# microsoft/esvit

Measured on NVIDIA H100. Metric: multi-crop images/sec, Swin-T W7 pretrain step (2 global 224^2 + 8 local 96^2 crops, DDINOLoss V+R, K=65536), higher is better.
Workload: dtype bf16

## Files before the change

esvit_b200/_lib.py:

```python
from __future__ import annotations

import ctypes
import os
from ctypes import c_double, c_float, c_int, c_longlong, c_void_p

HERE = os.path.dirname(os.path.abspath(__file__))
LIB_PATH = os.path.join(HERE, "lib", "libesvit_b200.so")
HEADER_PATH = os.path.join(os.path.dirname(HERE), "include", "esvit_b200.h")

ERR_BAD_ARG = 1001

P, I, L, F, D = c_void_p, c_int, c_longlong, c_float, c_double

SIGNATURES = {
    "esvit_add_ln_fwd": [P, P, P, I, P, P, F, P, P, I, P, P, L, I, P],
    "esvit_add_ln_bwd": [P, I, P, P, P, P, P, P, I, P, P, P, P, P, L, I, P],
    "esvit_patch_merge_ln_fwd": [P, P, P, F, P, P, P, I, I, I, I, P],
    "esvit_patch_merge_ln_bwd": [P, P, P, P, P, P, P, P, I, I, I, I, P],
    "esvit_token_mean_fwd": [P, P, I, I, I, P],
    "esvit_token_mean_bwd": [P, P, P, I, I, I, P],
    "esvit_patch_embed_fwd": [P, P, P, P, P, F, P, P, P, I, I, I, I, P],
    "esvit_patch_embed_bwd": [P, P, P, P, P, P, P, P, P, P, P, I, I, I, I, P],
    "esvit_window_attn_expand_bias": [P, P, I, I, P],
    "esvit_window_attn_fwd": [P, P, P, P, I, P, P, I, I, I, I, I, I, I, F, P],
    "esvit_window_attn_bwd": [P, P, P, P, I, P, P, P, P, P, P, I, I, I, I, I, I, I, F, P],
    "esvit_window_attn_probs": [P, P, P, P, I, P, I, I, I, I, I, I, I, F, P],
    "esvit_gemm_bias_act": [P, P, P, P, P, L, I, I, I, P],
    "esvit_gemm_mul_colsum": [P, P, P, P, P, P, L, I, I, P],
    "esvit_gemm_bf16": [P, P, P, P, P, L, I, I, I, I, I, I, P],
    "esvit_gemm_mul_colsum2": [P, P, P, P, P, P, L, I, I, I, I, P],
    "esvit_gemm_wgrad_ws_floats": [I, I],
    "esvit_gemm_wgrad": [P, P, P, P, L, I, I, I, I, P],
    "esvit_mlp_fwd": [P, P, P, P, P, P, P, P, L, I, P],
    "esvit_gelu_fwd": [P, P, L, P],
    "esvit_gelu_bwd": [P, P, P, L, P],
    "esvit_gelu_bwd_dbias": [P, P, P, P, L, I, P],
    "esvit_mul_bwd_dbias": [P, P, P, P, L, I, P],
    "esvit_l2norm_fwd": [P, P, P, F, L, I, P],
    "esvit_l2norm_bwd": [P, P, P, P, L, I, P],
    "esvit_weight_norm_fwd": [P, P, P, P, L, I, P],
    "esvit_weight_norm_bwd": [P, P, P, P, I, P, P, L, I, P],
    "esvit_row_lse": [P, P, F, P, L, I, P],
    "esvit_dino_ce_fwd": [P, P, P, P, P, P, P, F, F, P, L, I, P],
    "esvit_dino_ce_bwd": [P, P, P, P, P, P, P, P, P, F, F, P, L, I, P],
    "esvit_weighted_sum": [P, P, I, P, P],
    "esvit_row_softmax_q_max_k": [],
    "esvit_row_softmax_q": [P, P, F, P, P, L, I, P],
    "esvit_dino_ce_q_fwd": [P, P, P, P, P, F, P, L, I, P],
    "esvit_dino_ce_q_bwd": [P, P, P, P, P, P, P, F, P, L, I, P],
    "esvit_mixup_q_kpad": [I],
    "esvit_mixup_q": [P, P, I, I, I, F, P, P, P, P],
    "esvit_colsum_workspace_rows": [],
    "esvit_colsum": [P, L, I, P, P, P],
    "esvit_center_ema": [P, P, F, F, P, I, P],
    "esvit_normalize_rows": [P, P, L, I, F, P],
    "esvit_region_match": [P, P, I, I, I, I, I, P, P, P],
    "esvit_mhsa_fwd": [P, P, P, I, I, I, I, F, P],
    "esvit_mhsa_bwd": [P, P, P, P, P, P, I, I, I, I, F, P],
    "esvit_conv_im2col": [P, P, I, I, I, I, I, I, I, I, I, P],
    "esvit_conv_col2im": [P, P, I, I, I, I, I, I, I, I, P],
    "esvit_mhsa_win_fwd": [P, P, P, I, I, I, I, I, I, F, P],
    "esvit_mhsa_win_bwd": [P, P, P, P, P, P, I, I, I, I, I, I, F, P],
    "esvit_dwbn_fwd_stats": [P, P, P, P, P, I, I, I, I, I, I, P],
    "esvit_dwbn_fwd_apply": [P, P, P, P, P, P, P, P, P, L, I, I, F, F, P],
    "esvit_dwbn_bwd_stats": [P, P, P, P, P, P, P, L, I, P],
    "esvit_dwbn_bwd_apply": [P, P, P, P, P, P, P, P, P, P, I, I, I, I, I, I, I, P],
    "esvit_vil_sc_ws_floats": [I, I, I, I],
    "esvit_vil_sc_fwd": [P, P, P, P, P, P, P, P, I, I, I, I, F, P],
    "esvit_vil_sc_bwd": [P, P, P, P, P, P, P, P, P, P, P, P, P, P, P, I, I, I, I, F, P],
    "esvit_vil_dense_parts": [I],
    "esvit_vil_dense_fwd": [P, P, P, P, I, I, I, I, F, P],
    "esvit_vil_dense_bwd": [P, P, P, P, P, P, P, P, P, I, I, I, I, F, P],
    "esvit_vil_im2col": [P, P, I, I, I, I, I, I, I, I, P],
    "esvit_vil_col2im": [P, P, I, I, I, I, I, I, I, I, P],
    "esvit_vil_cls_cat_fwd": [P, P, P, I, I, I, P],
    "esvit_vil_cls_cat_bwd": [P, P, P, I, I, I, I, P],
    "esvit_vil_bias_spmv": [P, P, P, P, P, P, I, I, P, I, P],
    "esvit_vit_patches": [P, P, I, I, I, P],
    "esvit_vit_tokens_fwd": [P, P, P, P, I, I, I, P],
    "esvit_vit_tokens_bwd": [P, P, P, P, P, I, I, I, I, P],
    "esvit_vit_split": [P, P, P, I, I, I, I, P],
    "esvit_ema_multi": [P, P, P, I, D, P],
    "esvit_clip_multi": [P, P, I, F, P, P, P],
    "esvit_grad_sumsq_multi": [P, P, I, P, P],
    "esvit_adamw_ema_multi": [P, P, P, P, P, P, P, P, I, P, P, P, P],
    "esvit_knn_prep": [P, P, P, P, L, L, I, P],
    "esvit_knn_select": [P, L, P, P, P, P, P, I, I, I, I, I, P, P, P, P, P, P],
    "esvit_knn_vote": [P, P, P, P, L, I, F, I, P, P],
    "esvit_augment_coeffs": [P, P, P, I, I, P],
    "esvit_augment_resize_h": [P, P, P, P, P, I, L, P],
    "esvit_augment_color": [P, P, P, P, P, I, I, I, P],
    "esvit_augment_eval_coeffs": [P, P, P, I, I, P],
    "esvit_augment_eval_resize_h": [P, P, P, P, P, I, I, L, P],
    "esvit_augment_eval_resize_v": [P, P, P, P, P, I, I, P],
}

_lib = None


class EsvitKernelError(RuntimeError):
    pass


def load() -> ctypes.CDLL:
    global _lib
    if _lib is not None:
        return _lib
    if not os.path.isfile(LIB_PATH):
        raise EsvitKernelError(
            f"{LIB_PATH} not found: the esvit_b200 CUDA library has not been built "
            "(run `python -m esvit_b200.build` or `__graft_entry__.build()`); there is no CPU fallback")
    lib = ctypes.CDLL(LIB_PATH)
    for name, argtypes in SIGNATURES.items():
        fn = getattr(lib, name)
        fn.argtypes = argtypes
        fn.restype = c_int
    _lib = lib
    return lib


def _cuda_error_string(code: int) -> str:
    try:
        import torch
        return torch.cuda.cudart().cudaGetErrorString(code) if hasattr(torch.cuda.cudart(), "cudaGetErrorString") \
            else f"cudaError {code}"
    except Exception:
        return f"cudaError {code}"


def call(name: str, *args) -> None:
    rc = getattr(load(), name)(*args)
    if rc != 0:
        if rc == ERR_BAD_ARG:
            raise ValueError(f"{name}: unsupported shape / argument (ESVIT_ERR_BAD_ARG)")
        raise EsvitKernelError(f"{name} failed: {_cuda_error_string(rc)} (status {rc})")


_LAUNCHES = {"esvit_colsum": 2, "esvit_gemm_mul_colsum": 2, "esvit_gemm_mul_colsum2": 2, "esvit_gemm_wgrad": 2,
             "esvit_mixup_q": 2}
_launch_count = 0
_timed_names = set()
_timed_events = []
_META = {
    "esvit_dino_ce_bwd": lambda a: {"rows": int(a[-3]), "K": int(a[-2])},
    "esvit_window_attn_bwd": lambda a: _attn_meta(a),
    "esvit_window_attn_fwd": lambda a: _attn_meta(a),
    "esvit_window_attn_probs": lambda a: _attn_meta(a),
    "esvit_gemm_bias_act": lambda a: {"M": int(a[5]), "N": int(a[6]), "K": int(a[7])},
    "esvit_gemm_mul_colsum": lambda a: {"M": int(a[6]), "N": int(a[7]), "K": int(a[8])},
    "esvit_gemm_bf16": lambda a: {"M": int(a[5]), "N": int(a[6]), "K": int(a[7]), "b_mn": int(a[9]), "act": int(a[10]),
                                  "pre": a[4] is not None and a[4].value is not None},
    "esvit_gemm_mul_colsum2": lambda a: {"M": int(a[6]), "N": int(a[7]), "K": int(a[8])},
    "esvit_gemm_wgrad": lambda a: {"T": int(a[4]), "N": int(a[5]), "K": int(a[6])},
    "esvit_mlp_fwd": lambda a: {"M": int(a[8]), "C": int(a[9]), "student": a[6] is not None and a[6].value is not None},
    "esvit_add_ln_fwd": lambda a: {"T": int(a[-3]), "C": int(a[-2]), "has_x": a[0] is not None and a[0].value is not None,
                                   "has_delta": a[1] is not None and a[1].value is not None},
    "esvit_add_ln_bwd": lambda a: {"T": int(a[-3]), "C": int(a[-2])},
    "esvit_dino_ce_fwd": lambda a: {"rows": int(a[-3]), "K": int(a[-2])},
    "esvit_dino_ce_q_fwd": lambda a: {"rows": int(a[-3]), "K": int(a[-2])},
    "esvit_dino_ce_q_bwd": lambda a: {"rows": int(a[-3]), "K": int(a[-2])},
    "esvit_row_softmax_q": lambda a: {"rows": int(a[-3]), "K": int(a[-2])},
    "esvit_mixup_q": lambda a: {"ncrops": int(a[2]), "B": int(a[3]), "K": int(a[4])},
    "esvit_conv_im2col": lambda a: {"B": int(a[3]), "C": int(a[4]), "H": int(a[5]), "W": int(a[6]), "k": int(a[7]),
                                    "s": int(a[8]), "p": int(a[9]), "Kp": int(a[10])},
    "esvit_conv_col2im": lambda a: {"B": int(a[2]), "C": int(a[3]), "H": int(a[4]), "W": int(a[5]), "k": int(a[6]),
                                    "s": int(a[7]), "p": int(a[8]), "Kp": int(a[9])},
    "esvit_dwbn_fwd_stats": lambda a: {"B": int(a[5]), "H": int(a[6]), "W": int(a[7]), "Hp": int(a[8]), "Wp": int(a[9]),
                                       "C": int(a[10])},
    "esvit_dwbn_fwd_apply": lambda a: {"N": int(a[9]), "C": int(a[10])},
    "esvit_dwbn_bwd_stats": lambda a: {"N": int(a[7]), "C": int(a[8])},
    "esvit_dwbn_bwd_apply": lambda a: {"B": int(a[10]), "H": int(a[11]), "W": int(a[12]), "Hp": int(a[13]),
                                       "Wp": int(a[14]), "C": int(a[15])},
    "esvit_mhsa_win_fwd": lambda a: {"B": int(a[3]), "H": int(a[4]), "W": int(a[5]), "w": int(a[6]), "C": int(a[7]),
                                     "nH": int(a[8])},
    "esvit_mhsa_win_bwd": lambda a: {"B": int(a[6]), "H": int(a[7]), "W": int(a[8]), "w": int(a[9]), "C": int(a[10]),
                                     "nH": int(a[11])},
    "esvit_vil_sc_fwd": lambda a: {"B": int(a[8]), "nx": int(a[9]), "ny": int(a[10]), "nH": int(a[11])},
    "esvit_vil_sc_bwd": lambda a: {"B": int(a[15]), "nx": int(a[16]), "ny": int(a[17]), "nH": int(a[18])},
    "esvit_vil_dense_fwd": lambda a: {"B": int(a[4]), "L": int(a[5]), "C": int(a[6]), "nH": int(a[7])},
    "esvit_vil_dense_bwd": lambda a: {"B": int(a[9]), "L": int(a[10]), "C": int(a[11]), "nH": int(a[12])},
    "esvit_mhsa_fwd": lambda a: {"B": int(a[3]), "L": int(a[4]), "C": int(a[5]), "nH": int(a[6])},
    "esvit_mhsa_bwd": lambda a: {"B": int(a[6]), "L": int(a[7]), "C": int(a[8]), "nH": int(a[9])},
    "esvit_vit_tokens_bwd": lambda a: {"B": int(a[-5]), "N": int(a[-4]), "D": int(a[-3])},
    "esvit_patch_embed_fwd": lambda a: {"B": int(a[-5]), "H": int(a[-4]), "W": int(a[-3]), "E": int(a[-2])},
    "esvit_patch_embed_bwd": lambda a: {"B": int(a[-5]), "H": int(a[-4]), "W": int(a[-3]), "E": int(a[-2])},
}


def _attn_meta(a):
    B, H, W, C, nH, ws = (int(a[i]) for i in (-9, -8, -7, -6, -5, -4))
    return {"tokens": B * H * W, "C": C, "nH": nH, "ws": ws, "windows": B * (-(-H // ws)) * (-(-W // ws))}


def reset_counters() -> None:
    global _launch_count
    _launch_count = 0
    _timed_events.clear()


def launch_count() -> int:
    return _launch_count


def time_entry_point(names) -> None:
    global _timed_names
    if names is None:
        _timed_names = set()
    elif isinstance(names, str):
        _timed_names = {names}
    else:
        _timed_names = set(names)


def timed_results():
    out = []
    for name, e0, e1, meta in _timed_events:
        d = {"name": name, "ms": e0.elapsed_time(e1)}
        d.update(meta)
        out.append(d)
    return out


_plain_call = call


def call(name: str, *args) -> None:
    global _launch_count
    if name == "esvit_ema_multi":
        _launch_count += (args[3] + 63) // 64
    elif name == "esvit_clip_multi":
        _launch_count += 2 * ((args[2] + 63) // 64)
    elif name == "esvit_grad_sumsq_multi":
        _launch_count += (args[2] + 63) // 64
    elif name == "esvit_adamw_ema_multi":
        _launch_count += (args[8] + 31) // 32 + 1
    else:
        _launch_count += _LAUNCHES.get(name, 1)
    if name in _timed_names:
        import torch
        e0, e1 = torch.cuda.Event(enable_timing=True), torch.cuda.Event(enable_timing=True)
        e0.record()
        _plain_call(name, *args)
        e1.record()
        _timed_events.append((name, e0, e1, _META[name](args) if name in _META else {}))
    else:
        _plain_call(name, *args)
```

esvit_b200/csrc/gemm2_wgmma.cu:

```cuda
#include <cuda.h>

#include "common.cuh"

namespace hg {

constexpr int BK = 64;
constexpr int FOLD_THREADS = 64;
constexpr int SMEM_LIMIT = 232448;
enum { EPI_BIAS = 0, EPI_GELU = 1, EPI_MUL = 2, EPI_F32 = 3 };

__device__ __forceinline__ uint32_t smem_u32(const void* p) { return (uint32_t)__cvta_generic_to_shared(p); }
__device__ __forceinline__ void mbar_init(uint64_t* bar, uint32_t count) {
  asm volatile("mbarrier.init.shared::cta.b64 [%0], %1;\n" ::"r"(smem_u32(bar)), "r"(count));
}
__device__ __forceinline__ void mbar_expect_tx(uint64_t* bar, uint32_t bytes) {
  asm volatile("mbarrier.arrive.expect_tx.shared::cta.b64 _, [%0], %1;\n" ::"r"(smem_u32(bar)), "r"(bytes) : "memory");
}
__device__ __forceinline__ void mbar_arrive(uint64_t* bar) {
  asm volatile("mbarrier.arrive.shared::cta.b64 _, [%0];\n" ::"r"(smem_u32(bar)) : "memory");
}
__device__ __forceinline__ uint64_t global_ns() {
  uint64_t t;
  asm volatile("mov.u64 %0, %%globaltimer;\n" : "=l"(t));
  return t;
}
__device__ __forceinline__ void mbar_wait(uint64_t* bar, uint32_t parity) {
  const uint32_t a = smem_u32(bar);
  uint32_t done = 0;
  uint64_t t0 = 0;
  for (uint32_t it = 0;; ++it) {
    asm volatile(
        "{\n\t.reg .pred p;\n\t"
        "mbarrier.try_wait.parity.shared::cta.b64 p, [%1], %2;\n\t"
        "selp.u32 %0, 1, 0, p;\n\t}\n"
        : "=r"(done)
        : "r"(a), "r"(parity)
        : "memory");
    if (done) return;
    if ((it & 1023u) == 1023u) {
      const uint64_t t = global_ns();
      if (t0 == 0) t0 = t;
      else if (t - t0 > 2000000000ull) __trap();
    }
  }
}
__device__ __forceinline__ void tma_load_2d(uint32_t smem_dst, const CUtensorMap* map, uint64_t* bar, int c0, int c1) {
  asm volatile(
      "cp.async.bulk.tensor.2d.shared::cluster.global.mbarrier::complete_tx::bytes [%0], [%1, {%3, %4}], [%2];\n" ::"r"(smem_dst),
      "l"(map), "r"(smem_u32(bar)), "r"(c0), "r"(c1)
      : "memory");
}
__device__ __forceinline__ void tma_store_2d(const CUtensorMap* map, uint32_t smem_src, int c0, int c1) {
  asm volatile("cp.async.bulk.tensor.2d.global.shared::cta.bulk_group [%0, {%2, %3}], [%1];\n" ::"l"(map), "r"(smem_src),
               "r"(c0), "r"(c1)
               : "memory");
}
__device__ __forceinline__ void bulk_commit() { asm volatile("cp.async.bulk.commit_group;\n" ::: "memory"); }
template <int N>
__device__ __forceinline__ void bulk_wait_read() { asm volatile("cp.async.bulk.wait_group.read %0;\n" ::"n"(N) : "memory"); }
__device__ __forceinline__ void bulk_wait_all() { asm volatile("cp.async.bulk.wait_group 0;\n" ::: "memory"); }
__device__ __forceinline__ void fence_proxy_async() { asm volatile("fence.proxy.async.shared::cta;\n" ::: "memory"); }
__device__ __forceinline__ void named_barrier(int id, int threads) {
  asm volatile("bar.sync %0, %1;\n" ::"r"(id), "r"(threads) : "memory");
}
__device__ __forceinline__ void stmatrix_x4(uint32_t addr, uint32_t r0, uint32_t r1, uint32_t r2, uint32_t r3) {
  asm volatile("stmatrix.sync.aligned.m8n8.x4.shared.b16 [%0], {%1, %2, %3, %4};\n" ::"r"(addr), "r"(r0), "r"(r1), "r"(r2),
               "r"(r3)
               : "memory");
}
__device__ __forceinline__ void ldmatrix_x4(uint32_t addr, uint32_t& r0, uint32_t& r1, uint32_t& r2, uint32_t& r3) {
  asm volatile("ldmatrix.sync.aligned.m8n8.x4.shared.b16 {%0, %1, %2, %3}, [%4];\n"
               : "=r"(r0), "=r"(r1), "=r"(r2), "=r"(r3)
               : "r"(addr)
               : "memory");
}
__device__ __forceinline__ float2 unpack_bf162(uint32_t u) { return __bfloat1622float2(*reinterpret_cast<const bf162*>(&u)); }

__device__ __forceinline__ uint64_t make_smem_desc(uint32_t smem_addr, bool mn_major) {
  uint64_t d = 0;
  d |= (uint64_t)((smem_addr & 0x3FFFF) >> 4);
  d |= (uint64_t)(mn_major ? (8192 >> 4) : 1) << 16;
  d |= (uint64_t)(1024 >> 4) << 32;
  d |= (uint64_t)1 << 62;
  return d;
}
__device__ __forceinline__ void wgmma_fence() { asm volatile("wgmma.fence.sync.aligned;\n" ::: "memory"); }
__device__ __forceinline__ void wgmma_commit() { asm volatile("wgmma.commit_group.sync.aligned;\n" ::: "memory"); }
template <int N>
__device__ __forceinline__ void wgmma_wait() { asm volatile("wgmma.wait_group.sync.aligned %0;\n" ::"n"(N) : "memory"); }

template <int TA, int TB>
__device__ __forceinline__ void wgmma_n128(float (&d)[64], uint64_t da, uint64_t db, uint32_t scale_d) {
  asm volatile(
      "{\n\t.reg .pred p;\n\t"
      "setp.ne.b32 p, %66, 0;\n\t"
      "wgmma.mma_async.sync.aligned.m64n128k16.f32.bf16.bf16 "
      "{%0, %1, %2, %3, %4, %5, %6, %7, %8, %9, %10, %11, %12, %13, %14, %15, %16, %17, %18, %19, %20, %21, %22, %23, %24, %25, %26, %27, %28, %29, %30, %31, %32, %33, %34, %35, %36, %37, %38, %39, %40, %41, %42, %43, %44, %45, %46, %47, %48, %49, %50, %51, %52, %53, %54, %55, %56, %57, %58, %59, %60, %61, %62, %63}, "
      "%64, %65, p, 1, 1, %67, %68;\n\t}\n"
      : "+f"(d[0]), "+f"(d[1]), "+f"(d[2]), "+f"(d[3]), "+f"(d[4]), "+f"(d[5]), "+f"(d[6]), "+f"(d[7]), "+f"(d[8]), "+f"(d[9]), "+f"(d[10]), "+f"(d[11]), "+f"(d[12]), "+f"(d[13]), "+f"(d[14]), "+f"(d[15]), "+f"(d[16]), "+f"(d[17]), "+f"(d[18]), "+f"(d[19]), "+f"(d[20]), "+f"(d[21]), "+f"(d[22]), "+f"(d[23]), "+f"(d[24]), "+f"(d[25]), "+f"(d[26]), "+f"(d[27]), "+f"(d[28]), "+f"(d[29]), "+f"(d[30]), "+f"(d[31]), "+f"(d[32]), "+f"(d[33]), "+f"(d[34]), "+f"(d[35]), "+f"(d[36]), "+f"(d[37]), "+f"(d[38]), "+f"(d[39]), "+f"(d[40]), "+f"(d[41]), "+f"(d[42]), "+f"(d[43]), "+f"(d[44]), "+f"(d[45]), "+f"(d[46]), "+f"(d[47]), "+f"(d[48]), "+f"(d[49]), "+f"(d[50]), "+f"(d[51]), "+f"(d[52]), "+f"(d[53]), "+f"(d[54]), "+f"(d[55]), "+f"(d[56]), "+f"(d[57]), "+f"(d[58]), "+f"(d[59]), "+f"(d[60]), "+f"(d[61]), "+f"(d[62]), "+f"(d[63])
      : "l"(da), "l"(db), "r"(scale_d), "n"(TA), "n"(TB));
}
template <int TA, int TB>
__device__ __forceinline__ void wgmma_n256(float (&d)[128], uint64_t da, uint64_t db, uint32_t scale_d) {
  asm volatile(
      "{\n\t.reg .pred p;\n\t"
      "setp.ne.b32 p, %130, 0;\n\t"
      "wgmma.mma_async.sync.aligned.m64n256k16.f32.bf16.bf16 "
      "{%0, %1, %2, %3, %4, %5, %6, %7, %8, %9, %10, %11, %12, %13, %14, %15, %16, %17, %18, %19, %20, %21, %22, %23, %24, %25, %26, %27, %28, %29, %30, %31, %32, %33, %34, %35, %36, %37, %38, %39, %40, %41, %42, %43, %44, %45, %46, %47, %48, %49, %50, %51, %52, %53, %54, %55, %56, %57, %58, %59, %60, %61, %62, %63, %64, %65, %66, %67, %68, %69, %70, %71, %72, %73, %74, %75, %76, %77, %78, %79, %80, %81, %82, %83, %84, %85, %86, %87, %88, %89, %90, %91, %92, %93, %94, %95, %96, %97, %98, %99, %100, %101, %102, %103, %104, %105, %106, %107, %108, %109, %110, %111, %112, %113, %114, %115, %116, %117, %118, %119, %120, %121, %122, %123, %124, %125, %126, %127}, "
      "%128, %129, p, 1, 1, %131, %132;\n\t}\n"
      : "+f"(d[0]), "+f"(d[1]), "+f"(d[2]), "+f"(d[3]), "+f"(d[4]), "+f"(d[5]), "+f"(d[6]), "+f"(d[7]), "+f"(d[8]), "+f"(d[9]), "+f"(d[10]), "+f"(d[11]), "+f"(d[12]), "+f"(d[13]), "+f"(d[14]), "+f"(d[15]), "+f"(d[16]), "+f"(d[17]), "+f"(d[18]), "+f"(d[19]), "+f"(d[20]), "+f"(d[21]), "+f"(d[22]), "+f"(d[23]), "+f"(d[24]), "+f"(d[25]), "+f"(d[26]), "+f"(d[27]), "+f"(d[28]), "+f"(d[29]), "+f"(d[30]), "+f"(d[31]), "+f"(d[32]), "+f"(d[33]), "+f"(d[34]), "+f"(d[35]), "+f"(d[36]), "+f"(d[37]), "+f"(d[38]), "+f"(d[39]), "+f"(d[40]), "+f"(d[41]), "+f"(d[42]), "+f"(d[43]), "+f"(d[44]), "+f"(d[45]), "+f"(d[46]), "+f"(d[47]), "+f"(d[48]), "+f"(d[49]), "+f"(d[50]), "+f"(d[51]), "+f"(d[52]), "+f"(d[53]), "+f"(d[54]), "+f"(d[55]), "+f"(d[56]), "+f"(d[57]), "+f"(d[58]), "+f"(d[59]), "+f"(d[60]), "+f"(d[61]), "+f"(d[62]), "+f"(d[63]), "+f"(d[64]), "+f"(d[65]), "+f"(d[66]), "+f"(d[67]), "+f"(d[68]), "+f"(d[69]), "+f"(d[70]), "+f"(d[71]), "+f"(d[72]), "+f"(d[73]), "+f"(d[74]), "+f"(d[75]), "+f"(d[76]), "+f"(d[77]), "+f"(d[78]), "+f"(d[79]), "+f"(d[80]), "+f"(d[81]), "+f"(d[82]), "+f"(d[83]), "+f"(d[84]), "+f"(d[85]), "+f"(d[86]), "+f"(d[87]), "+f"(d[88]), "+f"(d[89]), "+f"(d[90]), "+f"(d[91]), "+f"(d[92]), "+f"(d[93]), "+f"(d[94]), "+f"(d[95]), "+f"(d[96]), "+f"(d[97]), "+f"(d[98]), "+f"(d[99]), "+f"(d[100]), "+f"(d[101]), "+f"(d[102]), "+f"(d[103]), "+f"(d[104]), "+f"(d[105]), "+f"(d[106]), "+f"(d[107]), "+f"(d[108]), "+f"(d[109]), "+f"(d[110]), "+f"(d[111]), "+f"(d[112]), "+f"(d[113]), "+f"(d[114]), "+f"(d[115]), "+f"(d[116]), "+f"(d[117]), "+f"(d[118]), "+f"(d[119]), "+f"(d[120]), "+f"(d[121]), "+f"(d[122]), "+f"(d[123]), "+f"(d[124]), "+f"(d[125]), "+f"(d[126]), "+f"(d[127])
      : "l"(da), "l"(db), "r"(scale_d), "n"(TA), "n"(TB));
}

__device__ __forceinline__ void wgmma_ss_n64(float (&d)[32], uint64_t da, uint64_t db, uint32_t scale_d) {
  asm volatile(
      "{\n\t.reg .pred p;\n\t"
      "setp.ne.b32 p, %34, 0;\n\t"
      "wgmma.mma_async.sync.aligned.m64n64k16.f32.bf16.bf16 "
      "{%0, %1, %2, %3, %4, %5, %6, %7, %8, %9, %10, %11, %12, %13, %14, %15, %16, %17, %18, %19, %20, %21, %22, %23, %24, %25, %26, %27, %28, %29, %30, %31}, "
      "%32, %33, p, 1, 1, 0, 0;\n\t}\n"
      : "+f"(d[0]), "+f"(d[1]), "+f"(d[2]), "+f"(d[3]), "+f"(d[4]), "+f"(d[5]), "+f"(d[6]), "+f"(d[7]), "+f"(d[8]), "+f"(d[9]), "+f"(d[10]), "+f"(d[11]), "+f"(d[12]), "+f"(d[13]), "+f"(d[14]), "+f"(d[15]), "+f"(d[16]), "+f"(d[17]), "+f"(d[18]), "+f"(d[19]), "+f"(d[20]), "+f"(d[21]), "+f"(d[22]), "+f"(d[23]), "+f"(d[24]), "+f"(d[25]), "+f"(d[26]), "+f"(d[27]), "+f"(d[28]), "+f"(d[29]), "+f"(d[30]), "+f"(d[31])
      : "l"(da), "l"(db), "r"(scale_d));
}
__device__ __forceinline__ void wgmma_rs(float (&d)[48], const uint32_t (&a)[4], uint64_t db, uint32_t scale_d) {
  asm volatile(
      "{\n\t.reg .pred p;\n\t"
      "setp.ne.b32 p, %53, 0;\n\t"
      "wgmma.mma_async.sync.aligned.m64n96k16.f32.bf16.bf16 "
      "{%0, %1, %2, %3, %4, %5, %6, %7, %8, %9, %10, %11, %12, %13, %14, %15, %16, %17, %18, %19, %20, %21, %22, %23, %24, %25, %26, %27, %28, %29, %30, %31, %32, %33, %34, %35, %36, %37, %38, %39, %40, %41, %42, %43, %44, %45, %46, %47}, "
      "{%48, %49, %50, %51}, %52, p, 1, 1, 0;\n\t}\n"
      : "+f"(d[0]), "+f"(d[1]), "+f"(d[2]), "+f"(d[3]), "+f"(d[4]), "+f"(d[5]), "+f"(d[6]), "+f"(d[7]), "+f"(d[8]), "+f"(d[9]), "+f"(d[10]), "+f"(d[11]), "+f"(d[12]), "+f"(d[13]), "+f"(d[14]), "+f"(d[15]), "+f"(d[16]), "+f"(d[17]), "+f"(d[18]), "+f"(d[19]), "+f"(d[20]), "+f"(d[21]), "+f"(d[22]), "+f"(d[23]), "+f"(d[24]), "+f"(d[25]), "+f"(d[26]), "+f"(d[27]), "+f"(d[28]), "+f"(d[29]), "+f"(d[30]), "+f"(d[31]), "+f"(d[32]), "+f"(d[33]), "+f"(d[34]), "+f"(d[35]), "+f"(d[36]), "+f"(d[37]), "+f"(d[38]), "+f"(d[39]), "+f"(d[40]), "+f"(d[41]), "+f"(d[42]), "+f"(d[43]), "+f"(d[44]), "+f"(d[45]), "+f"(d[46]), "+f"(d[47])
      : "r"(a[0]), "r"(a[1]), "r"(a[2]), "r"(a[3]), "l"(db), "r"(scale_d));
}
__device__ __forceinline__ void wgmma_rs(float (&d)[64], const uint32_t (&a)[4], uint64_t db, uint32_t scale_d) {
  asm volatile(
      "{\n\t.reg .pred p;\n\t"
      "setp.ne.b32 p, %69, 0;\n\t"
      "wgmma.mma_async.sync.aligned.m64n128k16.f32.bf16.bf16 "
      "{%0, %1, %2, %3, %4, %5, %6, %7, %8, %9, %10, %11, %12, %13, %14, %15, %16, %17, %18, %19, %20, %21, %22, %23, %24, %25, %26, %27, %28, %29, %30, %31, %32, %33, %34, %35, %36, %37, %38, %39, %40, %41, %42, %43, %44, %45, %46, %47, %48, %49, %50, %51, %52, %53, %54, %55, %56, %57, %58, %59, %60, %61, %62, %63}, "
      "{%64, %65, %66, %67}, %68, p, 1, 1, 0;\n\t}\n"
      : "+f"(d[0]), "+f"(d[1]), "+f"(d[2]), "+f"(d[3]), "+f"(d[4]), "+f"(d[5]), "+f"(d[6]), "+f"(d[7]), "+f"(d[8]), "+f"(d[9]), "+f"(d[10]), "+f"(d[11]), "+f"(d[12]), "+f"(d[13]), "+f"(d[14]), "+f"(d[15]), "+f"(d[16]), "+f"(d[17]), "+f"(d[18]), "+f"(d[19]), "+f"(d[20]), "+f"(d[21]), "+f"(d[22]), "+f"(d[23]), "+f"(d[24]), "+f"(d[25]), "+f"(d[26]), "+f"(d[27]), "+f"(d[28]), "+f"(d[29]), "+f"(d[30]), "+f"(d[31]), "+f"(d[32]), "+f"(d[33]), "+f"(d[34]), "+f"(d[35]), "+f"(d[36]), "+f"(d[37]), "+f"(d[38]), "+f"(d[39]), "+f"(d[40]), "+f"(d[41]), "+f"(d[42]), "+f"(d[43]), "+f"(d[44]), "+f"(d[45]), "+f"(d[46]), "+f"(d[47]), "+f"(d[48]), "+f"(d[49]), "+f"(d[50]), "+f"(d[51]), "+f"(d[52]), "+f"(d[53]), "+f"(d[54]), "+f"(d[55]), "+f"(d[56]), "+f"(d[57]), "+f"(d[58]), "+f"(d[59]), "+f"(d[60]), "+f"(d[61]), "+f"(d[62]), "+f"(d[63])
      : "r"(a[0]), "r"(a[1]), "r"(a[2]), "r"(a[3]), "l"(db), "r"(scale_d));
}
__device__ __forceinline__ void wgmma_rs(float (&d)[96], const uint32_t (&a)[4], uint64_t db, uint32_t scale_d) {
  asm volatile(
      "{\n\t.reg .pred p;\n\t"
      "setp.ne.b32 p, %101, 0;\n\t"
      "wgmma.mma_async.sync.aligned.m64n192k16.f32.bf16.bf16 "
      "{%0, %1, %2, %3, %4, %5, %6, %7, %8, %9, %10, %11, %12, %13, %14, %15, %16, %17, %18, %19, %20, %21, %22, %23, %24, %25, %26, %27, %28, %29, %30, %31, %32, %33, %34, %35, %36, %37, %38, %39, %40, %41, %42, %43, %44, %45, %46, %47, %48, %49, %50, %51, %52, %53, %54, %55, %56, %57, %58, %59, %60, %61, %62, %63, %64, %65, %66, %67, %68, %69, %70, %71, %72, %73, %74, %75, %76, %77, %78, %79, %80, %81, %82, %83, %84, %85, %86, %87, %88, %89, %90, %91, %92, %93, %94, %95}, "
      "{%96, %97, %98, %99}, %100, p, 1, 1, 0;\n\t}\n"
      : "+f"(d[0]), "+f"(d[1]), "+f"(d[2]), "+f"(d[3]), "+f"(d[4]), "+f"(d[5]), "+f"(d[6]), "+f"(d[7]), "+f"(d[8]), "+f"(d[9]), "+f"(d[10]), "+f"(d[11]), "+f"(d[12]), "+f"(d[13]), "+f"(d[14]), "+f"(d[15]), "+f"(d[16]), "+f"(d[17]), "+f"(d[18]), "+f"(d[19]), "+f"(d[20]), "+f"(d[21]), "+f"(d[22]), "+f"(d[23]), "+f"(d[24]), "+f"(d[25]), "+f"(d[26]), "+f"(d[27]), "+f"(d[28]), "+f"(d[29]), "+f"(d[30]), "+f"(d[31]), "+f"(d[32]), "+f"(d[33]), "+f"(d[34]), "+f"(d[35]), "+f"(d[36]), "+f"(d[37]), "+f"(d[38]), "+f"(d[39]), "+f"(d[40]), "+f"(d[41]), "+f"(d[42]), "+f"(d[43]), "+f"(d[44]), "+f"(d[45]), "+f"(d[46]), "+f"(d[47]), "+f"(d[48]), "+f"(d[49]), "+f"(d[50]), "+f"(d[51]), "+f"(d[52]), "+f"(d[53]), "+f"(d[54]), "+f"(d[55]), "+f"(d[56]), "+f"(d[57]), "+f"(d[58]), "+f"(d[59]), "+f"(d[60]), "+f"(d[61]), "+f"(d[62]), "+f"(d[63]), "+f"(d[64]), "+f"(d[65]), "+f"(d[66]), "+f"(d[67]), "+f"(d[68]), "+f"(d[69]), "+f"(d[70]), "+f"(d[71]), "+f"(d[72]), "+f"(d[73]), "+f"(d[74]), "+f"(d[75]), "+f"(d[76]), "+f"(d[77]), "+f"(d[78]), "+f"(d[79]), "+f"(d[80]), "+f"(d[81]), "+f"(d[82]), "+f"(d[83]), "+f"(d[84]), "+f"(d[85]), "+f"(d[86]), "+f"(d[87]), "+f"(d[88]), "+f"(d[89]), "+f"(d[90]), "+f"(d[91]), "+f"(d[92]), "+f"(d[93]), "+f"(d[94]), "+f"(d[95])
      : "r"(a[0]), "r"(a[1]), "r"(a[2]), "r"(a[3]), "l"(db), "r"(scale_d));
}

template <int BN, int TA, int TB>
__device__ __forceinline__ void wgmma_tile(float (&d)[BN / 2], uint64_t da, uint64_t db, uint32_t scale_d) {
  if constexpr (BN == 256) wgmma_n256<TA, TB>(d, da, db, scale_d);
  else wgmma_n128<TA, TB>(d, da, db, scale_d);
}

constexpr float GELU_A = 0.7978845608028654f, GELU_B = 0.7978845608028654f * 0.044715f;
__device__ __forceinline__ float tanh_approx(float x) {
  float y;
  asm("tanh.approx.f32 %0, %1;\n" : "=f"(y) : "f"(x));
  return y;
}
__device__ __forceinline__ float gelu_fwd(float x) {
  const float x2 = x * x;
  const float th = tanh_approx(x * fmaf(GELU_B, x2, GELU_A));
  const float hx = 0.5f * x;
  return fmaf(hx, th, hx);
}
__device__ __forceinline__ float gelu_fwd_grad(float x, float& dy) {
  const float x2 = x * x;
  const float th = tanh_approx(x * fmaf(GELU_B, x2, GELU_A));
  const float hx = 0.5f * x;
  const float m = fmaf(th, th, -1.f);
  const float nc = fmaf(-3.f * GELU_B, x2, -GELU_A);
  dy = fmaf(hx * m, nc, fmaf(0.5f, th, 0.5f));
  return fmaf(hx, th, hx);
}
constexpr float QGELU_A = 1.702f;
__device__ __forceinline__ float qgelu_fwd(float x) { return x * __frcp_rn(1.f + __expf(-QGELU_A * x)); }
__device__ __forceinline__ float qgelu_fwd_grad(float x, float& dy) {
  const float s = __frcp_rn(1.f + __expf(-QGELU_A * x));
  dy = s * fmaf(QGELU_A * x, 1.f - s, 1.f);
  return x * s;
}

struct Params {
  const float* bias;
  bf16* out;
  bf16* aux;
  float* colsum;
  float* part;
  int M, N, K;
  int splits;
  int kb_per_split;
};

template <int WG, int BN, int EPI>
struct Cfg {
  static constexpr bool PP = WG == 1;
  static constexpr int NEP = PP ? 2 : 1;
  static constexpr int BM = 64 * WG;
  static constexpr int A_BYTES = BM * BK * 2;
  static constexpr int B_BYTES = BN * BK * 2;
  static constexpr int STAGE_BYTES = A_BYTES + B_BYTES;
  static constexpr int BAR_BYTES = PP ? 512 : 256;
  static constexpr int NCHUNK = BN / 64;
  static constexpr int CHUNK_BYTES = BM * 128;
  static constexpr int EP_WG_BYTES = EPI == EPI_BIAS ? 2 * CHUNK_BYTES
                                   : EPI == EPI_GELU ? 4 * CHUNK_BYTES
                                   : EPI == EPI_MUL  ? NCHUNK * CHUNK_BYTES : 0;
  static constexpr int EP_BYTES = NEP * EP_WG_BYTES;
  static constexpr int CS_BYTES = EPI == EPI_MUL ? 8 * BN * 4 : 0;
  static constexpr int STAGES_RAW = (SMEM_LIMIT - 1024  - BAR_BYTES - EP_BYTES - CS_BYTES) / STAGE_BYTES;
  static constexpr int STAGES = STAGES_RAW > 6 ? 6 : STAGES_RAW;
  static constexpr int SMEM = 1024 + STAGES * STAGE_BYTES + EP_BYTES + CS_BYTES + BAR_BYTES;
  static constexpr int NTHREADS = 384;
  static_assert(STAGES >= (BN == 256 && (WG == 2 || EPI == EPI_MUL) ? 3 : 4), "operand ring too shallow");
  static_assert(SMEM <= SMEM_LIMIT, "shared memory budget");
  static_assert((2 * STAGES + 2 * NEP + 2 * NEP * NCHUNK + 2) * 8 <= BAR_BYTES, "mbarrier area");
};

template <int WG, int BN, int EPI, int AMN, int BMN, bool QUICK = false>
__global__ void __launch_bounds__(384, 1) gemm_kernel(const __grid_constant__ CUtensorMap map_a,
                                                      const __grid_constant__ CUtensorMap map_b,
                                                      const __grid_constant__ CUtensorMap map_o,
                                                      const __grid_constant__ CUtensorMap map_x,
                                                      const Params p) {
  using C = Cfg<WG, BN, EPI>;
  constexpr int STAGES = C::STAGES, BM = C::BM, NCHUNK = C::NCHUNK;
  constexpr bool PP = C::PP;
  extern __shared__ __align__(1024) uint8_t smem_raw[];
  uint8_t* tiles = smem_raw + ((1024u - (smem_u32(smem_raw) & 1023u)) & 1023u);
  uint8_t* ep = tiles + STAGES * C::STAGE_BYTES;
  float* cs_part = reinterpret_cast<float*>(ep + C::EP_BYTES);
  uint64_t* full = reinterpret_cast<uint64_t*>(ep + C::EP_BYTES + C::CS_BYTES);
  uint64_t* empty = full + STAGES;
  uint64_t* cs_full = empty + STAGES;
  uint64_t* cs_empty = cs_full + C::NEP;
  uint64_t* mul_full = cs_empty + C::NEP;
  uint64_t* mul_empty = mul_full + C::NEP * NCHUNK;
  uint64_t* turn = mul_empty + C::NEP * NCHUNK;

  const int wg = threadIdx.x >> 7;
  const int m_tiles = (p.M + BM - 1) / BM, n_tiles = (p.N + BN - 1) / BN;
  const int tiles_mn = m_tiles * n_tiles, num_items = tiles_mn * p.splits;
  const int k_blocks = (p.K + BK - 1) / BK;

  if (threadIdx.x == 0) {
    asm volatile("prefetch.tensormap [%0];\n" ::"l"(&map_a) : "memory");
    asm volatile("prefetch.tensormap [%0];\n" ::"l"(&map_b) : "memory");
    for (int i = 0; i < STAGES; i++) { mbar_init(&full[i], 1); mbar_init(&empty[i], 128 * WG); }
    for (int e = 0; e < C::NEP; e++) { mbar_init(&cs_full[e], 4 * WG); mbar_init(&cs_empty[e], FOLD_THREADS); }
    if constexpr (EPI == EPI_MUL)
      for (int i = 0; i < C::NEP * NCHUNK; i++) { mbar_init(&mul_full[i], 1); mbar_init(&mul_empty[i], WG); }
    if constexpr (PP) { mbar_init(&turn[0], 128); mbar_init(&turn[1], 128); }
    asm volatile("fence.mbarrier_init.release.cluster;\n" ::: "memory");
  }
  __syncthreads();

  if (wg == 2) {
    asm volatile("setmaxnreg.dec.sync.aligned.u32 40;\n" ::: "memory");
    if (threadIdx.x == 256) {
      int stage = 0;
      uint32_t phase = 0;
      int local = 0;
      if constexpr (EPI == EPI_MUL) asm volatile("prefetch.tensormap [%0];\n" ::"l"(&map_x) : "memory");
      for (int item = blockIdx.x; item < num_items; item += gridDim.x, local++) {
        const int tile = item % tiles_mn, split = item / tiles_mn;
        const int m0 = (tile / n_tiles) * BM, n0 = (tile % n_tiles) * BN;
        const int kb0 = split * p.kb_per_split;
        int kb1 = kb0 + p.kb_per_split; kb1 = kb1 < k_blocks ? kb1 : k_blocks;
        const int e = PP ? (local & 1) : 0, use = PP ? local >> 1 : local;
        auto load_mul = [&](int j) {
          mbar_wait(&mul_empty[e * NCHUNK + j], (use & 1) ^ 1);
          const uint32_t dst = smem_u32(ep + e * C::EP_WG_BYTES + j * C::CHUNK_BYTES);
          mbar_expect_tx(&mul_full[e * NCHUNK + j], C::CHUNK_BYTES);
#pragma unroll
          for (int h = 0; h < WG; h++)
            tma_load_2d(dst + h * 8192, &map_x, &mul_full[e * NCHUNK + j], n0 + 64 * j, m0 + 64 * h);
        };
        for (int kb = kb0; kb < kb1; kb++) {
          mbar_wait(&empty[stage], phase ^ 1);
          const uint32_t sa = smem_u32(tiles + stage * C::STAGE_BYTES), sb = sa + C::A_BYTES;
          mbar_expect_tx(&full[stage], C::STAGE_BYTES);
          if (!AMN) {
            tma_load_2d(sa, &map_a, &full[stage], kb * BK, m0);
          } else {
#pragma unroll
            for (int j = 0; j < BM / 64; j++)
              tma_load_2d(sa + j * 8192, &map_a, &full[stage], m0 + j * 64, kb * BK);
          }
          if (!BMN) {
            tma_load_2d(sb, &map_b, &full[stage], kb * BK, n0);
          } else {
#pragma unroll
            for (int j = 0; j < BN / 64; j++)
              tma_load_2d(sb + j * 8192, &map_b, &full[stage], n0 + j * 64, kb * BK);
          }
          if (++stage == STAGES) { stage = 0; phase ^= 1; }
          if constexpr (EPI == EPI_MUL) if (kb - kb0 < NCHUNK) load_mul(kb - kb0);
        }
        if constexpr (EPI == EPI_MUL)
          for (int j = kb1 - kb0; j < NCHUNK; j++) load_mul(j);
      }
    } else if (EPI == EPI_MUL && threadIdx.x >= 256 + 32 && threadIdx.x < 256 + 32 + FOLD_THREADS) {
      const int t = threadIdx.x - 256 - 32;
      float* dst = p.colsum + (long long)blockIdx.x * p.N;
      int local = 0;
      for (int item = blockIdx.x; item < num_items; item += gridDim.x, local++) {
        const int n0 = ((item % tiles_mn) % n_tiles) * BN;
        const int e = PP ? (local & 1) : 0, use = PP ? local >> 1 : local;
        mbar_wait(&cs_full[e], use & 1);
        for (int c = t; c < BN && n0 + c < p.N; c += FOLD_THREADS) {
          float sum = 0.f;
#pragma unroll
          for (int w = 0; w < 4 * WG; w++) sum += cs_part[(4 * e + w) * BN + c];
          atomicAdd(dst + n0 + c, sum);
        }
        mbar_arrive(&cs_empty[e]);
      }
    }
  } else {
    asm volatile("setmaxnreg.inc.sync.aligned.u32 232;\n" ::: "memory");
    const int t = threadIdx.x & 127, warp = t >> 5, lane = t & 31;
    const int row0 = PP ? 0 : 64 * wg;
    const int frag_row = row0 + warp * 16 + (lane >> 2);
    const int frag_col = 2 * (lane & 3);
    const uint32_t rows_off = PP ? 0u : (uint32_t)wg * 8192u;
    const int e = PP ? wg : 0;
    uint8_t* const my_ep = ep + e * C::EP_WG_BYTES;
    constexpr uint32_t KSTEP_A = AMN ? (2048 >> 4) : (32 >> 4), KSTEP_B = BMN ? (2048 >> 4) : (32 >> 4);
    int stage = 0;
    uint32_t phase = 0;
    int local = 0;
    for (int item = blockIdx.x; item < num_items; item += gridDim.x, local++) {
      const int tile = item % tiles_mn, split = item / tiles_mn;
      const int m0 = (tile / n_tiles) * BM, n0 = (tile % n_tiles) * BN;
      const int kb0 = split * p.kb_per_split;
      int kb1 = kb0 + p.kb_per_split; kb1 = kb1 < k_blocks ? kb1 : k_blocks;
      if constexpr (PP) {
        if ((local & 1) != wg) {
          stage += kb1 - kb0;
          while (stage >= STAGES) { stage -= STAGES; phase ^= 1; }
          continue;
        }
        if (local > 0) mbar_wait(&turn[wg], ((local - 1) >> 1) & 1);
      }
      const int use = PP ? local >> 1 : local;
      float acc[BN / 2];
      int prev = -1;
      for (int kb = kb0; kb < kb1; kb++) {
        mbar_wait(&full[stage], phase);
        const uint32_t sa = smem_u32(tiles + stage * C::STAGE_BYTES) + rows_off;
        const uint64_t da = make_smem_desc(sa, AMN), db = make_smem_desc(smem_u32(tiles + stage * C::STAGE_BYTES) + C::A_BYTES, BMN);
        wgmma_fence();
#pragma unroll
        for (int k = 0; k < BK / 16; k++)
          wgmma_tile<BN, AMN, BMN>(acc, da + k * KSTEP_A, db + k * KSTEP_B, (kb > kb0 || k != 0) ? 1u : 0u);
        wgmma_commit();
        wgmma_wait<1>();
        if (prev >= 0) mbar_arrive(&empty[prev]);
        prev = stage;
        if (++stage == STAGES) { stage = 0; phase ^= 1; }
      }
      if constexpr (PP) mbar_arrive(&turn[wg ^ 1]);
      wgmma_wait<0>();
      if (prev >= 0) mbar_arrive(&empty[prev]);

      if constexpr (EPI == EPI_F32) {
#pragma unroll
        for (int i = 0; i < BN / 8; i++) {
          const int col = n0 + i * 8 + frag_col;
          if (col >= p.N) continue;
#pragma unroll
          for (int h = 0; h < 2; h++) {
            const int row = m0 + frag_row + 8 * h;
            if (row >= p.M) continue;
            const long long off = (long long)row * p.N + col;
            *reinterpret_cast<float2*>(p.part + (long long)split * p.M * p.N + off) =
                make_float2(acc[4 * i + 2 * h], acc[4 * i + 2 * h + 1]);
          }
        }
        continue;
      }

      if constexpr (EPI == EPI_MUL) mbar_wait(&cs_empty[e], (use & 1) ^ 1);
      const uint32_t lrow = (uint32_t)(warp * 16 + (lane & 15)) * 128u, lsw = lane & 7, lblk = lane >> 4;
      const bool leader = t == 0;
#pragma unroll
      for (int c = 0; c < NCHUNK; c++) {
        uint32_t buf;
        if constexpr (EPI == EPI_MUL) {
          buf = smem_u32(my_ep + c * C::CHUNK_BYTES) + rows_off;
          mbar_wait(&mul_full[e * NCHUNK + c], use & 1);
        } else {
          buf = smem_u32(my_ep + (c & 1) * (EPI == EPI_GELU ? 2 : 1) * C::CHUNK_BYTES) + rows_off;
        }
#pragma unroll
        for (int jj = 0; jj < 8; jj += 2) {
          const int i = c * 8 + jj;
          const uint32_t addr = buf + lrow + (((jj + lblk) ^ lsw) << 4);
          const float* a0 = acc + 4 * i;
          if constexpr (EPI == EPI_MUL) {
            uint32_t m[4];
            ldmatrix_x4(addr, m[0], m[1], m[2], m[3]);
            uint32_t o[4];
            float cs[2][2] = {{0.f, 0.f}, {0.f, 0.f}};
#pragma unroll
            for (int q = 0; q < 4; q++) {
              const float2 mf = unpack_bf162(m[q]);
              o[q] = pack_bf162(a0[2 * q] * mf.x, a0[2 * q + 1] * mf.y);
              const float2 of = unpack_bf162(o[q]);
              cs[q >> 1][0] += of.x; cs[q >> 1][1] += of.y;
            }
            stmatrix_x4(addr, o[0], o[1], o[2], o[3]);
#pragma unroll
            for (int s = 0; s < 2; s++) {
              float cs0 = cs[s][0], cs1 = cs[s][1];
#pragma unroll
              for (int o2 = 4; o2 < 32; o2 <<= 1) {
                cs0 += __shfl_xor_sync(0xffffffffu, cs0, o2);
                cs1 += __shfl_xor_sync(0xffffffffu, cs1, o2);
              }
              if (lane < 4)
                *reinterpret_cast<float2*>(cs_part + (wg * 4 + warp) * BN + (i + s) * 8 + frag_col) = make_float2(cs0, cs1);
            }
          } else {
            float b[4] = {0.f, 0.f, 0.f, 0.f};
            if (p.bias) {
#pragma unroll
              for (int s = 0; s < 2; s++) {
                const int col = n0 + (i + s) * 8 + frag_col;
                if (col < p.N) {
                  const float2 bb = __ldg(reinterpret_cast<const float2*>(p.bias + col));
                  b[2 * s] = bb.x; b[2 * s + 1] = bb.y;
                }
              }
            }
            uint32_t o[4], d[4];
#pragma unroll
            for (int q = 0; q < 4; q++) {
              const float v0 = a0[2 * q] + b[2 * (q >> 1)], v1 = a0[2 * q + 1] + b[2 * (q >> 1) + 1];
              if constexpr (EPI == EPI_GELU) {
                if (p.aux) {
                  float d0, d1;
                  float y0, y1;
                  if constexpr (QUICK) {
                    y0 = qgelu_fwd_grad(v0, d0); y1 = qgelu_fwd_grad(v1, d1);
                  } else {
                    y0 = gelu_fwd_grad(v0, d0); y1 = gelu_fwd_grad(v1, d1);
                  }
                  o[q] = pack_bf162(y0, y1);
                  d[q] = pack_bf162(d0, d1);
                } else if constexpr (QUICK) {
                  o[q] = pack_bf162(qgelu_fwd(v0), qgelu_fwd(v1));
                } else {
                  o[q] = pack_bf162(gelu_fwd(v0), gelu_fwd(v1));
                }
              } else {
                o[q] = pack_bf162(v0, v1);
              }
            }
            stmatrix_x4(addr, o[0], o[1], o[2], o[3]);
            if constexpr (EPI == EPI_GELU)
              if (p.aux) stmatrix_x4(addr + C::CHUNK_BYTES, d[0], d[1], d[2], d[3]);
          }
        }
        fence_proxy_async();
        if constexpr (EPI != EPI_MUL)
          if (leader) bulk_wait_read<0>();
        named_barrier(1 + wg, 128);
        if (leader) {
          const int gc = n0 + 64 * c, gr = m0 + row0;
          if (gc < p.N && gr < p.M) {
            tma_store_2d(&map_o, buf, gc, gr);
            if constexpr (EPI == EPI_GELU)
              if (p.aux) tma_store_2d(&map_x, buf + C::CHUNK_BYTES, gc, gr);
          }
          bulk_commit();
          if constexpr (EPI == EPI_MUL) {
            if (c > 0) { bulk_wait_read<1>(); mbar_arrive(&mul_empty[e * NCHUNK + c - 1]); }
            if (c == NCHUNK - 1) { bulk_wait_read<0>(); mbar_arrive(&mul_empty[e * NCHUNK + c]); }
          }
        }
      }
      if constexpr (EPI == EPI_MUL) {
        __syncwarp();
        if (lane == 0) mbar_arrive(&cs_full[e]);
      }
    }
    if constexpr (EPI != EPI_F32)
      if (t == 0) bulk_wait_all();
  }
}

template <int C>
struct MlpCfg {
  static constexpr int BM = 128, HB = 64;
  static constexpr int KB = (C + 63) / 64;
  static constexpr int NH = 4 * C / HB;
  static constexpr int X_BYTES = KB * BM * 128;
  static constexpr int W1_BYTES = KB * HB * 128;
  static constexpr int W2_BYTES = C * 128;
  static constexpr int STAGE_BYTES = W1_BYTES + W2_BYTES;
  static constexpr int CHUNK_BYTES = BM * 128;
  static constexpr int EP_BYTES = 2 * CHUNK_BYTES;
  static constexpr int BAR_BYTES = 128;
  static constexpr int STAGES_RAW = (SMEM_LIMIT - 1024 - BAR_BYTES - 2 * X_BYTES - EP_BYTES) / STAGE_BYTES;
  static constexpr int STAGES = STAGES_RAW > 4 ? 4 : STAGES_RAW;
  static constexpr int SMEM = 1024 + 2 * X_BYTES + STAGES * STAGE_BYTES + EP_BYTES + BAR_BYTES;
  static_assert(C % 32 == 0 && C <= 192, "acc2 [64 x C] must fit the consumer registers; C / 8 even");
  static_assert(STAGES >= 2, "weight ring too shallow");
  static_assert(SMEM <= SMEM_LIMIT, "shared memory budget");
  static_assert((2 * STAGES + 4) * 8 <= BAR_BYTES, "mbarrier area");
};

struct MlpParams {
  const float* b1;
  const float* b2;
  int M;
};

template <int C, bool STORE>
__global__ void __launch_bounds__(384, 1) mlp_fwd_kernel(const __grid_constant__ CUtensorMap map_x,
                                                         const __grid_constant__ CUtensorMap map_w1,
                                                         const __grid_constant__ CUtensorMap map_w2,
                                                         const __grid_constant__ CUtensorMap map_y,
                                                         const __grid_constant__ CUtensorMap map_h,
                                                         const __grid_constant__ CUtensorMap map_g, const MlpParams p) {
  using G = MlpCfg<C>;
  constexpr int BM = G::BM, KB = G::KB, NH = G::NH, STAGES = G::STAGES;
  extern __shared__ __align__(1024) uint8_t smem_raw[];
  uint8_t* xs = smem_raw + ((1024u - (smem_u32(smem_raw) & 1023u)) & 1023u);
  uint8_t* ws = xs + 2 * G::X_BYTES;
  uint8_t* ep = ws + STAGES * G::STAGE_BYTES;
  uint64_t* full = reinterpret_cast<uint64_t*>(ep + G::EP_BYTES);
  uint64_t* empty = full + STAGES;
  uint64_t* x_full = empty + STAGES;
  uint64_t* x_empty = x_full + 2;

  const int wg = threadIdx.x >> 7;
  const int num_items = (p.M + BM - 1) / BM;
  if (threadIdx.x == 0) {
    asm volatile("prefetch.tensormap [%0];\n" ::"l"(&map_x) : "memory");
    asm volatile("prefetch.tensormap [%0];\n" ::"l"(&map_w1) : "memory");
    asm volatile("prefetch.tensormap [%0];\n" ::"l"(&map_w2) : "memory");
    for (int i = 0; i < STAGES; i++) { mbar_init(&full[i], 1); mbar_init(&empty[i], 256); }
    for (int i = 0; i < 2; i++) { mbar_init(&x_full[i], 1); mbar_init(&x_empty[i], 256); }
    asm volatile("fence.mbarrier_init.release.cluster;\n" ::: "memory");
  }
  __syncthreads();

  if (wg == 2) {
    asm volatile("setmaxnreg.dec.sync.aligned.u32 40;\n" ::: "memory");
    if (threadIdx.x == 256) {
      int stage = 0;
      uint32_t phase = 0;
      int local = 0;
      for (int item = blockIdx.x; item < num_items; item += gridDim.x, local++) {
        const int m0 = item * BM, xb = local & 1;
        mbar_wait(&x_empty[xb], ((local >> 1) & 1) ^ 1);
        mbar_expect_tx(&x_full[xb], G::X_BYTES);
#pragma unroll
        for (int kb = 0; kb < KB; kb++)
          tma_load_2d(smem_u32(xs + xb * G::X_BYTES + kb * BM * 128), &map_x, &x_full[xb], kb * 64, m0);
        for (int j = 0; j < NH; j++) {
          mbar_wait(&empty[stage], phase ^ 1);
          const uint32_t sw = smem_u32(ws + stage * G::STAGE_BYTES);
          mbar_expect_tx(&full[stage], G::STAGE_BYTES);
#pragma unroll
          for (int kb = 0; kb < KB; kb++) tma_load_2d(sw + kb * 8192, &map_w1, &full[stage], kb * 64, j * 64);
          tma_load_2d(sw + G::W1_BYTES, &map_w2, &full[stage], j * 64, 0);
          if (++stage == STAGES) { stage = 0; phase ^= 1; }
        }
      }
    }
  } else {
    asm volatile("setmaxnreg.inc.sync.aligned.u32 232;\n" ::: "memory");
    const int t = threadIdx.x & 127, warp = t >> 5, lane = t & 31;
    const int frag_col = 2 * (lane & 3);
    const uint32_t lrow = (uint32_t)(warp * 16 + (lane & 15)) * 128u, lsw = lane & 7, lblk = lane >> 4;
    const bool leader = t == 0;
    const uint32_t hbuf = smem_u32(ep) + wg * 8192;
    int stage = 0;
    uint32_t phase = 0;
    int local = 0;
    for (int item = blockIdx.x; item < num_items; item += gridDim.x, local++) {
      const int m0 = item * BM, xb = local & 1;
      const uint64_t da = make_smem_desc(smem_u32(xs + xb * G::X_BYTES) + wg * 8192, false);
      float acc1[32], acc2[C / 2];
      mbar_wait(&x_full[xb], (local >> 1) & 1);
      for (int j = 0; j < NH; j++) {
        {
          const uint64_t db = make_smem_desc(smem_u32(ws + stage * G::STAGE_BYTES), false);
          mbar_wait(&full[stage], phase);
          wgmma_fence();
#pragma unroll
          for (int k = 0; k < C / 16; k++)
            wgmma_ss_n64(acc1, da + (k >> 2) * (BM * 128 >> 4) + (k & 3) * 2, db + (k >> 2) * (8192 >> 4) + (k & 3) * 2,
                         k ? 1u : 0u);
          wgmma_commit();
        }
        wgmma_wait<0>();
        if (j == NH - 1) mbar_arrive(&x_empty[xb]);
        if constexpr (STORE) {
          if (leader) bulk_wait_read<0>();
          named_barrier(1 + wg, 128);
        }
        uint32_t af[4][4];
#pragma unroll
        for (int s = 0; s < 4; s++) {
          const float* a0 = acc1 + 8 * s;
          float b[4] = {0.f, 0.f, 0.f, 0.f};
          if (p.b1) {
#pragma unroll
            for (int u = 0; u < 2; u++) {
              const float2 bb = __ldg(reinterpret_cast<const float2*>(p.b1 + j * 64 + (2 * s + u) * 8 + frag_col));
              b[2 * u] = bb.x; b[2 * u + 1] = bb.y;
            }
          }
          uint32_t d[4];
#pragma unroll
          for (int q = 0; q < 4; q++) {
            const float v0 = a0[2 * q] + b[2 * (q >> 1)], v1 = a0[2 * q + 1] + b[2 * (q >> 1) + 1];
            if constexpr (STORE) {
              float d0, d1;
              const float y0 = gelu_fwd_grad(v0, d0), y1 = gelu_fwd_grad(v1, d1);
              af[s][q] = pack_bf162(y0, y1);
              d[q] = pack_bf162(d0, d1);
            } else {
              af[s][q] = pack_bf162(gelu_fwd(v0), gelu_fwd(v1));
            }
          }
          if constexpr (STORE) {
            const uint32_t addr = hbuf + lrow + (((2 * s + lblk) ^ lsw) << 4);
            stmatrix_x4(addr, af[s][0], af[s][1], af[s][2], af[s][3]);
            stmatrix_x4(addr + G::CHUNK_BYTES, d[0], d[1], d[2], d[3]);
          }
        }
        if constexpr (STORE) fence_proxy_async();
        const uint64_t d2 = make_smem_desc(smem_u32(ws + stage * G::STAGE_BYTES) + G::W1_BYTES, false);
        wgmma_fence();
#pragma unroll
        for (int s = 0; s < 4; s++) wgmma_rs(acc2, af[s], d2 + s * 2, (j > 0 || s > 0) ? 1u : 0u);
        wgmma_commit();
        if constexpr (STORE) {
          named_barrier(1 + wg, 128);
          if (leader) {
            const int gr = m0 + 64 * wg;
            if (gr < p.M) {
              tma_store_2d(&map_h, hbuf, j * 64, gr);
              tma_store_2d(&map_g, hbuf + G::CHUNK_BYTES, j * 64, gr);
            }
            bulk_commit();
          }
        }
        wgmma_wait<0>();
        mbar_arrive(&empty[stage]);
        if (++stage == STAGES) { stage = 0; phase ^= 1; }
      }
#pragma unroll
      for (int c = 0; c < KB; c++) {
        const uint32_t buf = smem_u32(ep + (c & 1) * G::CHUNK_BYTES) + wg * 8192;
        if (leader) bulk_wait_read<0>();
        named_barrier(1 + wg, 128);
#pragma unroll
        for (int jj = 0; jj < 8; jj += 2) {
          const int i = c * 8 + jj;
          if (i >= C / 8) continue;
          const float* a0 = acc2 + 4 * i;
          float b[4] = {0.f, 0.f, 0.f, 0.f};
          if (p.b2) {
#pragma unroll
            for (int u = 0; u < 2; u++) {
              const float2 bb = __ldg(reinterpret_cast<const float2*>(p.b2 + (i + u) * 8 + frag_col));
              b[2 * u] = bb.x; b[2 * u + 1] = bb.y;
            }
          }
          uint32_t o[4];
#pragma unroll
          for (int q = 0; q < 4; q++) o[q] = pack_bf162(a0[2 * q] + b[2 * (q >> 1)], a0[2 * q + 1] + b[2 * (q >> 1) + 1]);
          stmatrix_x4(buf + lrow + (((jj + lblk) ^ lsw) << 4), o[0], o[1], o[2], o[3]);
        }
        fence_proxy_async();
        named_barrier(1 + wg, 128);
        if (leader) {
          const int gr = m0 + 64 * wg;
          if (gr < p.M) tma_store_2d(&map_y, buf, c * 64, gr);
          bulk_commit();
        }
      }
    }
    if (t == 0) bulk_wait_all();
  }
}

typedef CUresult (*EncodeFn)(CUtensorMap*, CUtensorMapDataType, cuuint32_t, void*, const cuuint64_t*, const cuuint64_t*,
                             const cuuint32_t*, const cuuint32_t*, CUtensorMapInterleave, CUtensorMapSwizzle,
                             CUtensorMapL2promotion, CUtensorMapFloatOOBfill);

static EncodeFn get_encode() {
  static EncodeFn fn = nullptr;
  if (!fn) {
    void* ptr = nullptr;
    cudaDriverEntryPointQueryResult qres;
    if (cudaGetDriverEntryPoint("cuTensorMapEncodeTiled", &ptr, cudaEnableDefault, &qres) == cudaSuccess &&
        qres == cudaDriverEntryPointSuccess)
      fn = (EncodeFn)ptr;
  }
  return fn;
}

static bool make_map(CUtensorMap* map, const void* ptr, long long rows, long long cols, int box_rows) {
  EncodeFn enc = get_encode();
  if (!enc) return false;
  cuuint64_t dims[2] = {(cuuint64_t)cols, (cuuint64_t)rows};
  cuuint64_t strides[1] = {(cuuint64_t)cols * 2};
  cuuint32_t box[2] = {64u, (cuuint32_t)box_rows};
  cuuint32_t estr[2] = {1, 1};
  auto encode = [&]() {
    return enc(map, CU_TENSOR_MAP_DATA_TYPE_BFLOAT16, 2, const_cast<void*>(ptr), dims, strides, box, estr,
               CU_TENSOR_MAP_INTERLEAVE_NONE, CU_TENSOR_MAP_SWIZZLE_128B, CU_TENSOR_MAP_L2_PROMOTION_L2_128B,
               CU_TENSOR_MAP_FLOAT_OOB_FILL_NONE);
  };
  CUresult r = encode();
  if (r == CUDA_ERROR_INVALID_CONTEXT) {
    int dev = 0;
    if (cudaGetDevice(&dev) == cudaSuccess && cudaSetDevice(dev) == cudaSuccess) r = encode();
  }
  return r == CUDA_SUCCESS;
}

template <int C, bool STORE>
static int mlp_launch(const void* x, const void* w1, const float* b1, const void* w2, const float* b2, void* y, void* h,
                      void* g, int M, void* stream) {
  using G = MlpCfg<C>;
  CUtensorMap mx, m1, m2, my, mh = {}, mg = {};
  if (!make_map(&mx, x, M, C, G::BM) || !make_map(&m1, w1, 4 * C, C, 64) || !make_map(&m2, w2, C, 4 * C, C) ||
      !make_map(&my, y, M, C, 64))
    return ESVIT_ERR_BAD_ARG;
  if (STORE && (!make_map(&mh, h, M, 4 * C, 64) || !make_map(&mg, g, M, 4 * C, 64))) return ESVIT_ERR_BAD_ARG;
  auto kernel = mlp_fwd_kernel<C, STORE>;
  static bool attr_set = false;
  if (!attr_set) {
    cudaError_t e = cudaFuncSetAttribute(kernel, cudaFuncAttributeMaxDynamicSharedMemorySize, G::SMEM);
    if (e != cudaSuccess) return (int)e;
    attr_set = true;
  }
  const int items = (M + G::BM - 1) / G::BM;
  int grid = esvit_num_sms();
  if (grid > items) grid = items;
  MlpParams p;
  p.b1 = b1; p.b2 = b2; p.M = M;
  kernel<<<grid, 384, G::SMEM, (cudaStream_t)stream>>>(mx, m1, m2, my, mh, mg, p);
  return (int)cudaGetLastError();
}

template <int C>
static int mlp_launch_c(const void* x, const void* w1, const float* b1, const void* w2, const float* b2, void* y, void* h,
                        void* g, int M, void* stream) {
  return h ? mlp_launch<C, true>(x, w1, b1, w2, b2, y, h, g, M, stream)
           : mlp_launch<C, false>(x, w1, b1, w2, b2, y, h, g, M, stream);
}

__global__ void __launch_bounds__(256) colsum_fold_kernel(const float* __restrict__ ws, int rows, int N, float* __restrict__ colsum) {
  const int n = blockIdx.x * 256 + threadIdx.x;
  if (n >= N) return;
  float s = 0.f;
  for (int r = 0; r < rows; r++) s += ws[(long long)r * N + n];
  colsum[n] += s;
}

__global__ void __launch_bounds__(256) split_fold_kernel(const float* __restrict__ part, int splits, long long n4,
                                                         float* __restrict__ out, int accumulate) {
  const long long i = (long long)blockIdx.x * 256 + threadIdx.x;
  if (i >= n4) return;
  float4 s = accumulate ? reinterpret_cast<const float4*>(out)[i] : make_float4(0.f, 0.f, 0.f, 0.f);
  for (int k = 0; k < splits; k++) {
    const float4 t = reinterpret_cast<const float4*>(part)[(long long)k * n4 + i];
    s.x += t.x; s.y += t.y; s.z += t.z; s.w += t.w;
  }
  reinterpret_cast<float4*>(out)[i] = s;
}

constexpr int MAX_GRID = 160;

struct Call {
  const void* a; const void* b;
  int a_mn, b_mn;
  Params p;
};

template <int WG, int BN, int EPI, int AMN, int BMN, bool QUICK = false>
static int launch_cfg(const Call& c, void* stream, int* rows_out) {
  using C = Cfg<WG, BN, EPI>;
  Params p = c.p;
  CUtensorMap ma, mb;
  if (!(AMN ? make_map(&ma, c.a, p.K, p.M, 64) : make_map(&ma, c.a, p.M, p.K, C::BM))) return ESVIT_ERR_BAD_ARG;
  if (!(BMN ? make_map(&mb, c.b, p.K, p.N, 64) : make_map(&mb, c.b, p.N, p.K, BN))) return ESVIT_ERR_BAD_ARG;
  CUtensorMap mo = {}, mx = {};
  if (EPI != EPI_F32) {
    auto aligned = [](const void* q) { return ((uintptr_t)q & 15u) == 0; };
    if (!p.out || !aligned(p.out) || (p.aux && !aligned(p.aux))) return ESVIT_ERR_BAD_ARG;
    if (!make_map(&mo, p.out, p.M, p.N, 64)) return ESVIT_ERR_BAD_ARG;
    if (p.aux && !make_map(&mx, p.aux, p.M, p.N, 64)) return ESVIT_ERR_BAD_ARG;
  }
  auto kernel = gemm_kernel<WG, BN, EPI, AMN, BMN, QUICK>;
  static bool attr_set = false;
  if (!attr_set) {
    cudaError_t e = cudaFuncSetAttribute(kernel, cudaFuncAttributeMaxDynamicSharedMemorySize, C::SMEM);
    if (e != cudaSuccess) return (int)e;
    attr_set = true;
  }
  const int m_tiles = (p.M + C::BM - 1) / C::BM, n_tiles = (p.N + BN - 1) / BN;
  const long long items = (long long)m_tiles * n_tiles * p.splits;
  int grid = esvit_num_sms();
  if (EPI == EPI_MUL && grid > MAX_GRID) grid = MAX_GRID;
  if ((long long)grid > items) grid = (int)items;
  if (EPI == EPI_MUL) {
    cudaError_t e = cudaMemsetAsync(p.colsum, 0, (size_t)grid * p.N * sizeof(float), (cudaStream_t)stream);
    if (e != cudaSuccess) return (int)e;
  }
  if (rows_out) *rows_out = grid;
  kernel<<<grid, C::NTHREADS, C::SMEM, (cudaStream_t)stream>>>(ma, mb, mo, mx, p);
  return (int)cudaGetLastError();
}

template <int WG, int BN, int EPI>
static int launch_majors(const Call& c, void* stream, int* rows_out) {
  if constexpr (EPI == EPI_F32) {
    if (c.a_mn && c.b_mn) return launch_cfg<WG, BN, EPI, 1, 1>(c, stream, rows_out);
  } else if constexpr (EPI == EPI_MUL) {
    if (!c.a_mn) return c.b_mn ? launch_cfg<WG, BN, EPI, 0, 1>(c, stream, rows_out) : launch_cfg<WG, BN, EPI, 0, 0>(c, stream, rows_out);
  } else {
    if (!c.a_mn) return c.b_mn ? launch_cfg<WG, BN, EPI, 0, 1>(c, stream, rows_out) : launch_cfg<WG, BN, EPI, 0, 0>(c, stream, rows_out);
    return c.b_mn ? launch_cfg<WG, BN, EPI, 1, 1>(c, stream, rows_out) : launch_cfg<WG, BN, EPI, 1, 0>(c, stream, rows_out);
  }
  return ESVIT_ERR_BAD_ARG;
}

template <int EPI>
static int launch_epi(const Call& c, int wg, int bn, void* stream, int* rows_out) {
  if (wg == 2 && bn == 256) return launch_majors<2, 256, EPI>(c, stream, rows_out);
  if (wg == 2 && bn == 128) return launch_majors<2, 128, EPI>(c, stream, rows_out);
  if (wg == 1 && bn == 256) return launch_majors<1, 256, EPI>(c, stream, rows_out);
  if (wg == 1 && bn == 128) return launch_majors<1, 128, EPI>(c, stream, rows_out);
  return ESVIT_ERR_BAD_ARG;
}

static int launch_quick(const Call& c, int wg, int bn, void* stream) {
  if (c.a_mn || c.b_mn) return ESVIT_ERR_BAD_ARG;
  if (wg == 2 && bn == 256) return launch_cfg<2, 256, EPI_GELU, 0, 0, true>(c, stream, nullptr);
  if (wg == 2 && bn == 128) return launch_cfg<2, 128, EPI_GELU, 0, 0, true>(c, stream, nullptr);
  if (wg == 1 && bn == 256) return launch_cfg<1, 256, EPI_GELU, 0, 0, true>(c, stream, nullptr);
  if (wg == 1 && bn == 128) return launch_cfg<1, 128, EPI_GELU, 0, 0, true>(c, stream, nullptr);
  return ESVIT_ERR_BAD_ARG;
}

static int launch(const Call& c, int epi, int wg, int bn, void* stream, int* rows_out = nullptr) {
  switch (epi) {
    case EPI_BIAS: return launch_epi<EPI_BIAS>(c, wg, bn, stream, rows_out);
    case EPI_GELU: return launch_epi<EPI_GELU>(c, wg, bn, stream, rows_out);
    case EPI_MUL: return launch_epi<EPI_MUL>(c, wg, bn, stream, rows_out);
    case EPI_F32: return launch_epi<EPI_F32>(c, wg, bn, stream, rows_out);
  }
  return ESVIT_ERR_BAD_ARG;
}

static bool pads_more(long long n, int wide, int narrow) {
  return (n + wide - 1) / wide * wide > (n + narrow - 1) / narrow * narrow;
}
static void pick_tile(long long M, int N, int K, int tile, bool fit_n, int* wg, int* bn) {
  tile %= 10000;
  if (tile > 0) { *wg = tile / 1000; *bn = tile % 1000; return; }
  const int sms = esvit_num_sms();
  const bool narrow = fit_n && (pads_more(N, 256, 128) || K <= 256);
  const int cand[4][2] = {{2, 256}, {2, 128}, {1, 256}, {1, 128}};
  for (const auto& cd : cand) {
    if (cd[1] == 256 && (N <= 128 || narrow)) continue;
    const long long items = ((M + 64 * cd[0] - 1) / (64 * cd[0])) * ((N + cd[1] - 1) / cd[1]);
    if (items >= sms) { *wg = cd[0]; *bn = cd[1]; return; }
  }
  *wg = 1; *bn = 128;
}
static void pick_tile_wgrad(int Nout, int Kin, int tile, int* wg, int* bn) {
  tile %= 10000;
  if (tile > 0) { *wg = tile / 1000; *bn = tile % 1000; return; }
  *bn = Kin > 128 && !pads_more(Kin, 256, 128) ? 256 : 128;
  *wg = Nout > 64 && !pads_more(Nout, 128, 64) ? 2 : 1;
}

}

ESVIT_API int esvit_gemm_bf16(const void* a, const void* b, const float* bias, void* out, void* pre, long long M, int N,
                              int K, int a_mn, int b_mn, int act, int tile, void* stream) {
  if (M <= 0 || N <= 0 || K <= 0 || (N % 8) || (K % 8) || M > 0x7fffffffLL || (a_mn && (M % 8)) || act < 0 || act > 2)
    return ESVIT_ERR_BAD_ARG;
  hg::Call c;
  c.a = a; c.b = b; c.a_mn = a_mn ? 1 : 0; c.b_mn = b_mn ? 1 : 0;
  c.p.bias = bias; c.p.out = (bf16*)out; c.p.aux = act ? (bf16*)pre : nullptr; c.p.colsum = nullptr; c.p.part = nullptr;
  c.p.M = (int)M; c.p.N = N; c.p.K = K; c.p.splits = 1; c.p.kb_per_split = (K + hg::BK - 1) / hg::BK;
  int wg, bn;
  hg::pick_tile(M, N, K, tile, true, &wg, &bn);
  if (act == 2) return hg::launch_quick(c, wg, bn, stream);
  return hg::launch(c, act ? hg::EPI_GELU : hg::EPI_BIAS, wg, bn, stream);
}

ESVIT_API int esvit_gemm_mul_colsum2(const void* a, const void* b, const void* mult, void* out, float* colsum, float* ws,
                                     long long M, int N, int K, int b_mn, int tile, void* stream) {
  if (M <= 0 || N <= 0 || K <= 0 || (N % 8) || (K % 8) || M > 0x7fffffffLL || !mult || !colsum || !ws) return ESVIT_ERR_BAD_ARG;
  hg::Call c;
  c.a = a; c.b = b; c.a_mn = 0; c.b_mn = b_mn ? 1 : 0;
  c.p.bias = nullptr; c.p.out = (bf16*)out; c.p.aux = (bf16*)mult; c.p.colsum = ws; c.p.part = nullptr;
  c.p.M = (int)M; c.p.N = N; c.p.K = K; c.p.splits = 1; c.p.kb_per_split = (K + hg::BK - 1) / hg::BK;
  int wg, bn, rows = 0;
  hg::pick_tile(M, N, K, tile, false, &wg, &bn);
  const int rc = hg::launch(c, hg::EPI_MUL, wg, bn, stream, &rows);
  if (rc != 0) return rc;
  hg::colsum_fold_kernel<<<(N + 255) / 256, 256, 0, (cudaStream_t)stream>>>(ws, rows, N, colsum);
  ESVIT_LAUNCH_CHECK();
}

static long long wgrad_ws_floats(int N, int K) {
  const int tiles = ((N + 127) / 128) * ((K + 255) / 256);
  long long splits = (2LL * 160 + tiles - 1) / tiles;
  if (splits > 96) splits = 96;
  if (splits < 1) splits = 1;
  return splits * (long long)N * K;
}
ESVIT_API int esvit_gemm_wgrad_ws_floats(int N, int K) {
  const long long n = wgrad_ws_floats(N, K);
  return n > 0x7fffffffLL ? -1 : (int)n;
}
ESVIT_API int esvit_gemm_wgrad(const void* dy, const void* x, float* dw, float* ws, long long T, int N, int K,
                               int accumulate, int tile, void* stream) {
  if (T <= 0 || N <= 0 || K <= 0 || (N % 8) || (K % 8) || T > 0x7fffffffLL || !ws) return ESVIT_ERR_BAD_ARG;
  int wg, bn;
  hg::pick_tile_wgrad(N, K, tile, &wg, &bn);
  const int m_tiles = (N + 64 * wg - 1) / (64 * wg), n_tiles = (K + bn - 1) / bn;
  const int tiles = m_tiles * n_tiles;
  const int k_blocks = (int)((T + hg::BK - 1) / hg::BK);
  const int ctas = esvit_num_sms();
  int splits = tiles >= ctas ? 1 : ctas / tiles;
  if (splits > k_blocks / 8) splits = k_blocks / 8;
  if (tile >= 10000) splits = tile / 10000;
  const long long cap = wgrad_ws_floats(N, K) / ((long long)N * K);
  if (splits > cap) splits = (int)cap;
  if (splits > k_blocks) splits = k_blocks;
  if (splits < 1) splits = 1;
  int kbs = (k_blocks + splits - 1) / splits;
  splits = (k_blocks + kbs - 1) / kbs;
  hg::Call c;
  c.a = dy; c.b = x; c.a_mn = 1; c.b_mn = 1;
  c.p.bias = nullptr; c.p.out = nullptr; c.p.aux = nullptr; c.p.colsum = nullptr; c.p.part = ws;
  c.p.M = N; c.p.N = K; c.p.K = (int)T; c.p.splits = splits; c.p.kb_per_split = kbs;
  const int rc = hg::launch(c, hg::EPI_F32, wg, bn, stream);
  if (rc != 0) return rc;
  const long long n4 = (long long)N * K / 4;
  hg::split_fold_kernel<<<(unsigned)((n4 + 255) / 256), 256, 0, (cudaStream_t)stream>>>(ws, splits, n4, dw, accumulate);
  ESVIT_LAUNCH_CHECK();
}

ESVIT_API int esvit_mlp_fwd(const void* x, const void* w1, const float* b1, const void* w2, const float* b2, void* y,
                            void* h, void* gelu_grad, long long M, int C, void* stream) {
  auto aligned = [](const void* q, uintptr_t a) { return ((uintptr_t)q & (a - 1)) == 0; };
  if (M <= 0 || M > 0x7fffffffLL || !x || !w1 || !w2 || !y || (h == nullptr) != (gelu_grad == nullptr)) return ESVIT_ERR_BAD_ARG;
  if (!aligned(x, 16) || !aligned(w1, 16) || !aligned(w2, 16) || !aligned(y, 16) || !aligned(h, 16) ||
      !aligned(gelu_grad, 16) || !aligned(b1, 8) || !aligned(b2, 8))
    return ESVIT_ERR_BAD_ARG;
  switch (C) {
    case 96: return hg::mlp_launch_c<96>(x, w1, b1, w2, b2, y, h, gelu_grad, (int)M, stream);
    case 128: return hg::mlp_launch_c<128>(x, w1, b1, w2, b2, y, h, gelu_grad, (int)M, stream);
    case 192: return hg::mlp_launch_c<192>(x, w1, b1, w2, b2, y, h, gelu_grad, (int)M, stream);
  }
  return ESVIT_ERR_BAD_ARG;
}

ESVIT_API int esvit_gemm_bias_act(const void* a, const void* w, const float* bias, void* out, void* pre, long long M,
                                  int N, int K, int act, void* stream) {
  return esvit_gemm_bf16(a, w, bias, out, pre, M, N, K, 0, 0, act, 0, stream);
}
ESVIT_API int esvit_gemm_mul_colsum(const void* a, const void* w, const void* mult, void* out, float* colsum, float* ws,
                                    long long M, int N, int K, void* stream) {
  return esvit_gemm_mul_colsum2(a, w, mult, out, colsum, ws, M, N, K, 0, 0, stream);
}
```

esvit_b200/linear.py:

```python
from __future__ import annotations

from typing import Optional

import torch
from torch.autograd import Function
from torch.autograd.function import once_differentiable

from . import ops

Tensor = torch.Tensor
BF16 = torch.bfloat16
F32 = torch.float32


def _wgrad(key, dy2: Tensor, x2: Tensor, shape):
    d = ops._Arena.accs
    if d is None:
        return ops.gemm_wgrad(dy2, x2).view(shape)
    buf = d.get(key)
    if buf is not None and tuple(buf.shape) == tuple(shape):
        ops.gemm_wgrad(dy2, x2, out=buf, accumulate=True)
        return None
    buf = d[key] = ops.gemm_wgrad(dy2, x2).view(shape)
    return buf.view(shape)


class LinearFn(Function):

    @staticmethod
    def forward(ctx, x, wp, w16, bias):
        y = ops.gemm(x, w16, bias)
        ctx.save_for_backward(x, w16)
        ctx.wkey = ("w", wp.data_ptr())
        ctx.wshape = tuple(wp.shape)
        return y

    @staticmethod
    @once_differentiable
    def backward(ctx, g):
        x, w16 = ctx.saved_tensors
        g = ops._chk(g, BF16, "g")
        N, K = w16.shape
        g2 = g.reshape(-1, N)
        dx = ops.gemm(g2, w16, None, b_mn=True).view(x.shape) if ctx.needs_input_grad[0] else None
        dw = _wgrad(ctx.wkey, g2, x.reshape(-1, K), ctx.wshape) if ctx.needs_input_grad[1] else None
        return dx, dw, None, None


class MlpFn(Function):

    @staticmethod
    def forward(ctx, x, w1p, w1, b1, w2p, w2, b2, act: int = 1):
        need = any(ctx.needs_input_grad)
        C = x.shape[-1]
        if act == 1 and C in ops.MLP_FUSED_C and w1.shape[0] == 4 * C:
            if need:
                y, h, pre = ops.mlp_fwd(x, w1, b1, w2, b2, want_h=True)
            else:
                y, h, pre = ops.mlp_fwd(x, w1, b1, w2, b2), None, None
        else:
            if need:
                h, pre = ops.gemm(x, w1, b1, act=act, want_pre=True)
            else:
                h, pre = ops.gemm(x, w1, b1, act=act), None
            y = ops.gemm(h, w2, b2)
        ctx.save_for_backward(x, w1, w2, pre, h)
        ctx.keys = (("w", w1p.data_ptr()), tuple(w1p.shape), ("w", w2p.data_ptr()), tuple(w2p.shape))
        ctx.bias_meta = (b1.shape, b1.device, b1.data_ptr())
        return y

    @staticmethod
    @once_differentiable
    def backward(ctx, g):
        x, w1, w2, pre, h = ctx.saved_tensors
        k1, s1, k2, s2 = ctx.keys
        g = ops._chk(g, BF16, "g")
        Cc, Nh = g.shape[-1], pre.shape[-1]
        g2 = g.reshape(-1, Cc)
        dw2 = _wgrad(k2, g2, h.reshape(-1, Nh), s2) if ctx.needs_input_grad[4] else None
        db1, first = ops._acc(("bias", ctx.bias_meta[2]), tuple(ctx.bias_meta[0]), ctx.bias_meta[1])
        dpre = ops.gemm_mul_colsum(g2, w2, pre.reshape(-1, Nh), db1, b_mn=True)
        dx = ops.gemm(dpre, w1, None, b_mn=True).view(x.shape) if ctx.needs_input_grad[0] else None
        dw1 = _wgrad(k1, dpre, x.reshape(-1, x.shape[-1]), s1) if ctx.needs_input_grad[1] else None
        return dx, dw1, None, (db1 if first else None), dw2, None, None, None


class HeadMlpFn(Function):

    @staticmethod
    def forward(ctx, x, w1p, w1, b1, w2p, w2, b2, w3p, w3, b3):
        need = any(ctx.needs_input_grad)
        if need:
            h1, p1 = ops.gemm(x, w1, b1, act=1, want_pre=True)
            h2, p2 = ops.gemm(h1, w2, b2, act=1, want_pre=True)
        else:
            h1, p1 = ops.gemm(x, w1, b1, act=1), None
            h2, p2 = ops.gemm(h1, w2, b2, act=1), None
        y = ops.gemm(h2, w3, b3)
        ctx.save_for_backward(x, w1, w2, w3, h1, p1, h2, p2)
        ctx.shapes = (tuple(w1p.shape), tuple(w2p.shape), tuple(w3p.shape))
        return y

    @staticmethod
    @once_differentiable
    def backward(ctx, g):
        x, w1, w2, w3, h1, p1, h2, p2 = ctx.saved_tensors
        s1, s2, s3 = ctx.shapes
        g = ops._chk(g, BF16, "g")
        g3 = g.reshape(-1, g.shape[-1])
        dev = g.device
        db3 = ops.colsum(g3)
        dw3 = ops.gemm_wgrad(g3, h2.reshape(-1, h2.shape[-1])).view(s3)
        db2 = torch.zeros(s2[0], dtype=F32, device=dev)
        d2 = ops.gemm_mul_colsum(g3, w3, p2.reshape(-1, p2.shape[-1]), db2, b_mn=True)
        dw2 = ops.gemm_wgrad(d2, h1.reshape(-1, h1.shape[-1])).view(s2)
        db1 = torch.zeros(s1[0], dtype=F32, device=dev)
        d1 = ops.gemm_mul_colsum(d2, w2, p1.reshape(-1, p1.shape[-1]), db1, b_mn=True)
        dw1 = ops.gemm_wgrad(d1, x.reshape(-1, x.shape[-1])).view(s1)
        dx = ops.gemm(d1, w1, None, b_mn=True).view(x.shape) if ctx.needs_input_grad[0] else None
        return dx, dw1, None, db1, dw2, None, db2, dw3, None, db3


class LastLayerFn(Function):

    @staticmethod
    def forward(ctx, x, w_eff):
        y = ops.gemm(x, w_eff, None)
        ctx.save_for_backward(x, w_eff)
        return y

    @staticmethod
    @once_differentiable
    def backward(ctx, g):
        x, w = ctx.saved_tensors
        g = ops._chk(g, BF16, "g")
        Kp, Dm = w.shape
        g2 = g.reshape(-1, Kp)
        dx = ops.gemm(g2, w, None, b_mn=True).view(x.shape) if ctx.needs_input_grad[0] else None
        dw = ops.gemm_wgrad(g2, x.reshape(-1, Dm)).view(Kp, Dm) if ctx.needs_input_grad[1] else None
        return dx, dw
```

esvit_b200/ops.py:

```python
from __future__ import annotations

import ctypes
from typing import List, Optional, Sequence, Tuple

import torch
from torch.autograd import Function
from torch.autograd.function import once_differentiable

from . import _lib, shadow

Tensor = torch.Tensor
BF16 = torch.bfloat16
F32 = torch.float32


def _p(t: Optional[Tensor]):
    return ctypes.c_void_p(t.data_ptr()) if t is not None else None


def _po(t: Tensor, off_elems: int):
    return ctypes.c_void_p(t.data_ptr() + off_elems * t.element_size())


def _stream():
    return ctypes.c_void_p(torch.cuda.current_stream().cuda_stream)


class _Arena:
    buf: Optional[Tensor] = None
    off = 0
    accs: Optional[dict] = None
    warned = False


def begin_step(device, nfloats: int = 1 << 22) -> None:
    _Arena.buf = torch.zeros(nfloats, dtype=F32, device=device)
    _Arena.off = 0
    _Arena.accs = {}


def end_step() -> None:
    _Arena.accs = None


def _acc(key, shape, device) -> Tuple[Tensor, bool]:
    d = _Arena.accs
    if d is None:
        return _zeros(shape, device), True
    t = d.get(key)
    if t is not None and tuple(t.shape) == tuple(shape):
        return t, False
    t = d[key] = _zeros(shape, device)
    return t.view(t.shape), True


def _zeros(shape, device) -> Tensor:
    n = 1
    for d in shape:
        n *= int(d)
    buf = _Arena.buf
    n16 = (n + 3) & ~3
    if buf is not None and buf.device == torch.device(device) and _Arena.off + n16 <= buf.numel():
        v = buf[_Arena.off:_Arena.off + n].view(*shape)
        _Arena.off += n16
        return v
    if buf is not None and not _Arena.warned:
        _Arena.warned = True
        import warnings
        warnings.warn("esvit_b200: gradient-accumulator arena exhausted (%d floats); falling back to per-tensor torch.zeros - "
                      "pass a larger nfloats to ops.begin_step" % buf.numel())
    return torch.zeros(*shape, dtype=F32, device=device)


def _chk(t: Optional[Tensor], dtype, name: str) -> Optional[Tensor]:
    if t is None:
        return None
    if not t.is_cuda:
        raise RuntimeError(f"esvit_b200 op input `{name}` must be a CUDA tensor (no CPU fallback exists)")
    if t.dtype != dtype:
        raise TypeError(f"`{name}` must be {dtype}, got {t.dtype}")
    return t if t.is_contiguous() else t.contiguous()




def _add_ln_fwd(x, delta, keep, tps, gamma, beta, eps, want_y, y_bf16):
    ref = x if x is not None else delta
    T, C = ref.numel() // ref.shape[-1], ref.shape[-1]
    xout = torch.empty(ref.shape, dtype=F32, device=ref.device) if delta is not None else None
    y = mean = rstd = None
    if want_y:
        y = torch.empty(ref.shape, dtype=BF16 if y_bf16 else F32, device=ref.device)
        mean = torch.empty(T, dtype=F32, device=ref.device)
        rstd = torch.empty(T, dtype=F32, device=ref.device)
    _lib.call("esvit_add_ln_fwd", _p(x), _p(delta), _p(keep), tps, _p(gamma), _p(beta), eps, _p(xout), _p(y),
              1 if y_bf16 else 0, _p(mean), _p(rstd), T, C, _stream())
    return (xout if delta is not None else x), y, mean, rstd


class AddLayerNormFn(Function):

    @staticmethod
    def forward(ctx, x, delta, dbias, keep, gamma, beta, eps: float, y_bf16: bool):
        x = _chk(x, F32, "x")
        delta = _chk(delta, BF16, "delta")
        dbias = _chk(dbias, F32, "delta_bias")
        keep = _chk(keep, F32, "keep")
        gamma, beta = _chk(gamma, F32, "gamma"), _chk(beta, F32, "beta")
        ref = x if x is not None else delta
        tps = ref.numel() // ref.shape[-1] // ref.shape[0]
        xout, y, mean, rstd = _add_ln_fwd(x, delta, keep, tps, gamma, beta, eps, True, y_bf16)
        ctx.save_for_backward(xout, mean, rstd, gamma, keep)
        ctx.tps, ctx.y_bf16, ctx.has_dbias, ctx.has_x = tps, y_bf16, dbias is not None, x is not None
        return xout, y

    @staticmethod
    @once_differentiable
    def backward(ctx, g_xout, g_y):
        xout, mean, rstd, gamma, keep = ctx.saved_tensors
        T, C = xout.numel() // xout.shape[-1], xout.shape[-1]
        g_xout = _chk(g_xout, F32, "g_xout") if g_xout is not None else None
        if g_y is not None:
            g_y = _chk(g_y, BF16 if ctx.y_bf16 else F32, "g_y")
        dx = torch.empty_like(xout) if ctx.has_x else None
        ddelta = torch.empty(xout.shape, dtype=BF16, device=xout.device)
        acc, first = _acc(("add_ln", gamma.data_ptr()), (3, C), xout.device)
        _lib.call("esvit_add_ln_bwd", _p(g_y), 1 if ctx.y_bf16 else 0, _p(g_xout), _p(xout), _p(mean), _p(rstd),
                  _p(gamma), _p(keep), ctx.tps, _p(dx), _p(ddelta), _p(acc[0]), _p(acc[1]),
                  _p(acc[2]) if ctx.has_dbias else None, T, C, _stream())
        if not first:
            return dx, ddelta, None, None, None, None, None, None
        return dx, ddelta, (acc[2] if ctx.has_dbias else None), None, acc[0], acc[1], None, None


class LayerNormFn(Function):

    @staticmethod
    def forward(ctx, x, gamma, beta, eps: float, y_bf16: bool):
        x = _chk(x, F32, "x")
        gamma, beta = _chk(gamma, F32, "gamma"), _chk(beta, F32, "beta")
        _, y, mean, rstd = _add_ln_fwd(x, None, None, 1, gamma, beta, eps, True, y_bf16)
        ctx.save_for_backward(x, mean, rstd, gamma)
        ctx.y_bf16 = y_bf16
        return y

    @staticmethod
    @once_differentiable
    def backward(ctx, g_y):
        x, mean, rstd, gamma = ctx.saved_tensors
        T, C = x.numel() // x.shape[-1], x.shape[-1]
        g_y = _chk(g_y, BF16 if ctx.y_bf16 else F32, "g_y")
        dx = torch.empty_like(x)
        acc, first = _acc(("ln", gamma.data_ptr()), (2, C), x.device)
        _lib.call("esvit_add_ln_bwd", _p(g_y), 1 if ctx.y_bf16 else 0, None, _p(x), _p(mean), _p(rstd), _p(gamma),
                  None, 1, _p(dx), None, _p(acc[0]), _p(acc[1]), None, T, C, _stream())
        return (dx, acc[0], acc[1], None, None) if first else (dx, None, None, None, None)


class LayerNormResidFn(Function):

    @staticmethod
    def forward(ctx, x, gamma, beta, eps: float, y_bf16: bool):
        x = _chk(x, F32, "x")
        gamma, beta = _chk(gamma, F32, "gamma"), _chk(beta, F32, "beta")
        _, y, mean, rstd = _add_ln_fwd(x, None, None, 1, gamma, beta, eps, True, y_bf16)
        ctx.save_for_backward(x, mean, rstd, gamma)
        ctx.y_bf16 = y_bf16
        return x.view(x.shape), y

    @staticmethod
    @once_differentiable
    def backward(ctx, g_x, g_y):
        x, mean, rstd, gamma = ctx.saved_tensors
        T, C = x.numel() // x.shape[-1], x.shape[-1]
        g_x = _chk(g_x, F32, "g_x") if g_x is not None else None
        if g_y is None:
            return g_x, None, None, None, None
        g_y = _chk(g_y, BF16 if ctx.y_bf16 else F32, "g_y")
        dx = torch.empty_like(x)
        acc, first = _acc(("ln", gamma.data_ptr()), (2, C), x.device)
        _lib.call("esvit_add_ln_bwd", _p(g_y), 1 if ctx.y_bf16 else 0, _p(g_x), _p(x), _p(mean), _p(rstd), _p(gamma),
                  None, 1, _p(dx), None, _p(acc[0]), _p(acc[1]), None, T, C, _stream())
        return (dx, acc[0], acc[1], None, None) if first else (dx, None, None, None, None)


class ResidualAddFn(Function):

    @staticmethod
    def forward(ctx, x, delta, dbias, keep):
        x, delta, keep = _chk(x, F32, "x"), _chk(delta, BF16, "delta"), _chk(keep, F32, "keep")
        dbias = _chk(dbias, F32, "delta_bias")
        tps = x.numel() // x.shape[-1] // x.shape[0]
        xout, _, _, _ = _add_ln_fwd(x, delta, keep, tps, None, None, 0.0, False, False)
        ctx.save_for_backward(keep)
        ctx.tps, ctx.has_dbias = tps, dbias is not None
        ctx.dbias_ptr = dbias.data_ptr() if dbias is not None else 0
        return xout

    @staticmethod
    @once_differentiable
    def backward(ctx, g):
        (keep,) = ctx.saved_tensors
        g = _chk(g, F32, "g")
        T, C = g.numel() // g.shape[-1], g.shape[-1]
        ddelta = torch.empty(g.shape, dtype=BF16, device=g.device)
        db, first = _acc(("res", ctx.dbias_ptr), (C,), g.device) if ctx.has_dbias else (None, True)
        _lib.call("esvit_add_ln_bwd", None, 0, _p(g), None, None, None, None, _p(keep), ctx.tps, None, _p(ddelta),
                  None, None, _p(db), T, C, _stream())
        return g, ddelta, (db if first else None), None


def add_layer_norm(x: Tensor, delta: Optional[Tensor], keep: Optional[Tensor], gamma: Tensor, beta: Tensor,
                   eps: float, y_bf16: bool = True, delta_bias: Optional[Tensor] = None) -> Tuple[Tensor, Tensor]:
    if delta is None:
        if x.requires_grad and torch.is_grad_enabled():
            return LayerNormResidFn.apply(x, gamma, beta, eps, y_bf16)
        return x, LayerNormFn.apply(x, gamma, beta, eps, y_bf16)
    return AddLayerNormFn.apply(x, delta, delta_bias, keep, gamma, beta, eps, y_bf16)


def residual_add(x: Tensor, delta: Optional[Tensor], keep: Optional[Tensor],
                 delta_bias: Optional[Tensor] = None) -> Tensor:
    return x if delta is None else ResidualAddFn.apply(x, delta, delta_bias, keep)


class PatchEmbedGroupsFn(Function):

    @staticmethod
    def forward(ctx, w, bias, gamma, beta, eps: float, *imgs):
        w, bias = _chk(w, F32, "w"), _chk(bias, F32, "bias")
        gamma, beta = _chk(gamma, F32, "gamma"), _chk(beta, F32, "beta")
        imgs = [_chk(im, F32, "img") for im in imgs]
        E = w.shape[0]
        if tuple(w.shape[1:]) != (3, 4, 4) or any(im.shape[1] != 3 for im in imgs):
            raise ValueError("PatchEmbed kernel supports in_chans=3, patch_size=4")
        rows = [im.shape[0] * (im.shape[2] // 4) * (im.shape[3] // 4) for im in imgs]
        T = sum(rows)
        dev = imgs[0].device
        out = torch.empty(T, E, dtype=F32, device=dev)
        mean = torch.empty(T, dtype=F32, device=dev)
        rstd = torch.empty(T, dtype=F32, device=dev)
        r0 = 0
        for im, n in zip(imgs, rows):
            B, _, H, W = im.shape
            _lib.call("esvit_patch_embed_fwd", _p(im), _p(w), _p(bias), _p(gamma), _p(beta), eps, _p(out[r0:]),
                      _p(mean[r0:]), _p(rstd[r0:]), B, H, W, E, _stream())
            r0 += n
        ctx.save_for_backward(w, bias, gamma, mean, rstd, *imgs)
        ctx.rows = rows
        return out

    @staticmethod
    @once_differentiable
    def backward(ctx, g):
        w, bias, gamma, mean, rstd = ctx.saved_tensors[:5]
        imgs = ctx.saved_tensors[5:]
        E = w.shape[0]
        g = _chk(g, F32, "g")
        dw, first = _acc(("pe_w", w.data_ptr()), tuple(w.shape), w.device)
        acc, _ = _acc(("pe_b", w.data_ptr()), (3, E), w.device)
        r0 = 0
        for im, n in zip(imgs, ctx.rows):
            B, _, H, W = im.shape
            _lib.call("esvit_patch_embed_bwd", _p(im), _p(w), _p(bias), _p(gamma), _p(mean[r0:]), _p(rstd[r0:]),
                      _p(g[r0:]), _p(dw), _p(acc[0]), _p(acc[1]), _p(acc[2]), B, H, W, E, _stream())
            r0 += n
        none = (None,) * len(imgs)
        return ((dw, acc[0], acc[1], acc[2], None) if first else (None, None, None, None, None)) + none


def cat_adjacent(ts):
    ts = list(ts)
    if len(ts) == 1:
        return ts[0]
    t0 = ts[0]
    ok = all(t.shape == t0.shape and t.dtype == t0.dtype and t.device == t0.device and t.is_contiguous()
             and not t.requires_grad for t in ts)
    if ok:
        st, n = t0.untyped_storage(), t0.numel()
        ok = all(t.untyped_storage().data_ptr() == st.data_ptr() and t.storage_offset() == t0.storage_offset() + i * n
                 for i, t in enumerate(ts))
    if not ok:
        return torch.cat(ts)
    shape = (t0.shape[0] * len(ts),) + tuple(t0.shape[1:])
    return torch.as_strided(t0, shape, t0.stride(), t0.storage_offset())


ATTN_WS_FLOATS = 8192


class WindowAttentionGroupsFn(Function):

    @staticmethod
    def forward(ctx, qkv, qkv_bias, bias_table, groups, num_heads: int, ws: int, shift: int, scale: float, bias_exp):
        qkv = _chk(qkv, BF16, "qkv")
        qkv_bias = _chk(qkv_bias, F32, "qkv_bias")
        bias_table = _chk(bias_table, F32, "relative_position_bias_table")
        T, C3 = qkv.shape
        C = C3 // 3
        assert sum(B * H * W for B, H, W, _ in groups) == T
        qb = shadow.lookup(qkv_bias)
        if qb is None:
            qb = qkv_bias.detach().to(BF16)
        out = torch.empty(T, C, dtype=BF16, device=qkv.device)
        lse_off, n = [], 0
        for B, H, W, _ in groups:
            lse_off.append(n)
            n += B * (-(-H // ws)) * (-(-W // ws)) * num_heads * ws * ws
        lse = torch.empty(n, dtype=F32, device=qkv.device)
        ready = 1 if (bias_exp is not None and ws == 7) else 0
        bws = bias_exp if ready else torch.empty(num_heads * ATTN_WS_FLOATS, dtype=F32, device=qkv.device)
        for (B, H, W, r0), lo in zip(groups, lse_off):
            _lib.call("esvit_window_attn_fwd", _po(qkv, r0 * C3), _p(qb), _p(bias_table), _p(bws), ready, _po(out, r0 * C),
                      _po(lse, lo), B, H, W, C, num_heads, ws, shift, scale, _stream())
        ctx.save_for_backward(qkv, qb, bias_table, out, lse, bws if ready else None)
        ctx.meta = (tuple(groups), tuple(lse_off), C, num_heads, ws, shift, scale)
        return out

    @staticmethod
    @once_differentiable
    def backward(ctx, g):
        qkv, qb, bias_table, out, lse, bias_exp = ctx.saved_tensors
        groups, lse_off, C, nH, ws, shift, scale = ctx.meta
        g = _chk(g, BF16, "g")
        ready = 1 if bias_exp is not None else 0
        dqkv = torch.empty_like(qkv)
        dtable, first = _acc(("attn_t", bias_table.data_ptr()), tuple(bias_table.shape), qkv.device)
        dqb, _ = _acc(("attn_b", bias_table.data_ptr()), (3 * C,), qkv.device)
        bws = bias_exp if ready else torch.empty(nH * ATTN_WS_FLOATS, dtype=F32, device=qkv.device)
        for (B, H, W, r0), lo in zip(groups, lse_off):
            _lib.call("esvit_window_attn_bwd", _po(qkv, r0 * 3 * C), _p(qb), _p(bias_table), _p(bws), ready, _po(out, r0 * C),
                      _po(g, r0 * C), _po(lse, lo), _po(dqkv, r0 * 3 * C), _p(dtable), _p(dqb), B, H, W, C, nH, ws, shift,
                      scale, _stream())
        return dqkv, (dqb if first else None), (dtable if first else None), None, None, None, None, None, None


class PatchMergeLNGroupsFn(Function):

    @staticmethod
    def forward(ctx, x, gamma, beta, eps: float, groups):
        x, gamma, beta = _chk(x, F32, "x"), _chk(gamma, F32, "gamma"), _chk(beta, F32, "beta")
        T, C = x.shape
        assert sum(B * H * W for B, H, W, _ in groups) == T
        out_off, n = [], 0
        for B, H, W, _ in groups:
            out_off.append(n)
            n += B * ((H + 1) // 2) * ((W + 1) // 2)
        y = torch.empty(n, 4 * C, dtype=BF16, device=x.device)
        mean = torch.empty(n, dtype=F32, device=x.device)
        rstd = torch.empty(n, dtype=F32, device=x.device)
        for (B, H, W, r0), o0 in zip(groups, out_off):
            _lib.call("esvit_patch_merge_ln_fwd", _po(x, r0 * C), _p(gamma), _p(beta), eps, _po(y, o0 * 4 * C), _po(mean, o0),
                      _po(rstd, o0), B, H, W, C, _stream())
        ctx.save_for_backward(x, mean, rstd, gamma)
        ctx.meta = (tuple(groups), tuple(out_off))
        return y

    @staticmethod
    @once_differentiable
    def backward(ctx, g):
        x, mean, rstd, gamma = ctx.saved_tensors
        groups, out_off = ctx.meta
        T, C = x.shape
        g = _chk(g, BF16, "g")
        dx = torch.empty_like(x)
        acc, first = _acc(("merge", gamma.data_ptr()), (2, gamma.numel()), x.device)
        for (B, H, W, r0), o0 in zip(groups, out_off):
            _lib.call("esvit_patch_merge_ln_bwd", _po(g, o0 * 4 * C), _po(x, r0 * C), _po(mean, o0), _po(rstd, o0), _p(gamma),
                      _po(dx, r0 * C), _p(acc[0]), _p(acc[1]), B, H, W, C, _stream())
        return (dx, acc[0], acc[1], None, None) if first else (dx, None, None, None, None)


class TokenMeanGroupsFn(Function):

    @staticmethod
    def forward(ctx, region, groups):
        region = _chk(region, F32, "region")
        T, C = region.shape
        nb = sum(B for B, _, _, _ in groups)
        pooled = torch.empty(nb, C, dtype=F32, device=region.device)
        b0 = 0
        for B, H, W, r0 in groups:
            _lib.call("esvit_token_mean_fwd", _po(region, r0 * C), _po(pooled, b0 * C), B, H * W, C, _stream())
            b0 += B
        ctx.meta = (tuple(groups), T, C)
        return pooled

    @staticmethod
    @once_differentiable
    def backward(ctx, g):
        groups, T, C = ctx.meta
        g = _chk(g, F32, "g")
        d = torch.empty(T, C, dtype=F32, device=g.device)
        b0 = 0
        for B, H, W, r0 in groups:
            _lib.call("esvit_token_mean_bwd", _po(g, b0 * C), None, _po(d, r0 * C), B, H * W, C, _stream())
            b0 += B
        return d, None


class MhsaGroupsFn(Function):

    @staticmethod
    def forward(ctx, qkv, qkv_bias, groups, num_heads: int, scale: float):
        qkv = _chk(qkv, BF16, "qkv")
        T, C3 = qkv.shape
        C = C3 // 3
        if sum(B * L for B, L, _ in groups) != T:
            raise ValueError(f"groups {groups} do not cover the {T} rows of qkv")
        out = torch.empty(T, C, dtype=BF16, device=qkv.device)
        lse = torch.empty(T * num_heads, dtype=F32, device=qkv.device)
        for B, L, r0 in groups:
            _lib.call("esvit_mhsa_fwd", _po(qkv, r0 * C3), _po(out, r0 * C), _po(lse, r0 * num_heads), B, L, C, num_heads,
                      scale, _stream())
        ctx.save_for_backward(qkv, out, lse)
        ctx.meta = (tuple(groups), num_heads, scale, qkv_bias is not None)
        return out

    @staticmethod
    @once_differentiable
    def backward(ctx, g):
        qkv, out, lse = ctx.saved_tensors
        groups, nH, scale, has_bias = ctx.meta
        g = _chk(g, BF16, "g")
        T, C3 = qkv.shape
        C = C3 // 3
        dqkv = torch.empty_like(qkv)
        dvec = torch.empty_like(lse)
        for B, L, r0 in groups:
            _lib.call("esvit_mhsa_bwd", _po(qkv, r0 * C3), _po(out, r0 * C), _po(g, r0 * C), _po(lse, r0 * nH),
                      _po(dvec, r0 * nH), _po(dqkv, r0 * C3), B, L, C, nH, scale, _stream())
        return dqkv, (colsum(dqkv) if has_bias else None), None, None, None


def mhsa(qkv: Tensor, num_heads: int, scale: float) -> Tuple[Tensor, Tensor]:
    qkv = _chk(qkv, BF16, "qkv")
    B, L, C3 = qkv.shape
    out = torch.empty(B * L, C3 // 3, dtype=BF16, device=qkv.device)
    lse = torch.empty(B, num_heads, L, dtype=F32, device=qkv.device)
    _lib.call("esvit_mhsa_fwd", _p(qkv), _p(out), _p(lse), B, L, C3 // 3, num_heads, scale, _stream())
    return out, lse


def vit_patches(imgs: Sequence[Tensor], p: int) -> Tensor:
    imgs = [_chk(im, F32, "img") for im in imgs]
    rows = [im.shape[0] * (im.shape[2] // p) * (im.shape[3] // p) for im in imgs]
    out = torch.empty(sum(rows), 3 * p * p, dtype=BF16, device=imgs[0].device)
    r0 = 0
    for im, n in zip(imgs, rows):
        B, Cin, H, W = im.shape
        if Cin != 3 or H != W or H % p != 0:
            raise ValueError(f"expected square crops [B, 3, S, S] with S a multiple of {p}, got {tuple(im.shape)}")
        _lib.call("esvit_vit_patches", _p(im), _po(out, r0 * 3 * p * p), B, H, p, _stream())
        r0 += n
    return out


class VitTokensGroupsFn(Function):

    @staticmethod
    def forward(ctx, pe, bias, cls_token, groups, *pos):
        pe, cls = _chk(pe, BF16, "pe"), _chk(cls_token, F32, "cls_token")
        pos = [_chk(q, F32, "pos_embed") for q in pos]
        D = pe.shape[-1]
        T = sum(B * (N + 1) for B, N in groups)
        x = torch.empty(T, D, dtype=F32, device=pe.device)
        p0 = x0 = 0
        for (B, N), q in zip(groups, pos):
            if q.numel() != (N + 1) * D:
                raise ValueError(f"pos_embed of {q.numel()} values for {N} patches of width {D}")
            _lib.call("esvit_vit_tokens_fwd", _po(pe, p0 * D), _p(cls), _p(q), _po(x, x0 * D), B, N, D, _stream())
            p0 += B * N
            x0 += B * (N + 1)
        ctx.meta = (tuple(groups), D, pe.shape[0], tuple(tuple(q.shape) for q in pos))
        return x

    @staticmethod
    @once_differentiable
    def backward(ctx, g):
        groups, D, npe, pos_shapes = ctx.meta
        g = _chk(g, F32, "g")
        dpe = torch.empty(npe, D, dtype=BF16, device=g.device)
        dbias = torch.empty(D, dtype=F32, device=g.device)
        dcls = torch.empty(1, 1, D, dtype=F32, device=g.device)
        dpos, p0, x0 = [], 0, 0
        for gi, ((B, N), shp) in enumerate(zip(groups, pos_shapes)):
            d = torch.empty(shp, dtype=F32, device=g.device)
            _lib.call("esvit_vit_tokens_bwd", _po(g, x0 * D), _po(dpe, p0 * D), _p(d), _p(dbias), _p(dcls),
                      1 if gi else 0, B, N, D, _stream())
            dpos.append(d)
            p0 += B * N
            x0 += B * (N + 1)
        return (dpe, dbias, dcls, None) + tuple(dpos)


class VitSplitGroupsFn(Function):

    @staticmethod
    def forward(ctx, x, groups):
        x = _chk(x, F32, "x")
        D = x.shape[-1]
        nb = sum(B for B, _ in groups)
        cls = torch.empty(nb, D, dtype=F32, device=x.device)
        region = torch.empty(sum(B * N for B, N in groups), D, dtype=F32, device=x.device)
        _vit_split(x, cls, region, groups, 0)
        ctx.meta = (tuple(groups), tuple(x.shape))
        return cls, region

    @staticmethod
    @once_differentiable
    def backward(ctx, g_cls, g_region):
        groups, shape = ctx.meta
        g_cls = _chk(g_cls, F32, "g_cls")
        g_region = _chk(g_region, F32, "g_region")
        dx = torch.empty(shape, dtype=F32, device=(g_cls if g_cls is not None else g_region).device)
        _vit_split(dx, g_cls, g_region, groups, 1)
        return dx, None


def _vit_split(x, cls, region, groups, direction):
    D = x.shape[-1]
    x0 = b0 = q0 = 0
    for B, N in groups:
        _lib.call("esvit_vit_split", _po(x, x0 * D), _po(cls, b0 * D) if cls is not None else None,
                  _po(region, q0 * D) if region is not None else None, B, N, D, direction, _stream())
        x0 += B * (N + 1)
        b0 += B
        q0 += B * N


@torch.no_grad()
def window_attention_probs(qkv: Tensor, qkv_bias: Tensor, bias_table: Tensor, H: int, W: int, num_heads: int, ws: int,
                           shift: int, scale: float, bias_exp: Optional[Tensor] = None) -> Tensor:
    qkv = _chk(qkv, BF16, "qkv")
    qkv_bias = _chk(qkv_bias, F32, "qkv_bias")
    bias_table = _chk(bias_table.detach(), F32, "relative_position_bias_table")
    B, L, C3 = qkv.shape
    if L != H * W:
        raise ValueError(f"qkv has {L} tokens per sample, expected H * W = {H * W}")
    C = C3 // 3
    qb = shadow.lookup(qkv_bias)
    if qb is None:
        qb = qkv_bias.detach().to(BF16)
    nwin = B * (-(-H // ws)) * (-(-W // ws))
    probs = torch.empty(nwin, num_heads, ws * ws, ws * ws, dtype=F32, device=qkv.device)
    ready = 1 if (bias_exp is not None and ws == 7) else 0
    bws = bias_exp if ready else torch.empty(num_heads * ATTN_WS_FLOATS, dtype=F32, device=qkv.device)
    _lib.call("esvit_window_attn_probs", _p(qkv), _p(qb), _p(bias_table), _p(bws), ready, _p(probs), B, H, W, C,
              num_heads, ws, shift, scale, _stream())
    return probs


def expand_rel_pos_bias(bias_table: Tensor, num_heads: int, ws: int) -> Optional[Tensor]:
    if ws != 7:
        return None
    bias_table = _chk(bias_table.detach(), F32, "relative_position_bias_table")
    bws = torch.empty(num_heads * 4096, dtype=F32, device=bias_table.device)
    _lib.call("esvit_window_attn_expand_bias", _p(bias_table), _p(bws), num_heads, ws, _stream())
    return bws


class GeluFn(Function):
    @staticmethod
    def forward(ctx, x):
        x = _chk(x, BF16, "x")
        y = torch.empty_like(x)
        _lib.call("esvit_gelu_fwd", _p(x), _p(y), x.numel(), _stream())
        ctx.save_for_backward(x)
        return y

    @staticmethod
    @once_differentiable
    def backward(ctx, g):
        (x,) = ctx.saved_tensors
        g = _chk(g, BF16, "g")
        dx = torch.empty_like(x)
        _lib.call("esvit_gelu_bwd", _p(x), _p(g), _p(dx), x.numel(), _stream())
        return dx


class BiasGeluFn(Function):

    @staticmethod
    def forward(ctx, x, bias):
        x = _chk(x, BF16, "x")
        y = torch.empty_like(x)
        _lib.call("esvit_gelu_fwd", _p(x), _p(y), x.numel(), _stream())
        ctx.save_for_backward(x)
        ctx.bias_meta = (bias.shape, bias.device, bias.data_ptr())
        return y

    @staticmethod
    @once_differentiable
    def backward(ctx, g):
        (x,) = ctx.saved_tensors
        g = _chk(g, BF16, "g")
        N = x.shape[-1]
        dx = torch.empty_like(x)
        db, first = _acc(("bias", ctx.bias_meta[2]), tuple(ctx.bias_meta[0]), ctx.bias_meta[1])
        _lib.call("esvit_gelu_bwd_dbias", _p(x), _p(g), _p(dx), _p(db), x.numel() // N, N, _stream())
        return dx, (db if first else None)


GEMM_COLSUM_WS_ROWS = 160


def gemm_bias_act(a: Tensor, w: Tensor, bias: Optional[Tensor], act: int = 0, want_pre: bool = False):
    a, w = _chk(a, BF16, "a"), _chk(w, BF16, "w")
    bias = _chk(bias, F32, "bias")
    K = a.shape[-1]
    M = a.numel() // K
    N = w.shape[0]
    out = torch.empty(*a.shape[:-1], N, dtype=BF16, device=a.device)
    pre = torch.empty_like(out) if (act and want_pre) else None
    _lib.call("esvit_gemm_bias_act", _p(a), _p(w), _p(bias), _p(out), _p(pre), M, N, K, act, _stream())
    return (out, pre) if (act and want_pre) else out


def gemm(a: Tensor, b: Tensor, bias: Optional[Tensor] = None, act: int = 0, want_pre: bool = False, a_mn: bool = False,
         b_mn: bool = False, tile: int = 0):
    a, b = _chk(a, BF16, "a"), _chk(b, BF16, "b")
    bias = _chk(bias, F32, "bias")
    if a_mn:
        K, M = a.shape
        lead = (M,)
    else:
        K = a.shape[-1]
        M = a.numel() // K
        lead = tuple(a.shape[:-1])
    N = b.shape[1] if b_mn else b.shape[0]
    assert (b.shape[0] if b_mn else b.shape[1]) == K, (a.shape, b.shape)
    out = torch.empty(*lead, N, dtype=BF16, device=a.device)
    pre = torch.empty_like(out) if (act and want_pre) else None
    _lib.call("esvit_gemm_bf16", _p(a), _p(b), _p(bias), _p(out), _p(pre), M, N, K, 1 if a_mn else 0, 1 if b_mn else 0, act,
              tile, _stream())
    return (out, pre) if (act and want_pre) else out


def gemm_mul_colsum(a: Tensor, b: Tensor, mult: Tensor, colsum: Tensor, b_mn: bool = False, tile: int = 0) -> Tensor:
    a, b, mult = _chk(a, BF16, "a"), _chk(b, BF16, "b"), _chk(mult, BF16, "mult")
    K = a.shape[-1]
    M = a.numel() // K
    N = b.shape[1] if b_mn else b.shape[0]
    out = torch.empty_like(mult)
    ws = torch.empty(GEMM_COLSUM_WS_ROWS * N, dtype=F32, device=a.device)
    _lib.call("esvit_gemm_mul_colsum2", _p(a), _p(b), _p(mult), _p(out), _p(colsum), _p(ws), M, N, K, 1 if b_mn else 0, tile,
              _stream())
    return out


MLP_FUSED_C = (96, 128, 192)


def mlp_fwd(x: Tensor, w1: Tensor, b1: Optional[Tensor], w2: Tensor, b2: Optional[Tensor], want_h: bool = False):
    x, w1, w2 = _chk(x, BF16, "x"), _chk(w1, BF16, "w1"), _chk(w2, BF16, "w2")
    b1, b2 = _chk(b1, F32, "b1"), _chk(b2, F32, "b2")
    C = x.shape[-1]
    M = x.numel() // C
    assert tuple(w1.shape) == (4 * C, C) and tuple(w2.shape) == (C, 4 * C), (x.shape, w1.shape, w2.shape)
    y = torch.empty_like(x)
    h = torch.empty(*x.shape[:-1], 4 * C, dtype=BF16, device=x.device) if want_h else None
    pre = torch.empty_like(h) if want_h else None
    _lib.call("esvit_mlp_fwd", _p(x), _p(w1), _p(b1), _p(w2), _p(b2), _p(y), _p(h), _p(pre), M, C, _stream())
    return (y, h, pre) if want_h else y


_wgrad_ws = {}


def gemm_wgrad(dy: Tensor, x: Tensor, out: Optional[Tensor] = None, accumulate: bool = False, tile: int = 0) -> Tensor:
    dy, x = _chk(dy, BF16, "dy"), _chk(x, BF16, "x")
    N, K = dy.shape[-1], x.shape[-1]
    T = dy.numel() // N
    assert x.numel() // K == T
    if out is None:
        out = torch.empty(N, K, dtype=F32, device=dy.device)
        accumulate = False
    key = (dy.device, N, K)
    ws = _wgrad_ws.get(key)
    if ws is None:
        n = _lib.load().esvit_gemm_wgrad_ws_floats(N, K)
        if n <= 0:
            raise ValueError("esvit_gemm_wgrad: weight too large for the split-K workspace")
        ws = _wgrad_ws[key] = torch.empty(n, dtype=F32, device=dy.device)
    _lib.call("esvit_gemm_wgrad", _p(dy), _p(x), _p(out), _p(ws), T, N, K, 1 if accumulate else 0, tile, _stream())
    return out


class LinearGeluFn(Function):

    @staticmethod
    def forward(ctx, x, w, bias):
        out, pre = gemm_bias_act(x, w, bias, act=1, want_pre=True)
        ctx.save_for_backward(x, w, pre)
        ctx.bias_meta = (bias.shape, bias.device, bias.data_ptr())
        return out

    @staticmethod
    @once_differentiable
    def backward(ctx, g):
        x, w, pre = ctx.saved_tensors
        g = _chk(g, BF16, "g")
        N = pre.shape[-1]
        dh = torch.empty_like(pre)
        db, first = _acc(("bias", ctx.bias_meta[2]), tuple(ctx.bias_meta[0]), ctx.bias_meta[1])
        _lib.call("esvit_mul_bwd_dbias", _p(pre), _p(g), _p(dh), _p(db), pre.numel() // N, N, _stream())
        dh2 = dh.reshape(-1, N)
        dx = (dh2 @ w).view(x.shape) if ctx.needs_input_grad[0] else None
        dw = dh2.t() @ x.reshape(-1, x.shape[-1]) if ctx.needs_input_grad[1] else None
        return dx, dw, (db if first else None)




class MlpFn(Function):

    @staticmethod
    def forward(ctx, x, w1, b1, w2, b2, w2t):
        h, pre = gemm_bias_act(x, w1, b1, act=1, want_pre=True)
        with torch.autocast("cuda", enabled=False):
            y = torch.nn.functional.linear(h, w2, b2)
        ctx.save_for_backward(x, w1, pre, h, w2t)
        ctx.bias_meta = (b1.shape, b1.device, b1.data_ptr())
        return y

    @staticmethod
    @once_differentiable
    def backward(ctx, g):
        x, w1, pre, h, w2t = ctx.saved_tensors
        g = _chk(g, BF16, "g")
        C, N = g.shape[-1], pre.shape[-1]
        g2 = g.reshape(-1, C)
        M = g2.shape[0]
        dw2 = g2.t() @ h.reshape(-1, N) if ctx.needs_input_grad[3] else None
        dpre = torch.empty_like(pre)
        db1, first = _acc(("bias", ctx.bias_meta[2]), tuple(ctx.bias_meta[0]), ctx.bias_meta[1])
        ws = torch.empty(GEMM_COLSUM_WS_ROWS * N, dtype=F32, device=g.device)
        _lib.call("esvit_gemm_mul_colsum", _p(g2), _p(w2t), _p(pre), _p(dpre), _p(db1), _p(ws), M, N, C, _stream())
        d2 = dpre.reshape(-1, N)
        dx = (d2 @ w1).view(x.shape) if ctx.needs_input_grad[0] else None
        dw1 = d2.t() @ x.reshape(-1, x.shape[-1]) if ctx.needs_input_grad[1] else None
        return dx, dw1, (db1 if first else None), dw2, None, None


class LinearBiasFn(Function):

    @staticmethod
    def forward(ctx, x, w, b):
        ctx.save_for_backward(x, w)
        with torch.autocast("cuda", enabled=False):
            return torch.nn.functional.linear(x, w, b)

    @staticmethod
    @once_differentiable
    def backward(ctx, g):
        x, w = ctx.saved_tensors
        g2 = g.reshape(-1, g.shape[-1])
        dx = (g2 @ w).view(x.shape) if ctx.needs_input_grad[0] else None
        dw = g2.t() @ x.reshape(-1, x.shape[-1]) if ctx.needs_input_grad[1] else None
        return dx, dw, None


class L2NormFn(Function):
    @staticmethod
    def forward(ctx, x, eps: float):
        x = _chk(x, BF16, "x")
        R, Dm = x.numel() // x.shape[-1], x.shape[-1]
        y = torch.empty_like(x)
        inv = torch.empty(R, dtype=F32, device=x.device)
        _lib.call("esvit_l2norm_fwd", _p(x), _p(y), _p(inv), eps, R, Dm, _stream())
        ctx.save_for_backward(x, inv)
        return y

    @staticmethod
    @once_differentiable
    def backward(ctx, g):
        x, inv = ctx.saved_tensors
        g = _chk(g, BF16, "g")
        R, Dm = x.numel() // x.shape[-1], x.shape[-1]
        dx = torch.empty_like(x)
        _lib.call("esvit_l2norm_bwd", _p(x), _p(g), _p(inv), _p(dx), R, Dm, _stream())
        return dx, None


class WeightNormFn(Function):

    @staticmethod
    def forward(ctx, v, g):
        v, g = _chk(v, F32, "weight_v"), _chk(g, F32, "weight_g")
        K, Dm = v.shape
        w = torch.empty(K, Dm, dtype=BF16, device=v.device)
        norm = torch.empty(K, dtype=F32, device=v.device)
        _lib.call("esvit_weight_norm_fwd", _p(v), _p(g), _p(w), _p(norm), K, Dm, _stream())
        ctx.save_for_backward(v, g, norm)
        return w

    @staticmethod
    @once_differentiable
    def backward(ctx, gw):
        v, g, norm = ctx.saved_tensors
        f32 = gw.dtype == F32
        gw = _chk(gw, F32 if f32 else BF16, "gw")
        K, Dm = v.shape
        dv = torch.empty_like(v)
        dg = torch.empty_like(g) if ctx.needs_input_grad[1] else None
        _lib.call("esvit_weight_norm_bwd", _p(v), _p(g), _p(norm), _p(gw), 1 if f32 else 0, _p(dv), _p(dg), K, Dm, _stream())
        return dv, dg




def row_lse(x: Tensor, center: Optional[Tensor], inv_temp: float) -> Tensor:
    x = _chk(x, BF16, "logits")
    R, K = x.shape
    lse = torch.empty(R, dtype=F32, device=x.device)
    _lib.call("esvit_row_lse", _p(x), _p(center), inv_temp, _p(lse), R, K, _stream())
    return lse


def ce_q_enabled(K: int) -> bool:
    import os
    return os.environ.get("ESVIT_CE_Q", "1") != "0" and K <= _lib.load().esvit_row_softmax_q_max_k()


def row_softmax_q(x: Tensor, center: Tensor, inv_temp: float) -> Tuple[Tensor, Tensor]:
    x, center = _chk(x, BF16, "teacher logits"), _chk(center, F32, "center")
    R, K = x.shape
    lse = torch.empty(R, dtype=F32, device=x.device)
    q = torch.empty(R, K, dtype=torch.float16, device=x.device)
    _lib.call("esvit_row_softmax_q", _p(x), _p(center), inv_temp, _p(lse), _p(q), R, K, _stream())
    return lse, q


def _ce_q_fwd(s: Tensor, q: Tensor, trow: Tensor, order: Optional[Tensor], w: Tensor,
              inv_tau_s: float) -> Tuple[Tensor, Tensor]:
    R, K = s.shape
    lse_s = torch.empty(R, dtype=F32, device=s.device)
    row_loss = torch.empty(R, dtype=F32, device=s.device)
    _lib.call("esvit_dino_ce_q_fwd", _p(s), _p(q), _p(lse_s), _p(trow), _p(order), inv_tau_s, _p(row_loss), R, K,
              _stream())
    loss = torch.empty((), dtype=F32, device=s.device)
    _lib.call("esvit_weighted_sum", _p(row_loss), _p(w), R, _p(loss), _stream())
    return loss, lse_s


def _ce_q_bwd(s, q, lse_s, trow, w, order, gs, inv_tau_s: float) -> Tensor:
    R, K = s.shape
    ds = torch.empty_like(s)
    _lib.call("esvit_dino_ce_q_bwd", _p(s), _p(q), _p(lse_s), _p(trow), _p(order), _p(w), _p(gs), inv_tau_s, _p(ds),
              R, K, _stream())
    return ds


class DinoCEFn(Function):

    @staticmethod
    def forward(ctx, s, t, center, lse_t, trow, w, inv_temp_t: float, inv_tau_s: float, order=None):
        s, t = _chk(s, BF16, "student logits"), _chk(t, BF16, "teacher logits")
        center, w = _chk(center, F32, "center"), _chk(w, F32, "w")
        trow = _chk(trow, torch.int32, "trow")
        order = _chk(order, torch.int32, "order")
        ctx.use_q = lse_t is None
        ctx.temps = (inv_temp_t, inv_tau_s)
        if ctx.use_q:
            _, q = row_softmax_q(t, center, inv_temp_t)
            loss, lse_s = _ce_q_fwd(s, q, trow, order, w, inv_tau_s)
            ctx.save_for_backward(s, q, lse_s, trow, w, order)
            return loss
        R, K = s.shape
        lse_s = torch.empty(R, dtype=F32, device=s.device)
        row_loss = torch.empty(R, dtype=F32, device=s.device)
        lse_t = _chk(lse_t, F32, "lse_t")
        _lib.call("esvit_dino_ce_fwd", _p(s), _p(t), _p(center), _p(lse_s), _p(lse_t), _p(trow), _p(order), inv_temp_t,
                  inv_tau_s, _p(row_loss), R, K, _stream())
        ctx.save_for_backward(s, t, center, lse_s, lse_t, trow, w, order)
        loss = torch.empty((), dtype=F32, device=s.device)
        _lib.call("esvit_weighted_sum", _p(row_loss), _p(w), R, _p(loss), _stream())
        return loss

    @staticmethod
    @once_differentiable
    def backward(ctx, g):
        inv_temp_t, inv_tau_s = ctx.temps
        gs = _chk(g.reshape(1).to(F32), F32, "g")
        if ctx.use_q:
            ds = _ce_q_bwd(*ctx.saved_tensors, gs, inv_tau_s)
        else:
            s, t, center, lse_s, lse_t, trow, w, order = ctx.saved_tensors
            R, K = s.shape
            ds = torch.empty_like(s)
            _lib.call("esvit_dino_ce_bwd", _p(s), _p(t), _p(center), _p(lse_s), _p(lse_t), _p(trow), _p(order), _p(w),
                      _p(gs), inv_temp_t, inv_tau_s, _p(ds), R, K, _stream())
        return ds, None, None, None, None, None, None, None, None


def mixup_q(q: Tensor, targets: Tensor, w_scale: float) -> Tuple[Tensor, Tensor]:
    q, targets = _chk(q, torch.float16, "teacher probabilities"), _chk(targets, F32, "mixup targets")
    ncrops, B, B2 = targets.shape
    Rt, K = q.shape
    if B2 != B or Rt != 2 * B:
        raise ValueError(f"mixup targets {tuple(targets.shape)} do not fit {Rt} teacher rows")
    R = ncrops * B
    ws = torch.empty(2 * R * _lib.load().esvit_mixup_q_kpad(B), dtype=torch.float16, device=q.device)
    w = torch.empty(R, dtype=F32, device=q.device)
    q_hat = torch.empty(R, K, dtype=torch.float16, device=q.device)
    _lib.call("esvit_mixup_q", _p(targets), _p(q), ncrops, B, K, w_scale, _p(ws), _p(w), _p(q_hat), _stream())
    return q_hat, w


class DinoCEQFn(Function):

    @staticmethod
    def forward(ctx, s, q, trow, w, inv_tau_s: float):
        s, q = _chk(s, BF16, "student logits"), _chk(q, torch.float16, "teacher probabilities")
        trow, w = _chk(trow, torch.int32, "trow"), _chk(w, F32, "w")
        loss, lse_s = _ce_q_fwd(s, q, trow, None, w, inv_tau_s)
        ctx.save_for_backward(s, q, lse_s, trow, w)
        ctx.inv_tau_s = inv_tau_s
        return loss

    @staticmethod
    @once_differentiable
    def backward(ctx, g):
        s, q, lse_s, trow, w = ctx.saved_tensors
        gs = _chk(g.reshape(1).to(F32), F32, "g")
        return _ce_q_bwd(s, q, lse_s, trow, w, None, gs, ctx.inv_tau_s), None, None, None, None


_colsum_ws = {}


def colsum(t: Tensor, out: Optional[Tensor] = None) -> Tensor:
    t = _chk(t, BF16, "teacher logits")
    R, K = t.shape
    key = (t.device, K)
    ws = _colsum_ws.get(key)
    if ws is None:
        rows = _lib.load().esvit_colsum_workspace_rows()
        ws = _colsum_ws[key] = torch.empty(rows * K, dtype=F32, device=t.device)
    if out is None:
        out = torch.empty(K, dtype=F32, device=t.device)
    _lib.call("esvit_colsum", _p(t), R, K, _p(ws), _p(out), _stream())
    return out


def center_ema(center: Tensor, colsum_total: Tensor, rows_total: int, momentum: float,
               out: Optional[Tensor] = None) -> Tensor:
    assert center.is_cuda and center.dtype == F32 and center.is_contiguous()
    if out is None:
        out = torch.empty_like(center)
    _lib.call("esvit_center_ema", _p(center), _p(colsum_total), float(rows_total), momentum, _p(out), center.numel(),
              _stream())
    return out


def normalize_rows(x: Tensor, eps: float = 1e-12) -> Tensor:
    x = _chk(x, F32, "features")
    y = torch.empty_like(x)
    _lib.call("esvit_normalize_rows", _p(x), _p(y), x.shape[0], x.shape[1], eps, _stream())
    return y


def region_match(s_fea: Tensor, t_fea: Tensor, B: int, ncrops: int, Tg: int, Tl: int) -> Tuple[Tensor, Tensor]:
    sn, tn = normalize_rows(s_fea), normalize_rows(t_fea)
    P = sn.shape[1]
    Rs = sn.shape[0]
    assert Rs == B * (2 * Tg + (ncrops - 2) * Tl) and tn.shape[0] == 2 * B * Tg
    idx = torch.full((2, ncrops, B, Tg), -1, dtype=torch.int64, device=sn.device)
    trow = torch.empty(Rs, 2, dtype=torch.int32, device=sn.device)
    _lib.call("esvit_region_match", _p(sn), _p(tn), B, ncrops, Tg, Tl, P, _p(idx), _p(trow), _stream())
    return idx, trow




def win_padded(H: int, W: int, w: int) -> Tuple[int, int]:
    return -(-H // w) * w, -(-W // w) * w


def conv_out_size(S: int, k: int, stride: int, pad: int) -> int:
    return (S + 2 * pad - k) // stride + 1


class ConvEmbedFn(Function):

    @staticmethod
    def forward(ctx, x, weight, w16, bias, imgs, groups, k: int, stride: int, pad: int):
        w16 = _chk(w16, BF16, "w16")
        Cout, Kp = w16.shape
        Cin = weight.shape[1]
        if imgs is not None:
            src = [(_chk(im, F32, "img"), 1, im.shape[0], im.shape[2], im.shape[3]) for im in imgs]
        else:
            x = _chk(x, F32, "x")
            src = [(x, 0, B, H, W, r0) for B, H, W, r0 in groups]
        n = [s[2] * conv_out_size(s[3], k, stride, pad) * conv_out_size(s[4], k, stride, pad) for s in src]
        rows = torch.empty(sum(n), Kp, dtype=BF16, device=w16.device)
        r0 = 0
        for s, ni in zip(src, n):
            t, nchw, B, H, W = s[:5]
            base = _p(t) if nchw else _po(t, s[5] * Cin)
            _lib.call("esvit_conv_im2col", base, _po(rows, r0 * Kp), nchw, B, Cin, H, W, k, stride, pad, Kp, _stream())
            r0 += ni
        y = gemm(rows, w16, bias)
        ctx.save_for_backward(rows, w16)
        ctx.meta = (tuple(weight.shape), None if imgs is not None else (tuple(x.shape), tuple(groups)), k, stride, pad)
        return y

    @staticmethod
    @once_differentiable
    def backward(ctx, g):
        rows, w16 = ctx.saved_tensors
        wshape, xmeta, k, stride, pad = ctx.meta
        g = _chk(g, BF16, "g")
        Cout, Cin = wshape[0], wshape[1]
        K = Cin * k * k
        dw = None
        if ctx.needs_input_grad[1]:
            dw = gemm_wgrad(g, rows)
            dw = (dw[:, :K].contiguous() if dw.shape[1] != K else dw).view(wshape)
        dx = None
        if xmeta is not None and ctx.needs_input_grad[0]:
            xshape, groups = xmeta
            drows = gemm(g, w16, None, b_mn=True)
            Kp = drows.shape[1]
            dx = torch.empty(xshape, dtype=F32, device=g.device)
            o0 = 0
            for B, H, W, r0 in groups:
                _lib.call("esvit_conv_col2im", _po(drows, o0 * Kp), _po(dx, r0 * Cin), B, Cin, H, W, k, stride, pad, Kp,
                          _stream())
                o0 += B * conv_out_size(H, k, stride, pad) * conv_out_size(W, k, stride, pad)
        return dx, dw, None, None, None, None, None, None, None


def _bn_part(groups, C: int, device) -> Tensor:
    n = max(-(-(B * Hp * Wp) // 256) for B, H, W, w, _, _ in groups for Hp, Wp in (win_padded(H, W, w),))
    return torch.empty(n * 9 * C, dtype=F32, device=device)


class DwBnFn(Function):

    @staticmethod
    def forward(ctx, y, weight, gamma, beta, bn, groups, train: bool, pg):
        y = _chk(y, BF16, "y")
        w = _chk(weight, F32, "weight").view(-1, 9)
        gamma, beta = _chk(gamma, F32, "gamma"), _chk(beta, F32, "beta")
        C = y.shape[1]
        Tp = sum(B * Hp * Wp for B, H, W, w_, _, _ in groups for Hp, Wp in (win_padded(H, W, w_),))
        z = torch.empty(Tp, C, dtype=BF16, device=y.device)
        out = torch.empty_like(z)
        part = _bn_part(groups, C, y.device)
        sums = torch.empty(len(groups), 2 * C + 1, dtype=torch.float64, device=y.device)
        stat = torch.empty(len(groups), 4 * C, dtype=F32, device=y.device)
        rm, rv, nbt = bn.running_mean, bn.running_var, bn.num_batches_tracked
        for i, (B, H, W, w_, r0, p0) in enumerate(groups):
            Hp, Wp = win_padded(H, W, w_)
            _lib.call("esvit_dwbn_fwd_stats", _po(y, r0 * C), _p(w), _po(z, p0 * C), _p(part), _p(sums[i]), B, H, W,
                      Hp, Wp, C, _stream())
            if train and pg is not None:
                torch.distributed.all_reduce(sums[i], group=pg)
            _lib.call("esvit_dwbn_fwd_apply", _po(z, p0 * C), _p(gamma), _p(beta), _p(sums[i]) if train else None,
                      _p(rm), _p(rv), _p(nbt) if (train and nbt is not None) else None, _p(stat[i]), _po(out, p0 * C),
                      B * Hp * Wp, C, 1 if train else 0, float(bn.momentum), float(bn.eps), _stream())
        ctx.save_for_backward(y, z, w, stat)
        ctx.meta = (tuple(groups), train, pg, tuple(weight.shape), gamma.data_ptr(), weight.data_ptr())
        return out

    @staticmethod
    @once_differentiable
    def backward(ctx, g):
        y, z, w, stat = ctx.saved_tensors
        groups, train, pg, wshape, gptr, wptr = ctx.meta
        g = _chk(g, BF16, "g")
        C = y.shape[1]
        dy = torch.empty_like(y)
        part = _bn_part(groups, C, y.device)
        bsums = torch.empty(2 * C + 1, dtype=torch.float64, device=y.device)
        coef = torch.empty(3 * C, dtype=F32, device=y.device)
        dwt, first_w = _acc(("dw", wptr), wshape, y.device)
        aff, first_a = _acc(("bn", gptr), (2, C), y.device)
        for i, (B, H, W, w_, r0, p0) in enumerate(groups):
            Hp, Wp = win_padded(H, W, w_)
            N = B * Hp * Wp
            _lib.call("esvit_dwbn_bwd_stats", _po(g, p0 * C), _po(z, p0 * C), _p(stat[i]), _p(part), _p(bsums),
                      _p(aff[0]), _p(aff[1]), N, C, _stream())
            if train and pg is not None:
                torch.distributed.all_reduce(bsums, group=pg)
            _lib.call("esvit_dwbn_bwd_apply", _po(g, p0 * C), _po(z, p0 * C), _po(y, r0 * C), _p(w), _p(stat[i]),
                      _p(bsums), _p(coef), _po(dy, r0 * C), _p(part), _p(dwt), B, H, W, Hp, Wp, C, 1 if train else 0,
                      _stream())
        return (dy, dwt if first_w else None, aff[0] if first_a else None, aff[1] if first_a else None,
                None, None, None, None)


class MhsaWinGroupsFn(Function):

    @staticmethod
    def forward(ctx, qkv, qkv_bias, groups, num_heads: int, scale: float):
        qkv = _chk(qkv, BF16, "qkv")
        Tp, C3 = qkv.shape
        C = C3 // 3
        T = sum(B * H * W for B, H, W, _, _, _ in groups)
        out = torch.empty(T, C, dtype=BF16, device=qkv.device)
        lse = torch.empty(Tp * num_heads, dtype=F32, device=qkv.device)
        for B, H, W, w, r0, p0 in groups:
            _lib.call("esvit_mhsa_win_fwd", _po(qkv, p0 * C3), _po(out, r0 * C), _po(lse, p0 * num_heads), B, H, W, w, C,
                      num_heads, scale, _stream())
        ctx.save_for_backward(qkv, out, lse)
        ctx.meta = (tuple(groups), num_heads, scale, qkv_bias is not None)
        return out

    @staticmethod
    @once_differentiable
    def backward(ctx, g):
        qkv, out, lse = ctx.saved_tensors
        groups, nH, scale, has_bias = ctx.meta
        g = _chk(g, BF16, "g")
        C3 = qkv.shape[1]
        C = C3 // 3
        dqkv = torch.empty_like(qkv)
        dvec = torch.empty_like(lse)
        for B, H, W, w, r0, p0 in groups:
            _lib.call("esvit_mhsa_win_bwd", _po(qkv, p0 * C3), _po(out, r0 * C), _po(g, r0 * C), _po(lse, p0 * nH),
                      _po(dvec, p0 * nH), _po(dqkv, p0 * C3), B, H, W, w, C, nH, scale, _stream())
        return dqkv, (colsum(dqkv) if has_bias else None), None, None, None


VIL_W = 7
VIL_NB = 1 + 9 * VIL_W * VIL_W
_vil_ws = {}


class SlidingChunkAttnFn(Function):

    @staticmethod
    def forward(ctx, q, kv, bias, bias_g, mode, B: int, nx: int, ny: int, num_heads: int, scale: float):
        q = _chk(q, BF16, "q")
        kv = _chk(kv, BF16, "kv")
        bias = _chk(bias, F32, "bias").contiguous()
        bias_g = _chk(bias_g, F32, "bias_g").contiguous()
        mode = _chk(mode, torch.int32, "mode")
        N, C = 1 + nx * ny, 32 * num_heads
        if q.shape != (B * N, C) or kv.shape != (B * N, 2 * C) or not q.is_contiguous() or not kv.is_contiguous():
            raise ValueError(f"q [B*N, C] = [{B * N}, {C}] and kv [B*N, 2C] contiguous required, got "
                             f"{tuple(q.shape)}, {tuple(kv.shape)}")
        if bias.shape != (num_heads, VIL_W * VIL_W, VIL_NB) or bias_g.shape != (num_heads, N) or mode.numel() != 1:
            raise ValueError("bias [nH, 49, 442], bias_g [nH, N] and a one-element mode required")
        mx, my = -(-nx // VIL_W), -(-ny // VIL_W)
        out = torch.empty(B * N, C, dtype=BF16, device=q.device)
        lse = torch.empty(B * num_heads * mx * my * VIL_W * VIL_W, dtype=F32, device=q.device)
        lse_g = torch.empty(B * num_heads, dtype=F32, device=q.device)
        _lib.call("esvit_vil_sc_fwd", _p(q), _p(kv), _p(bias), _p(bias_g), _p(mode), _p(out), _p(lse), _p(lse_g), B, nx,
                  ny, num_heads, scale, _stream())
        ctx.save_for_backward(q, kv, bias, bias_g, mode, out, lse, lse_g)
        ctx.meta = (B, nx, ny, num_heads, scale)
        return out

    @staticmethod
    @once_differentiable
    def backward(ctx, g):
        q, kv, bias, bias_g, mode, out, lse, lse_g = ctx.saved_tensors
        B, nx, ny, nH, scale = ctx.meta
        g = _chk(g, BF16, "g").contiguous()
        ws = _vil_sc_ws(q.device, B, nx, ny, nH)
        dq, dkv = torch.empty_like(q), torch.empty_like(kv)
        dvec = torch.empty_like(lse)
        dbias, dbias_g = torch.empty_like(bias), torch.empty_like(bias_g)
        _lib.call("esvit_vil_sc_bwd", _p(q), _p(kv), _p(bias), _p(bias_g), _p(mode), _p(out), _p(g), _p(lse), _p(lse_g),
                  _p(dvec), _p(ws), _p(dq), _p(dkv), _p(dbias), _p(dbias_g), B, nx, ny, nH, scale, _stream())
        return dq, dkv, dbias, dbias_g, None, None, None, None, None, None


def _vil_sc_ws(device, B: int, nx: int, ny: int, nH: int) -> Tensor:
    key = (device, B, nx, ny, nH)
    ws = _vil_ws.get(key)
    if ws is None:
        n = _lib.load().esvit_vil_sc_ws_floats(B, nx, ny, nH)
        if n <= 0:
            raise ValueError("esvit_vil_sc_bwd: problem too large for the workspace")
        ws = _vil_ws[key] = torch.empty(n, dtype=F32, device=device)
    return ws


class SlidingChunkAttnGroupsFn(Function):

    @staticmethod
    def forward(ctx, q, kv, q_bias, kv_bias, bias, modes, groups, num_heads: int, scale: float):
        q, kv = _chk(q, BF16, "q"), _chk(kv, BF16, "kv")
        bias = _chk(bias, F32, "bias")
        modes = _chk(modes, torch.int32, "modes")
        T, C = q.shape
        if C != 32 * num_heads or kv.shape != (T, 2 * C):
            raise ValueError(f"q [T, 32 nH] and kv [T, 2C] required, got {tuple(q.shape)}, {tuple(kv.shape)}")
        if sum(B * (1 + nx * ny) for B, nx, ny, _, _, _ in groups) != T or modes.numel() != len(groups):
            raise ValueError(f"groups {groups} do not cover the {T} rows, or not one mode per group")
        out = torch.empty(T, C, dtype=BF16, device=q.device)
        lse_off, lse_g_off, n, ng = [], [], 0, 0
        for B, nx, ny, _, _, _ in groups:
            lse_off.append(n)
            lse_g_off.append(ng)
            n += B * num_heads * (-(-nx // VIL_W)) * (-(-ny // VIL_W)) * VIL_W * VIL_W
            ng += B * num_heads
        lse = torch.empty(n, dtype=F32, device=q.device)
        lse_g = torch.empty(ng, dtype=F32, device=q.device)
        for gi, ((B, nx, ny, r0, bo, bgo), lo, lgo) in enumerate(zip(groups, lse_off, lse_g_off)):
            _lib.call("esvit_vil_sc_fwd", _po(q, r0 * C), _po(kv, r0 * 2 * C), _po(bias, bo), _po(bias, bgo),
                      _po(modes, gi), _po(out, r0 * C), _po(lse, lo), _po(lse_g, lgo), B, nx, ny, num_heads, scale,
                      _stream())
        ctx.save_for_backward(q, kv, bias, modes, out, lse, lse_g)
        ctx.meta = (tuple(groups), tuple(lse_off), tuple(lse_g_off), num_heads, scale, q_bias is not None,
                    kv_bias is not None)
        return out

    @staticmethod
    @once_differentiable
    def backward(ctx, g):
        q, kv, bias, modes, out, lse, lse_g = ctx.saved_tensors
        groups, lse_off, lse_g_off, nH, scale, has_qb, has_kvb = ctx.meta
        g = _chk(g, BF16, "g")
        C = q.shape[1]
        dq, dkv = torch.empty_like(q), torch.empty_like(kv)
        dvec = torch.empty_like(lse)
        dbias = torch.zeros_like(bias)
        for gi, ((B, nx, ny, r0, bo, bgo), lo, lgo) in enumerate(zip(groups, lse_off, lse_g_off)):
            ws = _vil_sc_ws(q.device, B, nx, ny, nH)
            _lib.call("esvit_vil_sc_bwd", _po(q, r0 * C), _po(kv, r0 * 2 * C), _po(bias, bo), _po(bias, bgo),
                      _po(modes, gi), _po(out, r0 * C), _po(g, r0 * C), _po(lse, lo), _po(lse_g, lgo), _po(dvec, lo),
                      _p(ws), _po(dq, r0 * C), _po(dkv, r0 * 2 * C), _po(dbias, bo), _po(dbias, bgo), B, nx, ny, nH,
                      scale, _stream())
        return (dq, dkv, colsum(dq) if has_qb else None, colsum(dkv) if has_kvb else None, dbias,
                None, None, None, None)


class DenseBiasAttnGroupsFn(Function):

    @staticmethod
    def forward(ctx, qkv, qkv_bias, bias, groups, num_heads: int, scale: float):
        qkv, bias = _chk(qkv, BF16, "qkv"), _chk(bias, F32, "bias")
        T, C3 = qkv.shape
        C = C3 // 3
        if sum(B * L for B, L, _, _ in groups) != T:
            raise ValueError(f"groups {groups} do not cover the {T} rows of qkv")
        out = torch.empty(T, C, dtype=BF16, device=qkv.device)
        lse = torch.empty(T * num_heads, dtype=F32, device=qkv.device)
        for B, L, r0, bo in groups:
            _lib.call("esvit_vil_dense_fwd", _po(qkv, r0 * C3), _po(bias, bo), _po(out, r0 * C), _po(lse, r0 * num_heads),
                      B, L, C, num_heads, scale, _stream())
        ctx.save_for_backward(qkv, bias, out, lse)
        ctx.meta = (tuple(groups), num_heads, scale, qkv_bias is not None)
        return out

    @staticmethod
    @once_differentiable
    def backward(ctx, g):
        qkv, bias, out, lse = ctx.saved_tensors
        groups, nH, scale, has_bias = ctx.meta
        g = _chk(g, BF16, "g")
        C = qkv.shape[1] // 3
        dqkv = torch.empty_like(qkv)
        dvec = torch.empty_like(lse)
        dbias = torch.zeros_like(bias)
        lib = _lib.load()
        for B, L, r0, bo in groups:
            part = torch.empty(lib.esvit_vil_dense_parts(B) * nH * L * L, dtype=F32, device=qkv.device)
            _lib.call("esvit_vil_dense_bwd", _po(qkv, r0 * 3 * C), _po(bias, bo), _po(out, r0 * C), _po(g, r0 * C),
                      _po(lse, r0 * nH), _po(dvec, r0 * nH), _p(part), _po(dqkv, r0 * 3 * C), _po(dbias, bo), B, L, C, nH,
                      scale, _stream())
        return dqkv, (colsum(dqkv) if has_bias else None), dbias, None, None, None


def vil_dense_attention(qkv: Tensor, bias: Tensor, num_heads: int, scale: float) -> Tuple[Tensor, Tensor]:
    qkv, bias = _chk(qkv, BF16, "qkv"), _chk(bias, F32, "bias")
    B, L, C3 = qkv.shape
    out = torch.empty(B * L, C3 // 3, dtype=BF16, device=qkv.device)
    lse = torch.empty(B, num_heads, L, dtype=F32, device=qkv.device)
    _lib.call("esvit_vil_dense_fwd", _p(qkv), _p(bias), _p(out), _p(lse), B, L, C3 // 3, num_heads, scale, _stream())
    return out, lse


class VilStreamEmbedFn(Function):

    @staticmethod
    def forward(ctx, x, weight, w16, bias, groups, p: int):
        x, w16 = _chk(x, F32, "x"), _chk(w16, BF16, "w16")
        Cout, Kp = w16.shape
        Cin = x.shape[1]
        if tuple(weight.shape) != (Cout, Cin, p, p):
            raise ValueError(f"weight {tuple(weight.shape)} is not [{Cout}, {Cin}, {p}, {p}]")
        n = [B * (H // p) * (W // p) for B, N, off, H, W, r0 in groups]
        alloc = torch.empty if Kp == Cin * p * p else torch.zeros
        rows = alloc(sum(n), Kp, dtype=BF16, device=x.device)
        o0 = 0
        for (B, N, off, H, W, r0), ni in zip(groups, n):
            _lib.call("esvit_vil_im2col", _po(x, r0 * Cin), _po(rows, o0 * Kp), B, N, off, Cin, H, W, p, Kp, _stream())
            o0 += ni
        y = gemm(rows, w16, bias)
        ctx.save_for_backward(rows, w16)
        ctx.meta = (tuple(weight.shape), tuple(x.shape), tuple(groups), tuple(n), p)
        return y

    @staticmethod
    @once_differentiable
    def backward(ctx, g):
        rows, w16 = ctx.saved_tensors
        wshape, xshape, groups, n, p = ctx.meta
        g = _chk(g, BF16, "g")
        K = wshape[1] * p * p
        dw = None
        if ctx.needs_input_grad[1]:
            dw = gemm_wgrad(g, rows)
            dw = (dw[:, :K].contiguous() if dw.shape[1] != K else dw).view(wshape)
        dx = None
        if ctx.needs_input_grad[0]:
            drows = gemm(g, w16, None, b_mn=True)
            Kp, Cin = drows.shape[1], xshape[1]
            dx = torch.empty(xshape, dtype=F32, device=g.device)
            o0 = 0
            for (B, N, off, H, W, r0), ni in zip(groups, n):
                _lib.call("esvit_vil_col2im", _po(drows, o0 * Kp), _po(dx, r0 * Cin), B, N, off, Cin, H, W, p, Kp,
                          _stream())
                o0 += ni
        return dx, dw, None, None, None, None


class ClsCatGroupsFn(Function):

    @staticmethod
    def forward(ctx, y, cls_token, groups):
        y, cls = _chk(y, F32, "y"), _chk(cls_token, F32, "cls_token")
        C = y.shape[1]
        out = torch.empty(sum(B * (1 + n) for B, n in groups), C, dtype=F32, device=y.device)
        y0 = x0 = 0
        for B, n in groups:
            _lib.call("esvit_vil_cls_cat_fwd", _po(y, y0 * C), _p(cls), _po(out, x0 * C), B, n, C, _stream())
            y0 += B * n
            x0 += B * (1 + n)
        ctx.meta = (tuple(groups), tuple(y.shape), tuple(cls_token.shape))
        return out

    @staticmethod
    @once_differentiable
    def backward(ctx, g):
        groups, yshape, cshape = ctx.meta
        g = _chk(g, F32, "g")
        C = yshape[1]
        dy = torch.empty(yshape, dtype=F32, device=g.device)
        dcls = torch.empty(cshape, dtype=F32, device=g.device)
        y0 = x0 = 0
        for gi, (B, n) in enumerate(groups):
            _lib.call("esvit_vil_cls_cat_bwd", _po(g, x0 * C), _po(dy, y0 * C), _p(dcls), B, n, C, 1 if gi else 0,
                      _stream())
            y0 += B * n
            x0 += B * (1 + n)
        return dy, dcls, None


class RelBiasFn(Function):

    @staticmethod
    def forward(ctx, table, g2l, g2g, plan):
        table = _chk(table, F32, "table")
        g2l, g2g = _chk(g2l, F32, "g2l"), _chk(g2g, F32, "g2g")
        (rp, col, val), _, nrows = plan
        n0, n1 = table.numel(), (g2l.numel() if g2l is not None else 0)
        y = torch.empty(nrows, dtype=F32, device=table.device)
        _lib.call("esvit_vil_bias_spmv", _p(rp), _p(col), _p(val), _p(table), _p(g2l), _p(g2g), n0, n1, _p(y), nrows,
                  _stream())
        ctx.plan = plan
        ctx.shapes = (tuple(table.shape), None if g2l is None else tuple(g2l.shape),
                      None if g2g is None else tuple(g2g.shape))
        return y

    @staticmethod
    @once_differentiable
    def backward(ctx, g):
        g = _chk(g, F32, "g")
        _, (rp, col, val), _ = ctx.plan
        shapes = ctx.shapes
        sizes = [0 if s is None else int(torch.Size(s).numel()) for s in shapes]
        d = torch.empty(sum(sizes), dtype=F32, device=g.device)
        _lib.call("esvit_vil_bias_spmv", _p(rp), _p(col), _p(val), _p(g), None, None, g.numel(), 0, _p(d), d.numel(),
                  _stream())
        out, o = [], 0
        for s, n in zip(shapes, sizes):
            out.append(None if s is None else d[o:o + n].view(s))
            o += n
        return out[0], out[1], out[2], None




def _ptr_array(tensors: Sequence[Tensor]):
    arr = (ctypes.c_void_p * len(tensors))()
    for i, t in enumerate(tensors):
        arr[i] = t.data_ptr()
    return arr


def _numel_array(tensors: Sequence[Tensor]):
    arr = (ctypes.c_longlong * len(tensors))()
    for i, t in enumerate(tensors):
        arr[i] = t.numel()
    return arr


def ema_update_(teacher: Sequence[Tensor], student: Sequence[Tensor], momentum: float) -> None:
    assert len(teacher) == len(student)
    for k, q in zip(teacher, student):
        if not (k.is_cuda and q.is_cuda and k.dtype == F32 and q.dtype == F32 and k.is_contiguous()
                and q.is_contiguous() and k.numel() == q.numel()):
            raise RuntimeError("ema_update_: fp32 contiguous CUDA tensors of equal size required")
    _lib.call("esvit_ema_multi", _ptr_array(teacher), _ptr_array(student), _numel_array(teacher), len(teacher),
              float(momentum), _stream())


def clip_grads_(grads: Sequence[Tensor], clip: float) -> Tensor:
    n = len(grads)
    dev = grads[0].device
    for g in grads:
        if not (g.is_cuda and g.dtype == F32 and g.is_contiguous()):
            raise RuntimeError("clip_grads_: fp32 contiguous CUDA gradients required")
    ws = torch.empty(n, dtype=torch.float64, device=dev)
    norms = torch.empty(n, dtype=F32, device=dev)
    _lib.call("esvit_clip_multi", _ptr_array(grads), _numel_array(grads), n, float(clip), _p(ws), _p(norms), _stream())
    return norms
```

include/esvit_b200.h:

```cpp
#ifndef ESVIT_B200_H
#define ESVIT_B200_H

#ifdef __cplusplus
extern "C" {
#endif

#define ESVIT_ERR_BAD_ARG 1001

int esvit_add_ln_fwd(const float* x, const void* delta, const float* keep, int tokens_per_sample,
                     const float* gamma, const float* beta, float eps, float* xout, void* y, int y_is_bf16,
                     float* mean, float* rstd, long long T, int C, void* stream);
int esvit_add_ln_bwd(const void* dy, int dy_is_bf16, const float* dxo, const float* xs, const float* mean,
                     const float* rstd, const float* gamma, const float* keep, int tokens_per_sample, float* dx,
                     void* ddelta, float* dgamma, float* dbeta, float* ddelta_bias, long long T, int C, void* stream);

int esvit_patch_merge_ln_fwd(const float* x, const float* gamma, const float* beta, float eps, void* y, float* mean,
                             float* rstd, int B, int H, int W, int C, void* stream);
int esvit_patch_merge_ln_bwd(const void* dy, const float* x, const float* mean, const float* rstd,
                             const float* gamma, float* dx, float* dgamma, float* dbeta, int B, int H, int W, int C,
                             void* stream);

int esvit_token_mean_fwd(const float* region, float* pooled, int B, int N, int C, void* stream);
int esvit_token_mean_bwd(const float* dpooled, const float* dregion_in, float* dregion, int B, int N, int C,
                         void* stream);

int esvit_patch_embed_fwd(const float* img, const float* w, const float* bias, const float* gamma, const float* beta,
                          float eps, float* out, float* mean, float* rstd, int B, int H, int W, int E, void* stream);
int esvit_patch_embed_bwd(const float* img, const float* w, const float* bias, const float* gamma, const float* mean,
                          const float* rstd, const float* dout, float* dw, float* dbias, float* dgamma, float* dbeta,
                          int B, int H, int W, int E, void* stream);

int esvit_window_attn_expand_bias(const float* bias_table, float* bias_ws, int nH, int ws, void* stream);
int esvit_window_attn_fwd(const void* qkv, const void* qkv_bias, const float* bias_table, float* bias_ws, int bias_ready,
                          void* out, float* lse, int B, int H, int W, int C, int nH, int ws, int shift, float scale,
                          void* stream);
int esvit_window_attn_bwd(const void* qkv, const void* qkv_bias, const float* bias_table, float* bias_ws, int bias_ready,
                          const void* out, const void* dout, const float* lse, void* dqkv, float* dbias_table,
                          float* dqkv_bias, int B, int H, int W, int C, int nH, int ws, int shift, float scale,
                          void* stream);
int esvit_window_attn_probs(const void* qkv, const void* qkv_bias, const float* bias_table, float* bias_ws, int bias_ready,
                            float* probs, int B, int H, int W, int C, int nH, int ws, int shift, float scale, void* stream);

int esvit_gemm_bias_act(const void* a, const void* w, const float* bias, void* out, void* pre, long long M, int N, int K,
                        int act, void* stream);
int esvit_gemm_mul_colsum(const void* a, const void* w, const void* mult, void* out, float* colsum, float* ws,
                          long long M, int N, int K, void* stream);

int esvit_gemm_bf16(const void* a, const void* b, const float* bias, void* out, void* pre, long long M, int N, int K,
                    int a_mn, int b_mn, int act, int tile, void* stream);
int esvit_gemm_mul_colsum2(const void* a, const void* b, const void* mult, void* out, float* colsum, float* ws,
                           long long M, int N, int K, int b_mn, int tile, void* stream);
int esvit_gemm_wgrad_ws_floats(int N, int K);
int esvit_gemm_wgrad(const void* dy, const void* x, float* dw, float* ws, long long T, int N, int K, int accumulate,
                     int tile, void* stream);
int esvit_mlp_fwd(const void* x, const void* w1, const float* b1, const void* w2, const float* b2, void* y, void* h,
                  void* gelu_grad, long long M, int C, void* stream);

int esvit_gelu_fwd(const void* x, void* y, long long n, void* stream);
int esvit_gelu_bwd(const void* x, const void* dy, void* dx, long long n, void* stream);
int esvit_gelu_bwd_dbias(const void* x, const void* dy, void* dx, float* dbias, long long R, int N, void* stream);
int esvit_mul_bwd_dbias(const void* gp, const void* dy, void* dx, float* dbias, long long R, int N, void* stream);

int esvit_l2norm_fwd(const void* x, void* y, float* inv, float eps, long long R, int D, void* stream);
int esvit_l2norm_bwd(const void* x, const void* dy, const float* inv, void* dx, long long R, int D, void* stream);
int esvit_weight_norm_fwd(const float* v, const float* g, void* w, float* norm, long long K, int D, void* stream);
int esvit_weight_norm_bwd(const float* v, const float* g, const float* norm, const void* dw, int dw_is_f32, float* dv,
                          float* dg, long long K, int D, void* stream);

int esvit_row_lse(const void* x, const float* center, float inv_temp, float* lse, long long R, int K, void* stream);
int esvit_dino_ce_fwd(const void* s, const void* t, const float* center, float* lse_s, const float* lse_t,
                      const int* trow, const int* order, float inv_temp_t, float inv_tau_s, float* row_loss, long long R,
                      int K, void* stream);
int esvit_dino_ce_bwd(const void* s, const void* t, const float* center, const float* lse_s, const float* lse_t,
                      const int* trow, const int* order, const float* w, const float* gscale, float inv_temp_t,
                      float inv_tau_s, void* ds, long long R, int K, void* stream);
int esvit_weighted_sum(const float* v, const float* w, int R, float* out, void* stream);
int esvit_row_softmax_q_max_k(void);
int esvit_row_softmax_q(const void* x, const float* center, float inv_temp, float* lse, void* q, long long R, int K,
                        void* stream);
int esvit_dino_ce_q_fwd(const void* s, const void* q, float* lse_s, const int* trow, const int* order, float inv_tau_s,
                        float* row_loss, long long R, int K, void* stream);
int esvit_dino_ce_q_bwd(const void* s, const void* q, const float* lse_s, const int* trow, const int* order,
                        const float* w, const float* gscale, float inv_tau_s, void* ds, long long R, int K, void* stream);
int esvit_mixup_q_kpad(int B);
int esvit_mixup_q(const float* targets, const void* q, int ncrops, int B, int K, float w_scale, void* ws, float* w,
                  void* q_out, void* stream);

int esvit_colsum_workspace_rows(void);
int esvit_colsum(const void* t, long long R, int K, float* workspace, float* out, void* stream);
int esvit_center_ema(const float* center, const float* colsum, float rows_total, float momentum, float* center_out,
                     int K, void* stream);

int esvit_normalize_rows(const float* x, float* y, long long R, int P, float eps, void* stream);
int esvit_region_match(const float* sn, const float* tn, int B, int ncrops, int Tg, int Tl, int P,
                       long long* idx_out, int* trow, void* stream);

int esvit_mhsa_fwd(const void* qkv, void* out, float* lse, int B, int L, int C, int nH, float scale, void* stream);
int esvit_mhsa_bwd(const void* qkv, const void* out, const void* dout, const float* lse, float* dvec, void* dqkv,
                   int B, int L, int C, int nH, float scale, void* stream);

int esvit_vit_patches(const float* img, void* patches, int B, int S, int p, void* stream);
int esvit_vit_tokens_fwd(const void* pe, const float* cls, const float* pos, float* x, int B, int N, int D, void* stream);
int esvit_vit_tokens_bwd(const float* g, void* dpe, float* dpos, float* dbias, float* dcls, int accumulate, int B, int N,
                         int D, void* stream);
int esvit_vit_split(float* x, float* cls, float* region, int B, int N, int D, int dir, void* stream);

int esvit_conv_im2col(const float* x, void* rows, int nchw, int B, int C, int H, int W, int k, int stride, int pad, int Kp,
                      void* stream);
int esvit_conv_col2im(const void* rows, float* dx, int B, int C, int H, int W, int k, int stride, int pad, int Kp,
                      void* stream);
int esvit_mhsa_win_fwd(const void* qkv, void* out, float* lse, int B, int H, int W, int w, int C, int nH, float scale,
                       void* stream);
int esvit_mhsa_win_bwd(const void* qkv, const void* out, const void* dout, const float* lse, float* dvec, void* dqkv,
                       int B, int H, int W, int w, int C, int nH, float scale, void* stream);
int esvit_dwbn_fwd_stats(const void* y, const float* w, void* z, float* part, double* sums, int B, int H, int W, int Hp,
                         int Wp, int C, void* stream);
int esvit_dwbn_fwd_apply(const void* z, const float* gamma, const float* beta, const double* sums, float* run_mean,
                         float* run_var, long long* nbt, float* stat, void* out, long long N, int C, int train,
                         float momentum, float eps, void* stream);
int esvit_dwbn_bwd_stats(const void* dy, const void* z, const float* stat, float* part, double* sums, float* dgamma,
                         float* dbeta, long long N, int C, void* stream);
int esvit_dwbn_bwd_apply(const void* dy, const void* z, const void* y, const float* w, const float* stat,
                         const double* sums, float* coef, void* dx, float* part, float* dw, int B, int H, int W, int Hp,
                         int Wp, int C, int train, void* stream);

int esvit_vil_sc_ws_floats(int B, int nx, int ny, int nH);
int esvit_vil_sc_fwd(const void* q, const void* kv, const float* bias, const float* bias_g, const int* mode, void* out,
                     float* lse, float* lse_g, int B, int nx, int ny, int nH, float scale, void* stream);
int esvit_vil_sc_bwd(const void* q, const void* kv, const float* bias, const float* bias_g, const int* mode,
                     const void* out, const void* dout, const float* lse, const float* lse_g, float* dvec, float* ws,
                     void* dq, void* dkv, float* dbias, float* dbias_g, int B, int nx, int ny, int nH, float scale,
                     void* stream);

int esvit_vil_dense_parts(int B);
int esvit_vil_dense_fwd(const void* qkv, const float* bias, void* out, float* lse, int B, int L, int C, int nH,
                        float scale, void* stream);
int esvit_vil_dense_bwd(const void* qkv, const float* bias, const void* out, const void* dout, const float* lse,
                        float* dvec, float* part, void* dqkv, float* dbias, int B, int L, int C, int nH, float scale,
                        void* stream);
int esvit_vil_im2col(const float* x, void* rows, int B, int N, int off, int Cin, int H, int W, int p, int Kp,
                     void* stream);
int esvit_vil_col2im(const void* drows, float* dx, int B, int N, int off, int Cin, int H, int W, int p, int Kp,
                     void* stream);
int esvit_vil_cls_cat_fwd(const float* y, const float* cls, float* out, int B, int n, int C, void* stream);
int esvit_vil_cls_cat_bwd(const float* g, float* dy, float* dcls, int B, int n, int C, int accumulate, void* stream);
int esvit_vil_bias_spmv(const int* rowptr, const int* col, const float* val, const float* s0, const float* s1,
                        const float* s2, int n0, int n1, float* y, int nrows, void* stream);

int esvit_ema_multi(void* const* teacher, const void* const* student, const long long* numel, int n, double momentum,
                    void* stream);
int esvit_clip_multi(void* const* grads, const long long* numel, int n, float clip, double* sumsq_ws, float* norms,
                     void* stream);
int esvit_grad_sumsq_multi(void* const* grads, const long long* numel, int n, double* sumsq, void* stream);
int esvit_adamw_ema_multi(void* const* params, const void* const* grads, void* const* exp_avg, void* const* exp_avg_sq,
                          void* const* teacher, void* const* param_bf16, void* const* teacher_bf16,
                          const long long* numel, int n, const float* hyper, float* state, const double* sumsq,
                          void* stream);

int esvit_knn_prep(const float* x, void* xb, float* norm, float* max_norm, long long R, long long R_pad, int D,
                   void* stream);
int esvit_knn_select(const void* S, long long ld, const float* a, const float* b, const float* a_norm,
                     const float* max_norm, const int* rows, int nrows, int N, int D, int k, int cap, int* cand_idx,
                     float* cand_val, int* count, float* sims, long long* idx, void* stream);
int esvit_knn_vote(const float* sims, const long long* idx, const long long* train_labels, const long long* test_labels,
                   long long M, int k, float T, int num_classes, long long* hits, void* stream);

int esvit_augment_coeffs(const double* params, const long long* meta, int* coef, int ncrops, int max_S, void* stream);
int esvit_augment_resize_h(const unsigned char* src, const double* params, const long long* meta, const int* coef,
                           unsigned char* tmp, int ncrops, long long max_pixels, void* stream);
int esvit_augment_color(const double* params, const long long* meta, const int* coef, const unsigned char* tmp,
                        const float* norm, int crop0, int ncrops, int S, void* stream);

int esvit_augment_eval_coeffs(const double* rec, const long long* meta, int* coef, int nimg, int S, void* stream);
int esvit_augment_eval_resize_h(const unsigned char* src, const double* rec, const long long* meta, const int* coef,
                                unsigned char* tmp, int nimg, int S, long long max_pixels, void* stream);
int esvit_augment_eval_resize_v(const long long* meta, const int* coef, const unsigned char* tmp, const float* norm,
                                float* out, int nimg, int S, void* stream);

#ifdef __cplusplus
}
#endif
#endif
```

Measured before the change: 1364.

## Fuse MLP backward with recompute of GELU pre-activation, drop saved gelu grad

The forward MLP no longer stores the GELU-gradient tensor and saves only the hidden activation. Backward calls a new warp-specialized wgmma kernel that recomputes x·W1+b1 on the fly, forms dpre from dy·W2ᵀ times the GELU derivative, and computes dx = dpre·W1 and the db1 column sums in the same pass. This removes a 4C-wide activation write and read plus separate GEMM launches. In exchange the first-layer GEMM runs again in backward, and a new kernel brings register and shared-memory pressure.

```diff
diff --git a/esvit_b200/_lib.py b/esvit_b200/_lib.py
--- a/esvit_b200/_lib.py
+++ b/esvit_b200/_lib.py
@@ -32,6 +32,9 @@
     "esvit_gemm_wgrad_ws_floats": [I, I],
     "esvit_gemm_wgrad": [P, P, P, P, L, I, I, I, I, P],
     "esvit_mlp_fwd": [P, P, P, P, P, P, P, P, L, I, P],
+    "esvit_mlp_bwd_ws_floats": [L, I],
+    "esvit_mlp_fwd_h": [P, P, P, P, P, P, P, L, I, P],
+    "esvit_mlp_bwd": [P, P, P, P, P, P, P, P, P, L, I, I, P],
     "esvit_gelu_fwd": [P, P, L, P],
     "esvit_gelu_bwd": [P, P, P, L, P],
     "esvit_gelu_bwd_dbias": [P, P, P, P, L, I, P],
@@ -137,7 +140,7 @@
 
 
 _LAUNCHES = {"esvit_colsum": 2, "esvit_gemm_mul_colsum": 2, "esvit_gemm_mul_colsum2": 2, "esvit_gemm_wgrad": 2,
-             "esvit_mixup_q": 2}
+             "esvit_mixup_q": 2, "esvit_mlp_bwd": 3}
 _launch_count = 0
 _timed_names = set()
 _timed_events = []
@@ -153,6 +156,8 @@
     "esvit_gemm_mul_colsum2": lambda a: {"M": int(a[6]), "N": int(a[7]), "K": int(a[8])},
     "esvit_gemm_wgrad": lambda a: {"T": int(a[4]), "N": int(a[5]), "K": int(a[6])},
     "esvit_mlp_fwd": lambda a: {"M": int(a[8]), "C": int(a[9]), "student": a[6] is not None and a[6].value is not None},
+    "esvit_mlp_fwd_h": lambda a: {"M": int(a[7]), "C": int(a[8]), "student": True},
+    "esvit_mlp_bwd": lambda a: {"M": int(a[9]), "C": int(a[10])},
     "esvit_add_ln_fwd": lambda a: {"T": int(a[-3]), "C": int(a[-2]), "has_x": a[0] is not None and a[0].value is not None,
                                    "has_delta": a[1] is not None and a[1].value is not None},
     "esvit_add_ln_bwd": lambda a: {"T": int(a[-3]), "C": int(a[-2])},
diff --git a/esvit_b200/csrc/gemm2_wgmma.cu b/esvit_b200/csrc/gemm2_wgmma.cu
--- a/esvit_b200/csrc/gemm2_wgmma.cu
+++ b/esvit_b200/csrc/gemm2_wgmma.cu
@@ -112,45 +112,49 @@
       : "l"(da), "l"(db), "r"(scale_d), "n"(TA), "n"(TB));
 }
 
+template <int TB = 0>
 __device__ __forceinline__ void wgmma_ss_n64(float (&d)[32], uint64_t da, uint64_t db, uint32_t scale_d) {
   asm volatile(
       "{\n\t.reg .pred p;\n\t"
       "setp.ne.b32 p, %34, 0;\n\t"
       "wgmma.mma_async.sync.aligned.m64n64k16.f32.bf16.bf16 "
       "{%0, %1, %2, %3, %4, %5, %6, %7, %8, %9, %10, %11, %12, %13, %14, %15, %16, %17, %18, %19, %20, %21, %22, %23, %24, %25, %26, %27, %28, %29, %30, %31}, "
-      "%32, %33, p, 1, 1, 0, 0;\n\t}\n"
+      "%32, %33, p, 1, 1, 0, %35;\n\t}\n"
       : "+f"(d[0]), "+f"(d[1]), "+f"(d[2]), "+f"(d[3]), "+f"(d[4]), "+f"(d[5]), "+f"(d[6]), "+f"(d[7]), "+f"(d[8]), "+f"(d[9]), "+f"(d[10]), "+f"(d[11]), "+f"(d[12]), "+f"(d[13]), "+f"(d[14]), "+f"(d[15]), "+f"(d[16]), "+f"(d[17]), "+f"(d[18]), "+f"(d[19]), "+f"(d[20]), "+f"(d[21]), "+f"(d[22]), "+f"(d[23]), "+f"(d[24]), "+f"(d[25]), "+f"(d[26]), "+f"(d[27]), "+f"(d[28]), "+f"(d[29]), "+f"(d[30]), "+f"(d[31])
-      : "l"(da), "l"(db), "r"(scale_d));
-}
+      : "l"(da), "l"(db), "r"(scale_d), "n"(TB));
+}
+template <int TB = 0>
 __device__ __forceinline__ void wgmma_rs(float (&d)[48], const uint32_t (&a)[4], uint64_t db, uint32_t scale_d) {
   asm volatile(
       "{\n\t.reg .pred p;\n\t"
       "setp.ne.b32 p, %53, 0;\n\t"
       "wgmma.mma_async.sync.aligned.m64n96k16.f32.bf16.bf16 "
       "{%0, %1, %2, %3, %4, %5, %6, %7, %8, %9, %10, %11, %12, %13, %14, %15, %16, %17, %18, %19, %20, %21, %22, %23, %24, %25, %26, %27, %28, %29, %30, %31, %32, %33, %34, %35, %36, %37, %38, %39, %40, %41, %42, %43, %44, %45, %46, %47}, "
-      "{%48, %49, %50, %51}, %52, p, 1, 1, 0;\n\t}\n"
+      "{%48, %49, %50, %51}, %52, p, 1, 1, %54;\n\t}\n"
       : "+f"(d[0]), "+f"(d[1]), "+f"(d[2]), "+f"(d[3]), "+f"(d[4]), "+f"(d[5]), "+f"(d[6]), "+f"(d[7]), "+f"(d[8]), "+f"(d[9]), "+f"(d[10]), "+f"(d[11]), "+f"(d[12]), "+f"(d[13]), "+f"(d[14]), "+f"(d[15]), "+f"(d[16]), "+f"(d[17]), "+f"(d[18]), "+f"(d[19]), "+f"(d[20]), "+f"(d[21]), "+f"(d[22]), "+f"(d[23]), "+f"(d[24]), "+f"(d[25]), "+f"(d[26]), "+f"(d[27]), "+f"(d[28]), "+f"(d[29]), "+f"(d[30]), "+f"(d[31]), "+f"(d[32]), "+f"(d[33]), "+f"(d[34]), "+f"(d[35]), "+f"(d[36]), "+f"(d[37]), "+f"(d[38]), "+f"(d[39]), "+f"(d[40]), "+f"(d[41]), "+f"(d[42]), "+f"(d[43]), "+f"(d[44]), "+f"(d[45]), "+f"(d[46]), "+f"(d[47])
-      : "r"(a[0]), "r"(a[1]), "r"(a[2]), "r"(a[3]), "l"(db), "r"(scale_d));
-}
+      : "r"(a[0]), "r"(a[1]), "r"(a[2]), "r"(a[3]), "l"(db), "r"(scale_d), "n"(TB));
+}
+template <int TB = 0>
 __device__ __forceinline__ void wgmma_rs(float (&d)[64], const uint32_t (&a)[4], uint64_t db, uint32_t scale_d) {
   asm volatile(
       "{\n\t.reg .pred p;\n\t"
       "setp.ne.b32 p, %69, 0;\n\t"
       "wgmma.mma_async.sync.aligned.m64n128k16.f32.bf16.bf16 "
       "{%0, %1, %2, %3, %4, %5, %6, %7, %8, %9, %10, %11, %12, %13, %14, %15, %16, %17, %18, %19, %20, %21, %22, %23, %24, %25, %26, %27, %28, %29, %30, %31, %32, %33, %34, %35, %36, %37, %38, %39, %40, %41, %42, %43, %44, %45, %46, %47, %48, %49, %50, %51, %52, %53, %54, %55, %56, %57, %58, %59, %60, %61, %62, %63}, "
-      "{%64, %65, %66, %67}, %68, p, 1, 1, 0;\n\t}\n"
+      "{%64, %65, %66, %67}, %68, p, 1, 1, %70;\n\t}\n"
       : "+f"(d[0]), "+f"(d[1]), "+f"(d[2]), "+f"(d[3]), "+f"(d[4]), "+f"(d[5]), "+f"(d[6]), "+f"(d[7]), "+f"(d[8]), "+f"(d[9]), "+f"(d[10]), "+f"(d[11]), "+f"(d[12]), "+f"(d[13]), "+f"(d[14]), "+f"(d[15]), "+f"(d[16]), "+f"(d[17]), "+f"(d[18]), "+f"(d[19]), "+f"(d[20]), "+f"(d[21]), "+f"(d[22]), "+f"(d[23]), "+f"(d[24]), "+f"(d[25]), "+f"(d[26]), "+f"(d[27]), "+f"(d[28]), "+f"(d[29]), "+f"(d[30]), "+f"(d[31]), "+f"(d[32]), "+f"(d[33]), "+f"(d[34]), "+f"(d[35]), "+f"(d[36]), "+f"(d[37]), "+f"(d[38]), "+f"(d[39]), "+f"(d[40]), "+f"(d[41]), "+f"(d[42]), "+f"(d[43]), "+f"(d[44]), "+f"(d[45]), "+f"(d[46]), "+f"(d[47]), "+f"(d[48]), "+f"(d[49]), "+f"(d[50]), "+f"(d[51]), "+f"(d[52]), "+f"(d[53]), "+f"(d[54]), "+f"(d[55]), "+f"(d[56]), "+f"(d[57]), "+f"(d[58]), "+f"(d[59]), "+f"(d[60]), "+f"(d[61]), "+f"(d[62]), "+f"(d[63])
-      : "r"(a[0]), "r"(a[1]), "r"(a[2]), "r"(a[3]), "l"(db), "r"(scale_d));
-}
+      : "r"(a[0]), "r"(a[1]), "r"(a[2]), "r"(a[3]), "l"(db), "r"(scale_d), "n"(TB));
+}
+template <int TB = 0>
 __device__ __forceinline__ void wgmma_rs(float (&d)[96], const uint32_t (&a)[4], uint64_t db, uint32_t scale_d) {
   asm volatile(
       "{\n\t.reg .pred p;\n\t"
       "setp.ne.b32 p, %101, 0;\n\t"
       "wgmma.mma_async.sync.aligned.m64n192k16.f32.bf16.bf16 "
       "{%0, %1, %2, %3, %4, %5, %6, %7, %8, %9, %10, %11, %12, %13, %14, %15, %16, %17, %18, %19, %20, %21, %22, %23, %24, %25, %26, %27, %28, %29, %30, %31, %32, %33, %34, %35, %36, %37, %38, %39, %40, %41, %42, %43, %44, %45, %46, %47, %48, %49, %50, %51, %52, %53, %54, %55, %56, %57, %58, %59, %60, %61, %62, %63, %64, %65, %66, %67, %68, %69, %70, %71, %72, %73, %74, %75, %76, %77, %78, %79, %80, %81, %82, %83, %84, %85, %86, %87, %88, %89, %90, %91, %92, %93, %94, %95}, "
-      "{%96, %97, %98, %99}, %100, p, 1, 1, 0;\n\t}\n"
+      "{%96, %97, %98, %99}, %100, p, 1, 1, %102;\n\t}\n"
       : "+f"(d[0]), "+f"(d[1]), "+f"(d[2]), "+f"(d[3]), "+f"(d[4]), "+f"(d[5]), "+f"(d[6]), "+f"(d[7]), "+f"(d[8]), "+f"(d[9]), "+f"(d[10]), "+f"(d[11]), "+f"(d[12]), "+f"(d[13]), "+f"(d[14]), "+f"(d[15]), "+f"(d[16]), "+f"(d[17]), "+f"(d[18]), "+f"(d[19]), "+f"(d[20]), "+f"(d[21]), "+f"(d[22]), "+f"(d[23]), "+f"(d[24]), "+f"(d[25]), "+f"(d[26]), "+f"(d[27]), "+f"(d[28]), "+f"(d[29]), "+f"(d[30]), "+f"(d[31]), "+f"(d[32]), "+f"(d[33]), "+f"(d[34]), "+f"(d[35]), "+f"(d[36]), "+f"(d[37]), "+f"(d[38]), "+f"(d[39]), "+f"(d[40]), "+f"(d[41]), "+f"(d[42]), "+f"(d[43]), "+f"(d[44]), "+f"(d[45]), "+f"(d[46]), "+f"(d[47]), "+f"(d[48]), "+f"(d[49]), "+f"(d[50]), "+f"(d[51]), "+f"(d[52]), "+f"(d[53]), "+f"(d[54]), "+f"(d[55]), "+f"(d[56]), "+f"(d[57]), "+f"(d[58]), "+f"(d[59]), "+f"(d[60]), "+f"(d[61]), "+f"(d[62]), "+f"(d[63]), "+f"(d[64]), "+f"(d[65]), "+f"(d[66]), "+f"(d[67]), "+f"(d[68]), "+f"(d[69]), "+f"(d[70]), "+f"(d[71]), "+f"(d[72]), "+f"(d[73]), "+f"(d[74]), "+f"(d[75]), "+f"(d[76]), "+f"(d[77]), "+f"(d[78]), "+f"(d[79]), "+f"(d[80]), "+f"(d[81]), "+f"(d[82]), "+f"(d[83]), "+f"(d[84]), "+f"(d[85]), "+f"(d[86]), "+f"(d[87]), "+f"(d[88]), "+f"(d[89]), "+f"(d[90]), "+f"(d[91]), "+f"(d[92]), "+f"(d[93]), "+f"(d[94]), "+f"(d[95])
-      : "r"(a[0]), "r"(a[1]), "r"(a[2]), "r"(a[3]), "l"(db), "r"(scale_d));
+      : "r"(a[0]), "r"(a[1]), "r"(a[2]), "r"(a[3]), "l"(db), "r"(scale_d), "n"(TB));
 }
 
 template <int BN, int TA, int TB>
@@ -523,6 +527,7 @@
   const float* b1;
   const float* b2;
   int M;
+  int store_g;
 };
 
 template <int C, bool STORE>
@@ -639,7 +644,7 @@
           if constexpr (STORE) {
             const uint32_t addr = hbuf + lrow + (((2 * s + lblk) ^ lsw) << 4);
             stmatrix_x4(addr, af[s][0], af[s][1], af[s][2], af[s][3]);
-            stmatrix_x4(addr + G::CHUNK_BYTES, d[0], d[1], d[2], d[3]);
+            if (p.store_g) stmatrix_x4(addr + G::CHUNK_BYTES, d[0], d[1], d[2], d[3]);
           }
         }
         if constexpr (STORE) fence_proxy_async();
@@ -654,7 +659,7 @@
             const int gr = m0 + 64 * wg;
             if (gr < p.M) {
               tma_store_2d(&map_h, hbuf, j * 64, gr);
-              tma_store_2d(&map_g, hbuf + G::CHUNK_BYTES, j * 64, gr);
+              if (p.store_g) tma_store_2d(&map_g, hbuf + G::CHUNK_BYTES, j * 64, gr);
             }
             bulk_commit();
           }
@@ -693,6 +698,255 @@
           if (gr < p.M) tma_store_2d(&map_y, buf, c * 64, gr);
           bulk_commit();
         }
+      }
+    }
+    if (t == 0) bulk_wait_all();
+  }
+}
+
+template <int C>
+struct MlpBwdCfg {
+  static constexpr int BM = 128, HB = 64;
+  static constexpr int KB = (C + 63) / 64;
+  static constexpr int NP = KB * 64;
+  static constexpr int NH = 4 * C / HB;
+  static constexpr int X_BYTES = KB * BM * 128;
+  static constexpr int W1_BYTES = KB * HB * 128;
+  static constexpr int W2_BYTES = C * 128;
+  static constexpr int STAGE_BYTES = W1_BYTES + W2_BYTES;
+  static constexpr int CHUNK_BYTES = BM * 128;
+  static constexpr int CS_BYTES = 2 * 8 * HB * 4;
+  static constexpr int BAR_BYTES = 128;
+  static constexpr int FIXED = 1024 + CS_BYTES + BAR_BYTES;
+  static constexpr bool fits(int nx, int ns) { return FIXED + 2 * nx * X_BYTES + 2 * STAGE_BYTES + ns * CHUNK_BYTES <= SMEM_LIMIT; }
+  static constexpr int NX = fits(2, 2) ? 2 : 1;
+  static constexpr int NS = fits(NX, 2) ? 2 : 1;
+  static constexpr int STAGES_RAW = (SMEM_LIMIT - FIXED - 2 * NX * X_BYTES - NS * CHUNK_BYTES) / STAGE_BYTES;
+  static constexpr int STAGES = STAGES_RAW > 4 ? 4 : STAGES_RAW;
+  static constexpr int SMEM = FIXED + 2 * NX * X_BYTES + STAGES * STAGE_BYTES + NS * CHUNK_BYTES;
+  static constexpr bool OVERLAP = NP <= 128;
+  static_assert(C % 32 == 0 && C <= 192, "acc2 [64 x NP] must fit the consumer registers");
+  static_assert(STAGES >= 2, "weight ring too shallow");
+  static_assert(SMEM <= SMEM_LIMIT, "shared memory budget");
+  static_assert((2 * STAGES + 2 * NX + 4) * 8 <= BAR_BYTES, "mbarrier area");
+};
+
+template <int C>
+__global__ void __launch_bounds__(384, 1) mlp_bwd_kernel(const __grid_constant__ CUtensorMap map_dy,
+                                                         const __grid_constant__ CUtensorMap map_x,
+                                                         const __grid_constant__ CUtensorMap map_w1,
+                                                         const __grid_constant__ CUtensorMap map_w2,
+                                                         const __grid_constant__ CUtensorMap map_p,
+                                                         const __grid_constant__ CUtensorMap map_dx, const float* b1,
+                                                         float* ws, int M) {
+  using G = MlpBwdCfg<C>;
+  constexpr int BM = G::BM, KB = G::KB, NH = G::NH, STAGES = G::STAGES, NX = G::NX, NS = G::NS, N4 = 4 * C;
+  extern __shared__ __align__(1024) uint8_t smem_raw[];
+  uint8_t* xs = smem_raw + ((1024u - (smem_u32(smem_raw) & 1023u)) & 1023u);
+  uint8_t* wsm = xs + 2 * NX * G::X_BYTES;
+  uint8_t* stg = wsm + STAGES * G::STAGE_BYTES;
+  float* cs_part = reinterpret_cast<float*>(stg + NS * G::CHUNK_BYTES);
+  uint64_t* full = reinterpret_cast<uint64_t*>(stg + NS * G::CHUNK_BYTES + G::CS_BYTES);
+  uint64_t* empty = full + STAGES;
+  uint64_t* x_full = empty + STAGES;
+  uint64_t* x_empty = x_full + NX;
+  uint64_t* cs_full = x_empty + NX;
+  uint64_t* cs_empty = cs_full + 2;
+
+  const int wg = threadIdx.x >> 7;
+  const int num_items = (M + BM - 1) / BM;
+  if (threadIdx.x == 0) {
+    asm volatile("prefetch.tensormap [%0];\n" ::"l"(&map_dy) : "memory");
+    asm volatile("prefetch.tensormap [%0];\n" ::"l"(&map_x) : "memory");
+    asm volatile("prefetch.tensormap [%0];\n" ::"l"(&map_w1) : "memory");
+    asm volatile("prefetch.tensormap [%0];\n" ::"l"(&map_w2) : "memory");
+    for (int i = 0; i < STAGES; i++) { mbar_init(&full[i], 1); mbar_init(&empty[i], 256); }
+    for (int i = 0; i < NX; i++) { mbar_init(&x_full[i], 1); mbar_init(&x_empty[i], 2); }
+    for (int i = 0; i < 2; i++) { mbar_init(&cs_full[i], 8); mbar_init(&cs_empty[i], FOLD_THREADS); }
+    asm volatile("fence.mbarrier_init.release.cluster;\n" ::: "memory");
+  }
+  __syncthreads();
+
+  if (wg == 2) {
+    asm volatile("setmaxnreg.dec.sync.aligned.u32 40;\n" ::: "memory");
+    if (threadIdx.x == 256) {
+      int stage = 0;
+      uint32_t phase = 0;
+      int local = 0;
+      for (int item = blockIdx.x; item < num_items; item += gridDim.x, local++) {
+        const int m0 = item * BM, xb = local % NX;
+        for (int j = 0; j < NH; j++) {
+          mbar_wait(&empty[stage], phase ^ 1);
+          const uint32_t sw = smem_u32(wsm + stage * G::STAGE_BYTES);
+          mbar_expect_tx(&full[stage], G::STAGE_BYTES);
+#pragma unroll
+          for (int kb = 0; kb < KB; kb++) tma_load_2d(sw + kb * 8192, &map_w1, &full[stage], kb * 64, j * 64);
+          tma_load_2d(sw + G::W1_BYTES, &map_w2, &full[stage], j * 64, 0);
+          if (++stage == STAGES) { stage = 0; phase ^= 1; }
+          if (j == 0) {
+            mbar_wait(&x_empty[xb], ((local / NX) & 1) ^ 1);
+            mbar_expect_tx(&x_full[xb], 2 * G::X_BYTES);
+            const uint32_t dst = smem_u32(xs + 2 * xb * G::X_BYTES);
+#pragma unroll
+            for (int kb = 0; kb < KB; kb++) {
+              tma_load_2d(dst + kb * BM * 128, &map_dy, &x_full[xb], kb * 64, m0);
+              tma_load_2d(dst + G::X_BYTES + kb * BM * 128, &map_x, &x_full[xb], kb * 64, m0);
+            }
+          }
+        }
+      }
+    } else if (threadIdx.x >= 256 + 32 && threadIdx.x < 256 + 32 + FOLD_THREADS) {
+      const int t = threadIdx.x - 256 - 32;
+      int g = 0;
+      for (int item = blockIdx.x; item < num_items; item += gridDim.x) {
+        for (int j = 0; j < NH; j++, g++) {
+          const int cb = g & 1;
+          mbar_wait(&cs_full[cb], (g >> 1) & 1);
+          float sum = 0.f;
+#pragma unroll
+          for (int w = 0; w < 8; w++) sum += cs_part[(cb * 8 + w) * 64 + t];
+          ws[(long long)item * N4 + j * 64 + t] = sum;
+          mbar_arrive(&cs_empty[cb]);
+        }
+      }
+    }
+  } else {
+    asm volatile("setmaxnreg.inc.sync.aligned.u32 232;\n" ::: "memory");
+    const int t = threadIdx.x & 127, warp = t >> 5, lane = t & 31;
+    const int frag_col = 2 * (lane & 3);
+    const uint32_t lrow = (uint32_t)(warp * 16 + (lane & 15)) * 128u, lsw = lane & 7, lblk = lane >> 4;
+    const bool leader = t == 0;
+    int stage = 0, g = 0;
+    uint32_t phase = 0;
+    int local = 0;
+    for (int item = blockIdx.x; item < num_items; item += gridDim.x, local++) {
+      const int m0 = item * BM, xb = local % NX;
+      uint8_t* const dybuf = xs + 2 * xb * G::X_BYTES;
+      const uint64_t ddy = make_smem_desc(smem_u32(dybuf) + wg * 8192, false);
+      float acc0[32], acc2[G::NP / 2];
+      float acc1[G::OVERLAP ? 32 : 1];
+      float (&acc)[32] = *reinterpret_cast<float (*)[32]>(G::OVERLAP ? acc1 : acc0);
+      mbar_wait(&x_full[xb], (local / NX) & 1);
+      for (int j = 0; j < NH; j++, g++) {
+        const uint32_t sw = smem_u32(wsm + stage * G::STAGE_BYTES);
+        if (leader) bulk_wait_read<NS - 1>();
+        named_barrier(1 + wg, 128);
+        mbar_wait(&full[stage], phase);
+        {
+          const uint64_t db = make_smem_desc(sw, false);
+          wgmma_fence();
+#pragma unroll
+          for (int k = 0; k < C / 16; k++)
+            wgmma_ss_n64(acc0, ddy + (G::X_BYTES >> 4) + (k >> 2) * (BM * 128 >> 4) + (k & 3) * 2,
+                         db + (k >> 2) * (8192 >> 4) + (k & 3) * 2, k ? 1u : 0u);
+          wgmma_commit();
+        }
+        auto dy_w2 = [&]() {
+          const uint64_t db = make_smem_desc(sw + G::W1_BYTES, true);
+          wgmma_fence();
+#pragma unroll
+          for (int k = 0; k < C / 16; k++)
+            wgmma_ss_n64<1>(acc, ddy + (k >> 2) * (BM * 128 >> 4) + (k & 3) * 2, db + k * (2048 >> 4), k ? 1u : 0u);
+          wgmma_commit();
+        };
+        if constexpr (G::OVERLAP) {
+          dy_w2();
+          wgmma_wait<1>();
+        } else {
+          wgmma_wait<0>();
+        }
+        uint32_t gp[4][4];
+        const float* bj = b1 + j * 64 + frag_col;
+#pragma unroll
+        for (int s = 0; s < 4; s++) {
+          const float* a0 = acc0 + 8 * s;
+          float b[4] = {0.f, 0.f, 0.f, 0.f};
+          if (b1) {
+#pragma unroll
+            for (int u = 0; u < 2; u++) {
+              const float2 bb = __ldg(reinterpret_cast<const float2*>(bj + (2 * s + u) * 8));
+              b[2 * u] = bb.x; b[2 * u + 1] = bb.y;
+            }
+          }
+#pragma unroll
+          for (int q = 0; q < 4; q++) {
+            float d0, d1;
+            gelu_fwd_grad(a0[2 * q] + b[2 * (q >> 1)], d0);
+            gelu_fwd_grad(a0[2 * q + 1] + b[2 * (q >> 1) + 1], d1);
+            gp[s][q] = pack_bf162(d0, d1);
+          }
+        }
+        if constexpr (!G::OVERLAP) dy_w2();
+        wgmma_wait<0>();
+        const uint32_t buf = smem_u32(stg + (g % NS) * G::CHUNK_BYTES) + wg * 8192;
+        const int cb = g & 1;
+        mbar_wait(&cs_empty[cb], ((g >> 1) & 1) ^ 1);
+#pragma unroll
+        for (int s = 0; s < 4; s++) {
+          const float* a0 = acc + 8 * s;
+          float cs[2][2] = {{0.f, 0.f}, {0.f, 0.f}};
+#pragma unroll
+          for (int q = 0; q < 4; q++) {
+            const float2 mf = unpack_bf162(gp[s][q]);
+            gp[s][q] = pack_bf162(a0[2 * q] * mf.x, a0[2 * q + 1] * mf.y);
+            const float2 of = unpack_bf162(gp[s][q]);
+            cs[q >> 1][0] += of.x; cs[q >> 1][1] += of.y;
+          }
+          stmatrix_x4(buf + lrow + (((2 * s + lblk) ^ lsw) << 4), gp[s][0], gp[s][1], gp[s][2], gp[s][3]);
+#pragma unroll
+          for (int u = 0; u < 2; u++) {
+            float cs0 = cs[u][0], cs1 = cs[u][1];
+#pragma unroll
+            for (int o2 = 4; o2 < 32; o2 <<= 1) {
+              cs0 += __shfl_xor_sync(0xffffffffu, cs0, o2);
+              cs1 += __shfl_xor_sync(0xffffffffu, cs1, o2);
+            }
+            if (lane < 4)
+              *reinterpret_cast<float2*>(cs_part + (cb * 8 + wg * 4 + warp) * 64 + (2 * s + u) * 8 + frag_col) =
+                  make_float2(cs0, cs1);
+          }
+        }
+        fence_proxy_async();
+        __syncwarp();
+        if (lane == 0) mbar_arrive(&cs_full[cb]);
+        const uint64_t d1 = make_smem_desc(sw, true);
+        wgmma_fence();
+#pragma unroll
+        for (int s = 0; s < 4; s++) wgmma_rs<1>(acc2, gp[s], d1 + s * (2048 >> 4), (j > 0 || s > 0) ? 1u : 0u);
+        wgmma_commit();
+        named_barrier(1 + wg, 128);
+        if (leader) {
+          if (m0 + 64 * wg < M) tma_store_2d(&map_p, buf, j * 64, m0 + 64 * wg);
+          bulk_commit();
+        }
+        wgmma_wait<0>();
+        mbar_arrive(&empty[stage]);
+        if (++stage == STAGES) { stage = 0; phase ^= 1; }
+      }
+#pragma unroll
+      for (int c = 0; c < KB; c++) {
+        const uint32_t dbuf = smem_u32(dybuf + c * BM * 128) + wg * 8192;
+#pragma unroll
+        for (int jj = 0; jj < 8; jj += 2) {
+          const int i = c * 8 + jj;
+          if (i >= C / 8) continue;
+          const float* a0 = acc2 + 4 * i;
+          uint32_t o[4];
+#pragma unroll
+          for (int q = 0; q < 4; q++) o[q] = pack_bf162(a0[2 * q], a0[2 * q + 1]);
+          stmatrix_x4(dbuf + lrow + (((jj + lblk) ^ lsw) << 4), o[0], o[1], o[2], o[3]);
+        }
+      }
+      fence_proxy_async();
+      named_barrier(1 + wg, 128);
+      if (leader) {
+        if (m0 + 64 * wg < M) {
+#pragma unroll
+          for (int c = 0; c < KB; c++) tma_store_2d(&map_dx, smem_u32(dybuf + c * BM * 128) + wg * 8192, c * 64, m0 + 64 * wg);
+        }
+        bulk_commit();
+        bulk_wait_read<0>();
+        mbar_arrive(&x_empty[xb]);
       }
     }
     if (t == 0) bulk_wait_all();
@@ -743,7 +997,7 @@
   if (!make_map(&mx, x, M, C, G::BM) || !make_map(&m1, w1, 4 * C, C, 64) || !make_map(&m2, w2, C, 4 * C, C) ||
       !make_map(&my, y, M, C, 64))
     return ESVIT_ERR_BAD_ARG;
-  if (STORE && (!make_map(&mh, h, M, 4 * C, 64) || !make_map(&mg, g, M, 4 * C, 64))) return ESVIT_ERR_BAD_ARG;
+  if (STORE && (!make_map(&mh, h, M, 4 * C, 64) || (g && !make_map(&mg, g, M, 4 * C, 64)))) return ESVIT_ERR_BAD_ARG;
   auto kernel = mlp_fwd_kernel<C, STORE>;
   static bool attr_set = false;
   if (!attr_set) {
@@ -755,7 +1009,7 @@
   int grid = esvit_num_sms();
   if (grid > items) grid = items;
   MlpParams p;
-  p.b1 = b1; p.b2 = b2; p.M = M;
+  p.b1 = b1; p.b2 = b2; p.M = M; p.store_g = g != nullptr;
   kernel<<<grid, 384, G::SMEM, (cudaStream_t)stream>>>(mx, m1, m2, my, mh, mg, p);
   return (int)cudaGetLastError();
 }
@@ -773,6 +1027,16 @@
   float s = 0.f;
   for (int r = 0; r < rows; r++) s += ws[(long long)r * N + n];
   colsum[n] += s;
+}
+
+__global__ void __launch_bounds__(256) row_group_fold_kernel(const float* __restrict__ ws, int rows, int N, int group,
+                                                             float* __restrict__ out) {
+  const int n = blockIdx.x * 256 + threadIdx.x;
+  if (n >= N) return;
+  const int r0 = blockIdx.y * group, r1 = r0 + group < rows ? r0 + group : rows;
+  float s = 0.f;
+  for (int r = r0; r < r1; r++) s += ws[(long long)r * N + n];
+  out[(long long)blockIdx.y * N + n] = s;
 }
 
 __global__ void __launch_bounds__(256) split_fold_kernel(const float* __restrict__ part, int splits, long long n4,
@@ -785,6 +1049,40 @@
     s.x += t.x; s.y += t.y; s.z += t.z; s.w += t.w;
   }
   reinterpret_cast<float4*>(out)[i] = s;
+}
+
+constexpr int MLP_BWD_GROUP = 32;
+static long long mlp_bwd_ws_floats(long long M, int C) {
+  const long long items = (M + 127) / 128;
+  return (items + (items + MLP_BWD_GROUP - 1) / MLP_BWD_GROUP) * 4LL * C;
+}
+
+template <int C>
+static int mlp_bwd_launch(const void* dy, const void* x, const void* w1, const float* b1, const void* w2, void* dpre,
+                          void* dx, float* db1, float* ws, int M, int grid, void* stream) {
+  using G = MlpBwdCfg<C>;
+  CUtensorMap mdy, mxx, m1, m2, mp, mdx;
+  if (!make_map(&mdy, dy, M, C, G::BM) || !make_map(&mxx, x, M, C, G::BM) || !make_map(&m1, w1, 4 * C, C, 64) ||
+      !make_map(&m2, w2, C, 4 * C, C) || !make_map(&mp, dpre, M, 4 * C, 64) || !make_map(&mdx, dx, M, C, 64))
+    return ESVIT_ERR_BAD_ARG;
+  auto kernel = mlp_bwd_kernel<C>;
+  static bool attr_set = false;
+  if (!attr_set) {
+    cudaError_t e = cudaFuncSetAttribute(kernel, cudaFuncAttributeMaxDynamicSharedMemorySize, G::SMEM);
+    if (e != cudaSuccess) return (int)e;
+    attr_set = true;
+  }
+  const int items = (M + G::BM - 1) / G::BM;
+  if (grid <= 0) grid = esvit_num_sms();
+  if (grid > items) grid = items;
+  kernel<<<grid, 384, G::SMEM, (cudaStream_t)stream>>>(mdy, mxx, m1, m2, mp, mdx, b1, ws, M);
+  cudaError_t e = cudaGetLastError();
+  if (e != cudaSuccess) return (int)e;
+  const int N4 = 4 * C, groups = (items + MLP_BWD_GROUP - 1) / MLP_BWD_GROUP;
+  float* ws2 = ws + (long long)items * N4;
+  row_group_fold_kernel<<<dim3((N4 + 255) / 256, groups), 256, 0, (cudaStream_t)stream>>>(ws, items, N4, MLP_BWD_GROUP, ws2);
+  colsum_fold_kernel<<<(N4 + 255) / 256, 256, 0, (cudaStream_t)stream>>>(ws2, groups, N4, db1);
+  return (int)cudaGetLastError();
 }
 
 constexpr int MAX_GRID = 160;
@@ -965,10 +1263,10 @@
   ESVIT_LAUNCH_CHECK();
 }
 
-ESVIT_API int esvit_mlp_fwd(const void* x, const void* w1, const float* b1, const void* w2, const float* b2, void* y,
-                            void* h, void* gelu_grad, long long M, int C, void* stream) {
+static int mlp_fwd_checked(const void* x, const void* w1, const float* b1, const void* w2, const float* b2, void* y, void* h,
+                           void* gelu_grad, long long M, int C, void* stream) {
   auto aligned = [](const void* q, uintptr_t a) { return ((uintptr_t)q & (a - 1)) == 0; };
-  if (M <= 0 || M > 0x7fffffffLL || !x || !w1 || !w2 || !y || (h == nullptr) != (gelu_grad == nullptr)) return ESVIT_ERR_BAD_ARG;
+  if (M <= 0 || M > 0x7fffffffLL || !x || !w1 || !w2 || !y) return ESVIT_ERR_BAD_ARG;
   if (!aligned(x, 16) || !aligned(w1, 16) || !aligned(w2, 16) || !aligned(y, 16) || !aligned(h, 16) ||
       !aligned(gelu_grad, 16) || !aligned(b1, 8) || !aligned(b2, 8))
     return ESVIT_ERR_BAD_ARG;
@@ -979,6 +1277,36 @@
   }
   return ESVIT_ERR_BAD_ARG;
 }
+ESVIT_API int esvit_mlp_fwd(const void* x, const void* w1, const float* b1, const void* w2, const float* b2, void* y,
+                            void* h, void* gelu_grad, long long M, int C, void* stream) {
+  if ((h == nullptr) != (gelu_grad == nullptr)) return ESVIT_ERR_BAD_ARG;
+  return mlp_fwd_checked(x, w1, b1, w2, b2, y, h, gelu_grad, M, C, stream);
+}
+ESVIT_API int esvit_mlp_fwd_h(const void* x, const void* w1, const float* b1, const void* w2, const float* b2, void* y,
+                              void* h, long long M, int C, void* stream) {
+  if (!h) return ESVIT_ERR_BAD_ARG;
+  return mlp_fwd_checked(x, w1, b1, w2, b2, y, h, nullptr, M, C, stream);
+}
+
+ESVIT_API int esvit_mlp_bwd_ws_floats(long long M, int C) {
+  const long long n = M > 0 && M <= 0x7fffffffLL ? hg::mlp_bwd_ws_floats(M, C) : -1;
+  return n > 0x7fffffffLL ? -1 : (int)n;
+}
+ESVIT_API int esvit_mlp_bwd(const void* dy, const void* x, const void* w1, const float* b1, const void* w2, void* dpre,
+                            void* dx, float* db1, float* ws, long long M, int C, int grid, void* stream) {
+  auto aligned = [](const void* q, uintptr_t a) { return ((uintptr_t)q & (a - 1)) == 0; };
+  if (M <= 0 || M > 0x7fffffffLL || !dy || !x || !w1 || !w2 || !dpre || !dx || !db1 || !ws || grid < 0)
+    return ESVIT_ERR_BAD_ARG;
+  if (!aligned(dy, 16) || !aligned(x, 16) || !aligned(w1, 16) || !aligned(w2, 16) || !aligned(dpre, 16) ||
+      !aligned(dx, 16) || !aligned(b1, 8) || !aligned(db1, 8) || !aligned(ws, 8))
+    return ESVIT_ERR_BAD_ARG;
+  switch (C) {
+    case 96: return hg::mlp_bwd_launch<96>(dy, x, w1, b1, w2, dpre, dx, db1, ws, (int)M, grid, stream);
+    case 128: return hg::mlp_bwd_launch<128>(dy, x, w1, b1, w2, dpre, dx, db1, ws, (int)M, grid, stream);
+    case 192: return hg::mlp_bwd_launch<192>(dy, x, w1, b1, w2, dpre, dx, db1, ws, (int)M, grid, stream);
+  }
+  return ESVIT_ERR_BAD_ARG;
+}
 
 ESVIT_API int esvit_gemm_bias_act(const void* a, const void* w, const float* bias, void* out, void* pre, long long M,
                                   int N, int K, int act, void* stream) {
diff --git a/esvit_b200/linear.py b/esvit_b200/linear.py
--- a/esvit_b200/linear.py
+++ b/esvit_b200/linear.py
@@ -55,7 +55,7 @@
         C = x.shape[-1]
         if act == 1 and C in ops.MLP_FUSED_C and w1.shape[0] == 4 * C:
             if need:
-                y, h, pre = ops.mlp_fwd(x, w1, b1, w2, b2, want_h=True)
+                (y, h), pre = ops.mlp_fwd(x, w1, b1, w2, b2, want_h=True, want_pre=False), None
             else:
                 y, h, pre = ops.mlp_fwd(x, w1, b1, w2, b2), None, None
         else:
@@ -64,7 +64,7 @@
             else:
                 h, pre = ops.gemm(x, w1, b1, act=act), None
             y = ops.gemm(h, w2, b2)
-        ctx.save_for_backward(x, w1, w2, pre, h)
+        ctx.save_for_backward(x, w1, w2, pre, h, b1 if pre is None else None)
         ctx.keys = (("w", w1p.data_ptr()), tuple(w1p.shape), ("w", w2p.data_ptr()), tuple(w2p.shape))
         ctx.bias_meta = (b1.shape, b1.device, b1.data_ptr())
         return y
@@ -72,15 +72,19 @@
     @staticmethod
     @once_differentiable
     def backward(ctx, g):
-        x, w1, w2, pre, h = ctx.saved_tensors
+        x, w1, w2, pre, h, b1 = ctx.saved_tensors
         k1, s1, k2, s2 = ctx.keys
         g = ops._chk(g, BF16, "g")
-        Cc, Nh = g.shape[-1], pre.shape[-1]
+        Cc, Nh = g.shape[-1], h.shape[-1]
         g2 = g.reshape(-1, Cc)
         dw2 = _wgrad(k2, g2, h.reshape(-1, Nh), s2) if ctx.needs_input_grad[4] else None
         db1, first = ops._acc(("bias", ctx.bias_meta[2]), tuple(ctx.bias_meta[0]), ctx.bias_meta[1])
-        dpre = ops.gemm_mul_colsum(g2, w2, pre.reshape(-1, Nh), db1, b_mn=True)
-        dx = ops.gemm(dpre, w1, None, b_mn=True).view(x.shape) if ctx.needs_input_grad[0] else None
+        if pre is None:
+            dpre, dx = ops.mlp_bwd(g2, x, w1, b1, w2, db1)
+            dx = dx.view(x.shape) if ctx.needs_input_grad[0] else None
+        else:
+            dpre = ops.gemm_mul_colsum(g2, w2, pre.reshape(-1, Nh), db1, b_mn=True)
+            dx = ops.gemm(dpre, w1, None, b_mn=True).view(x.shape) if ctx.needs_input_grad[0] else None
         dw1 = _wgrad(k1, dpre, x.reshape(-1, x.shape[-1]), s1) if ctx.needs_input_grad[1] else None
         return dx, dw1, None, (db1 if first else None), dw2, None, None, None
 
diff --git a/esvit_b200/ops.py b/esvit_b200/ops.py
--- a/esvit_b200/ops.py
+++ b/esvit_b200/ops.py
@@ -652,7 +652,8 @@
 MLP_FUSED_C = (96, 128, 192)
 
 
-def mlp_fwd(x: Tensor, w1: Tensor, b1: Optional[Tensor], w2: Tensor, b2: Optional[Tensor], want_h: bool = False):
+def mlp_fwd(x: Tensor, w1: Tensor, b1: Optional[Tensor], w2: Tensor, b2: Optional[Tensor], want_h: bool = False,
+            want_pre: bool = True):
     x, w1, w2 = _chk(x, BF16, "x"), _chk(w1, BF16, "w1"), _chk(w2, BF16, "w2")
     b1, b2 = _chk(b1, F32, "b1"), _chk(b2, F32, "b2")
     C = x.shape[-1]
@@ -660,9 +661,30 @@
     assert tuple(w1.shape) == (4 * C, C) and tuple(w2.shape) == (C, 4 * C), (x.shape, w1.shape, w2.shape)
     y = torch.empty_like(x)
     h = torch.empty(*x.shape[:-1], 4 * C, dtype=BF16, device=x.device) if want_h else None
+    if want_h and not want_pre:
+        _lib.call("esvit_mlp_fwd_h", _p(x), _p(w1), _p(b1), _p(w2), _p(b2), _p(y), _p(h), M, C, _stream())
+        return y, h
     pre = torch.empty_like(h) if want_h else None
     _lib.call("esvit_mlp_fwd", _p(x), _p(w1), _p(b1), _p(w2), _p(b2), _p(y), _p(h), _p(pre), M, C, _stream())
     return (y, h, pre) if want_h else y
+
+
+def mlp_bwd(dy: Tensor, x: Tensor, w1: Tensor, b1: Optional[Tensor], w2: Tensor, db1: Tensor, grid: int = 0):
+    dy, x, w1, w2 = _chk(dy, BF16, "dy"), _chk(x, BF16, "x"), _chk(w1, BF16, "w1"), _chk(w2, BF16, "w2")
+    b1 = _chk(b1, F32, "b1")
+    C = dy.shape[-1]
+    M = dy.numel() // C
+    assert tuple(w1.shape) == (4 * C, C) and tuple(w2.shape) == (C, 4 * C) and x.numel() == M * C, \
+        (dy.shape, x.shape, w1.shape, w2.shape)
+    dpre = torch.empty(M, 4 * C, dtype=BF16, device=dy.device)
+    dx = torch.empty_like(dy)
+    n = _lib.load().esvit_mlp_bwd_ws_floats(M, C)
+    if n <= 0:
+        raise ValueError(f"esvit_mlp_bwd: no workspace size for M = {M}, C = {C}")
+    ws = torch.empty(n, dtype=F32, device=dy.device)
+    _lib.call("esvit_mlp_bwd", _p(dy), _p(x), _p(w1), _p(b1), _p(w2), _p(dpre), _p(dx), _p(db1), _p(ws), M, C, grid,
+              _stream())
+    return dpre, dx
 
 
 _wgrad_ws = {}
diff --git a/include/esvit_b200.h b/include/esvit_b200.h
--- a/include/esvit_b200.h
+++ b/include/esvit_b200.h
@@ -55,6 +55,11 @@
                      int tile, void* stream);
 int esvit_mlp_fwd(const void* x, const void* w1, const float* b1, const void* w2, const float* b2, void* y, void* h,
                   void* gelu_grad, long long M, int C, void* stream);
+int esvit_mlp_fwd_h(const void* x, const void* w1, const float* b1, const void* w2, const float* b2, void* y, void* h,
+                    long long M, int C, void* stream);
+int esvit_mlp_bwd_ws_floats(long long M, int C);
+int esvit_mlp_bwd(const void* dy, const void* x, const void* w1, const float* b1, const void* w2, void* dpre, void* dx,
+                  float* db1, float* ws, long long M, int C, int grid, void* stream);
 
 int esvit_gelu_fwd(const void* x, void* y, long long n, void* stream);
 int esvit_gelu_bwd(const void* x, const void* dy, void* dx, long long n, void* stream);
```

Result: faster. 1384, median of 6 (+1.4%).
